# hyx1999/SAM-Decoding

Hardware: AMD Instinct MI355X
Metric: tokens/sec (+ mean accepted tokens), Vicuna-7B bs=1, samd_sam_only draft+verify (higher is better)
Workload: dtype f16

## Files before the change

sam-decoding_amd/csrc/gemm_kernels.hip:

```cpp
#include <hip/hip_runtime.h>
#include <cstdlib>
#include <type_traits>
#include "samd_common.h"

#define LAUNCHCHK() do { hipError_t e_ = hipGetLastError(); if (e_ != hipSuccess) { samd_set_error("kernel launch: %s", hipGetErrorString(e_)); return SAMD_E_HIP; } } while (0)

static int samd_cu_count() { return samd_device_cus(); }

typedef _Float16 half8 __attribute__((ext_vector_type(8)));
typedef __bf16 bf16x8 __attribute__((ext_vector_type(8)));
typedef float floatx4 __attribute__((ext_vector_type(4)));
typedef unsigned u32x4 __attribute__((ext_vector_type(4)));

struct GF16 { typedef _Float16 elem; typedef half8 vec8;
    static __device__ __forceinline__ floatx4 mfma(half8 a, half8 b, floatx4 c) { return __builtin_amdgcn_mfma_f32_16x16x32_f16(a, b, c, 0, 0, 0); } };
struct GBF16 { typedef __bf16 elem; typedef bf16x8 vec8;
    static __device__ __forceinline__ floatx4 mfma(bf16x8 a, bf16x8 b, floatx4 c) { return __builtin_amdgcn_mfma_f32_16x16x32_bf16(a, b, c, 0, 0, 0); } };

#define GEMM_KC 256
#define GEMM_WAVES 8
#define GEMM_COLS (16 * GEMM_WAVES)

typedef __attribute__((address_space(1))) const void *gptr_t;
typedef __attribute__((address_space(3))) void *lptr_t;

#ifdef SAMD_GEMM_ABLATE
__device__ int samd_abl_flag;
#endif

template <typename TT, int RT, int EPI, int DEPTH, bool GM = false>
__global__ __launch_bounds__(64 * GEMM_WAVES, RT >= 3 || DEPTH > 2 ? 2 : GEMM_WAVES / 2) void k_gemm_skinny(const typename TT::elem *__restrict__ A, const typename TT::elem *__restrict__ W,
                                                        float *__restrict__ partial, typename TT::elem *__restrict__ out,
                                                        int K, int N, int n_chunks, int n_splits) {
    typedef typename TT::elem E;
    typedef typename TT::vec8 V8;
    constexpr int R = 16 * RT;
    constexpr int NT = 64 * GEMM_WAVES;
    constexpr int XV = (R * 32) / NT;
    constexpr int NB = DEPTH + 1;
    extern __shared__ __attribute__((aligned(1024))) char gemm_lds[];
    E (*xs)[R][GEMM_KC] = reinterpret_cast<E (*)[R][GEMM_KC]>(gemm_lds);

    const int tid = threadIdx.x, w = tid >> 6, l = tid & 63, n = l & 15, g = l >> 4;
    const int n0 = blockIdx.x * GEMM_COLS + 16 * w;
    const int split = blockIdx.y;
    const int c0 = (int)((long long)split * n_chunks / n_splits), c1 = (int)((long long)(split + 1) * n_chunks / n_splits);
    constexpr size_t WCH = GM ? 8192 : 65536, WU = GM ? 1024 : 8192;
    const int ws = GM ? __builtin_amdgcn_readfirstlane(GEMM_WAVES * (int)blockIdx.x + w) : (int)blockIdx.x;
    const char *wtile = reinterpret_cast<const char *>(W) + (size_t)ws * n_chunks * WCH;
    const uint32_t wlane = (uint32_t)(GM ? l : tid) * 16;
    const uint32_t lds_base = (uint32_t)(uintptr_t)(lptr_t)&xs[0][0][0];

    floatx4 acc[RT];
#pragma unroll
    for (int mt = 0; mt < RT; mt++) acc[mt] = (floatx4){0.f, 0.f, 0.f, 0.f};

    u32x4 wr[DEPTH][4][2];
    auto load_wb = [&](u32x4 (&dst)[4][2], int c, int b) {
        const char *p = wtile + (size_t)c * WCH;
#pragma unroll
        for (int j = 0; j < 2; j++)
            asm volatile("global_load_dwordx4 %0, %1, %2 nt" : "=v"(dst[b][j]) : "v"(wlane), "s"(p + WU * (2 * b + j)) : "memory");
    };
    auto stage_xi = [&](int c, int buf, int i) {
        const int slot = tid + NT * i, row = slot >> 5, pos = slot & 31, unit = pos ^ (row & 15);
        const E *src = A + (size_t)row * K + (size_t)c * GEMM_KC + 8 * unit;
        E *dst = &xs[buf][0][0] + (size_t)(NT * i + 64 * w) * 8;
        __builtin_amdgcn_global_load_lds((gptr_t)src, (lptr_t)dst, 16, 0, 0);
        asm volatile("" ::: "memory");
    };
    auto load_w = [&](u32x4 (&dst)[4][2], int c) {
#pragma unroll
        for (int b = 0; b < 4; b++) load_wb(dst, c, b);
    };
    auto stage_x = [&](int c, int buf) {
#pragma unroll
        for (int i = 0; i < XV; i++) stage_xi(c, buf, i);
    };
    auto landed = [&](int younger_in_flight) {
        if (DEPTH > 2 && younger_in_flight >= 2) asm volatile("s_waitcnt vmcnt(%0)" : : "n"(2 * (8 + XV)) : "memory");
        else if (younger_in_flight >= 1) asm volatile("s_waitcnt vmcnt(%0)" : : "n"(8 + XV) : "memory");
        else asm volatile("s_waitcnt vmcnt(0)" : : : "memory");
        __builtin_amdgcn_s_barrier();
        asm volatile("" ::: "memory");
    };
    auto phase = [&](u32x4 (&cur)[4][2], int c, int buf) {
        landed(c1 - 1 - c);
        const uint32_t xbase = lds_base + (uint32_t)buf * (R * GEMM_KC * 2) + (uint32_t)n * (GEMM_KC * 2);
#pragma unroll
        for (int b = 0; b < 4; b++) {
            const uint32_t u0 = (uint32_t)((8 * b + 2 * g) ^ n) * 16, u1 = (uint32_t)((8 * b + 2 * g + 1) ^ n) * 16;
            const uint32_t a0 = xbase + u0, a1 = xbase + u1;
            u32x4 r[RT][2];
            if constexpr (RT == 1)
                asm volatile("ds_read_b128 %0, %2\n\tds_read_b128 %1, %3\n\ts_waitcnt lgkmcnt(0)" : "=&v"(r[0][0]), "=&v"(r[0][1]) : "v"(a0), "v"(a1));
            else if constexpr (RT == 2)
                asm volatile("ds_read_b128 %0, %4\n\tds_read_b128 %1, %5\n\tds_read_b128 %2, %4 offset:8192\n\tds_read_b128 %3, %5 offset:8192\n\t"
                             "s_waitcnt lgkmcnt(0)" : "=&v"(r[0][0]), "=&v"(r[0][1]), "=&v"(r[1][0]), "=&v"(r[1][1]) : "v"(a0), "v"(a1));
            else if constexpr (RT == 3)
                asm volatile("ds_read_b128 %0, %6\n\tds_read_b128 %1, %7\n\tds_read_b128 %2, %6 offset:8192\n\tds_read_b128 %3, %7 offset:8192\n\t"
                             "ds_read_b128 %4, %6 offset:16384\n\tds_read_b128 %5, %7 offset:16384\n\ts_waitcnt lgkmcnt(0)"
                             : "=&v"(r[0][0]), "=&v"(r[0][1]), "=&v"(r[1][0]), "=&v"(r[1][1]), "=&v"(r[2][0]), "=&v"(r[2][1]) : "v"(a0), "v"(a1));
            else
                asm volatile("ds_read_b128 %0, %8\n\tds_read_b128 %1, %9\n\tds_read_b128 %2, %8 offset:8192\n\tds_read_b128 %3, %9 offset:8192\n\t"
                             "ds_read_b128 %4, %8 offset:16384\n\tds_read_b128 %5, %9 offset:16384\n\tds_read_b128 %6, %8 offset:24576\n\t"
                             "ds_read_b128 %7, %9 offset:24576\n\ts_waitcnt lgkmcnt(0)"
                             : "=&v"(r[0][0]), "=&v"(r[0][1]), "=&v"(r[1][0]), "=&v"(r[1][1]), "=&v"(r[2][0]), "=&v"(r[2][1]), "=&v"(r[3][0]), "=&v"(r[3][1])
                             : "v"(a0), "v"(a1));
#pragma unroll
            for (int mt = 0; mt < RT; mt++) {
                acc[mt] = TT::mfma(__builtin_bit_cast(V8, r[mt][0]), __builtin_bit_cast(V8, cur[b][0]), acc[mt]);
                acc[mt] = TT::mfma(__builtin_bit_cast(V8, r[mt][1]), __builtin_bit_cast(V8, cur[b][1]), acc[mt]);
            }
            if (RT >= 3 && c + DEPTH < c1) {
                load_wb(cur, c + DEPTH, b);
                if (b < XV) stage_xi(c + DEPTH, buf == 0 ? NB - 1 : buf - 1, b);
            }
        }
        if (RT < 3 && c + DEPTH < c1) { load_w(cur, c + DEPTH); stage_x(c + DEPTH, buf == 0 ? NB - 1 : buf - 1); }
    };
    if (c0 < c1) {
#pragma unroll
        for (int d = 0; d < DEPTH; d++)
            if (c0 + d < c1) { load_w(wr[d], c0 + d); stage_x(c0 + d, d); }
        int buf = 0;
        for (int c = c0; c < c1; c += DEPTH) {
#pragma unroll
            for (int d = 0; d < DEPTH; d++)
                if (c + d < c1) { phase(wr[d], c + d, buf); buf = buf == NB - 1 ? 0 : buf + 1; }
        }
    }
    if constexpr (EPI == 1) {
        float *ex = reinterpret_cast<float *>(gemm_lds);
        __syncthreads();
        if (w >= 4) {
#pragma unroll
            for (int mt = 0; mt < RT; mt++)
#pragma unroll
                for (int r = 0; r < 4; r++) ex[(16 * mt + 4 * g + r) * 64 + 16 * (w - 4) + n] = acc[mt][r];
        }
        __syncthreads();
        if (w < 4) {
#pragma unroll
            for (int mt = 0; mt < RT; mt++)
#pragma unroll
                for (int r = 0; r < 4; r++) {
                    const int m = 16 * mt + 4 * g + r;
                    const float gf = (float)(E)acc[mt][r], uf = (float)(E)ex[m * 64 + 16 * w + n];
                    const E sv = (E)(gf / (1.f + __expf(-gf)));
                    out[(size_t)m * (N / 2) + blockIdx.x * 64 + 16 * w + n] = (E)((float)sv * uf);
                }
        }
        return;
    }
#pragma unroll
    for (int mt = 0; mt < RT; mt++) {
#pragma unroll
        for (int r = 0; r < 4; r++) {
            const int m = 16 * mt + 4 * g + r;
            if (out) out[(size_t)m * N + n0 + n] = (E)acc[mt][r];
            else __hip_atomic_store(&partial[((size_t)split * R + m) * N + n0 + n], acc[mt][r], __ATOMIC_RELAXED, __HIP_MEMORY_SCOPE_AGENT);
        }
    }
}

struct NormArgs { const float *ssq; const void *g; int tiles; float inv_hidden; float eps; };

#define NORM_NS 16
template <int NT>
__device__ __forceinline__ void norm_issue(const NormArgs &na, float (&sv)[NORM_NS]) {
    const int tid = threadIdx.x, row = tid & 15, p = tid >> 4;
#pragma unroll
    for (int k = 0; k < NORM_NS; k++) {
        sv[k] = 0.f;
        if ((NT / 16) * k >= na.tiles) continue;
        int t = p + (NT / 16) * k;
        t = t < na.tiles ? t : na.tiles - 1;
        const float *src = na.ssq + (size_t)t * 16 + row;
        asm volatile("global_load_dword %0, %1, off" : "=v"(sv[k]) : "v"(src) : "memory");
    }
}
template <int NT>
__device__ __forceinline__ void norm_finish(const NormArgs &na, float (&sv)[NORM_NS], float *part , float *rs ) {
    const int tid = threadIdx.x, row = tid & 15, p = tid >> 4;
    static_assert(NORM_NS == 16, "");
    asm volatile("" : "+v"(sv[0]), "+v"(sv[1]), "+v"(sv[2]), "+v"(sv[3]), "+v"(sv[4]), "+v"(sv[5]), "+v"(sv[6]), "+v"(sv[7]),
                      "+v"(sv[8]), "+v"(sv[9]), "+v"(sv[10]), "+v"(sv[11]), "+v"(sv[12]), "+v"(sv[13]), "+v"(sv[14]), "+v"(sv[15]) : : "memory");
    float s = 0.f;
#pragma unroll
    for (int k = 0; k < NORM_NS; k++) s += (p + (NT / 16) * k < na.tiles) ? sv[k] : 0.f;
    part[p * 16 + row] = s;
    asm volatile("s_waitcnt lgkmcnt(0)" ::: "memory");
    __builtin_amdgcn_s_barrier();
    asm volatile("" ::: "memory");
    if (tid < 16) {
        float tot = 0.f;
        for (int k = 0; k < NT / 16; k++) tot += part[k * 16 + tid];
        rs[tid] = rsqrtf(tot * na.inv_hidden + na.eps);
    }
    asm volatile("s_waitcnt lgkmcnt(0)" ::: "memory");
    __builtin_amdgcn_s_barrier();
    asm volatile("" ::: "memory");
}

template <typename E>
__device__ __forceinline__ u32x4 norm_scale8(u32x4 xraw, u32x4 graw, float rs) {
    const E *xe = reinterpret_cast<const E *>(&xraw);
    const E *ge = reinterpret_cast<const E *>(&graw);
    u32x4 out;
    E *oe = reinterpret_cast<E *>(&out);
#pragma unroll
    for (int j = 0; j < 8; j++) { const E h = (E)((float)xe[j] * rs); oe[j] = (E)((float)ge[j] * (float)h); }
    return out;
}


template <int DEPTH, int PC>
__device__ __forceinline__ void gemm_wait_younger(int younger) {
    if constexpr (PC == 0) asm volatile("s_waitcnt vmcnt(0)" : : : "memory");
    else {
        if (DEPTH > 3 && younger >= 3) asm volatile("s_waitcnt vmcnt(%0)" : : "n"(3 * PC) : "memory");
        else if (DEPTH > 2 && younger >= 2) asm volatile("s_waitcnt vmcnt(%0)" : : "n"(2 * PC) : "memory");
        else if (younger >= 1) asm volatile("s_waitcnt vmcnt(%0)" : : "n"(PC) : "memory");
        else asm volatile("s_waitcnt vmcnt(0)" : : : "memory");
    }
}

template <typename TT, int RT, int DEPTH, int CG, bool NORM, int AR = 16>
__global__ __launch_bounds__(64 * GEMM_WAVES, RT >= 3 || NORM ? 2 : GEMM_WAVES / 2) void k_gemm_qkv_rope(
        const typename TT::elem *__restrict__ A, const typename TT::elem *__restrict__ W, int K, int n_chunks,
        const float *__restrict__ cs, const int *__restrict__ d_L, const int *__restrict__ d_n,
        typename TT::elem *__restrict__ q_out, typename TT::elem *__restrict__ k_cache, typename TT::elem *__restrict__ v_cache,
        int H, int Hkv, long long max_len, NormArgs na, int v_t) {
    typedef typename TT::elem E;
    typedef typename TT::vec8 V8;
    constexpr int R = 16 * RT;
    constexpr int NT = 64 * GEMM_WAVES;
    constexpr int XV = (R * 32) / NT;
    constexpr int NB = DEPTH + 1;
    constexpr int WL = 4;
    constexpr int TW = 16 * CG, PP = 8 * CG;
    constexpr int CH = CG * 8192;
    extern __shared__ __attribute__((aligned(1024))) char gemm_lds[];
    E (*xs)[R][GEMM_KC] = reinterpret_cast<E (*)[R][GEMM_KC]>(gemm_lds);

    const int tid = threadIdx.x, w = tid >> 6, l = tid & 63, n = l & 15, g = l >> 4;
    const bool streams = CG == 4 || w < 2 * CG;
    static_assert(AR == 16 || (AR == 8 && NORM && RT == 1), "8 activation rows: the norm-fold kernels only");
    const bool stager = AR == 16 || w < GEMM_WAVES / 2;
    const int cg = CG == 4 ? (w & 3) : (streams ? w % CG : 0), kh = CG == 4 ? (w >> 2) : (streams ? w / CG : 0);
    const char *wtile = reinterpret_cast<const char *>(W) + (size_t)blockIdx.x * n_chunks * CH;
    const uint32_t wlane = (uint32_t)(64 * (CG * kh + cg) + l) * 16;
    const uint32_t lds_base = (uint32_t)(uintptr_t)(lptr_t)&xs[0][0][0];
    const int n_rows = d_n[0], L = d_L[0];

    floatx4 acc[RT];
#pragma unroll
    for (int mt = 0; mt < RT; mt++) acc[mt] = (floatx4){0.f, 0.f, 0.f, 0.f};

    u32x4 wr[DEPTH][2][2];
    auto load_wb = [&](u32x4 (&dst)[2][2], int c, int bl) {
        const char *p = wtile + (size_t)c * CH;
#pragma unroll
        for (int j = 0; j < 2; j++)
            asm volatile("global_load_dwordx4 %0, %1, %2 nt" : "=v"(dst[bl][j]) : "v"(wlane), "s"(p + (CH / 4) * (2 * bl + j)) : "memory");
    };
    static_assert(!NORM || RT == 1, "the norm-fold path is built for the 16-row tile");
    constexpr int XL = NORM ? 2 * XV : XV;
    u32x4 xr[NORM ? DEPTH : 1][NORM ? XV : 1], gr[NORM ? DEPTH : 1][NORM ? XV : 1];
    __shared__ float norm_part[NORM ? (NT / 16) * 16 : 1], norm_rs[NORM ? 16 : 1];
    auto stage_xi = [&](int c, int buf, int i, int d) {
        const int slot = tid + NT * i, row = slot >> 5, pos = slot & 31, unit = pos ^ (row & 15);
        const E *src = A + (size_t)row * K + (size_t)c * GEMM_KC + 8 * unit;
        if constexpr (NORM) {
            const E *gsrc = reinterpret_cast<const E *>(na.g) + (size_t)c * GEMM_KC + 8 * unit;
            asm volatile("global_load_dwordx4 %0, %1, off" : "=v"(xr[d][i]) : "v"(src) : "memory");
            asm volatile("global_load_dwordx4 %0, %1, off" : "=v"(gr[d][i]) : "v"(gsrc) : "memory");
        } else {
            E *dst = &xs[buf][0][0] + (size_t)(NT * i + 64 * w) * 8;
            __builtin_amdgcn_global_load_lds((gptr_t)src, (lptr_t)dst, 16, 0, 0);
            asm volatile("" ::: "memory");
        }
    };
    auto issue = [&](u32x4 (&dst)[2][2], int c, int buf, int d) {
        if (streams) { load_wb(dst, c, 0); load_wb(dst, c, 1); }
        if (stager) {
#pragma unroll
            for (int i = 0; i < XV; i++) stage_xi(c, buf, i, d);
        }
    };
    auto scale_to_lds = [&](int buf, int d) {
        if constexpr (NORM) {
            if (!stager) return;
#pragma unroll
            for (int i = 0; i < XV; i++) {
                const int slot = tid + NT * i, row = slot >> 5;
                asm volatile("" : "+v"(xr[d][i]), "+v"(gr[d][i]) : : "memory");
                const u32x4 v = norm_scale8<E>(xr[d][i], gr[d][i], norm_rs[row]);
                *reinterpret_cast<u32x4 *>(&xs[buf][0][0] + (size_t)slot * 8) = v;
            }
        }
    };
    auto landed = [&](int younger, int buf, int d) {
        if (streams) { if (stager) gemm_wait_younger<DEPTH, WL + XL>(younger); else gemm_wait_younger<DEPTH, WL>(younger); }
        else { if (stager) gemm_wait_younger<DEPTH, XL>(younger); else gemm_wait_younger<DEPTH, 0>(younger); }
        if constexpr (NORM) { scale_to_lds(buf, d); asm volatile("s_waitcnt lgkmcnt(0)" ::: "memory"); }
        __builtin_amdgcn_s_barrier();
        asm volatile("" ::: "memory");
    };
    auto phase = [&](u32x4 (&cur)[2][2], int c, int buf, int d) {
        landed(n_chunks - 1 - c, buf, d);
        const uint32_t xbase = lds_base + (uint32_t)buf * (R * GEMM_KC * 2) + (uint32_t)n * (GEMM_KC * 2);
#pragma unroll
        for (int bl = 0; bl < 2; bl++) {
            if (!streams) break;
            const int b = 2 * kh + bl;
            const uint32_t a0 = xbase + (uint32_t)((8 * b + 2 * g) ^ n) * 16, a1 = xbase + (uint32_t)((8 * b + 2 * g + 1) ^ n) * 16;
            u32x4 r[RT][2];
            if constexpr (RT == 1)
                asm volatile("ds_read_b128 %0, %2\n\tds_read_b128 %1, %3\n\ts_waitcnt lgkmcnt(0)" : "=&v"(r[0][0]), "=&v"(r[0][1]) : "v"(a0), "v"(a1));
            else if constexpr (RT == 2)
                asm volatile("ds_read_b128 %0, %4\n\tds_read_b128 %1, %5\n\tds_read_b128 %2, %4 offset:8192\n\tds_read_b128 %3, %5 offset:8192\n\t"
                             "s_waitcnt lgkmcnt(0)" : "=&v"(r[0][0]), "=&v"(r[0][1]), "=&v"(r[1][0]), "=&v"(r[1][1]) : "v"(a0), "v"(a1));
            else if constexpr (RT == 3)
                asm volatile("ds_read_b128 %0, %6\n\tds_read_b128 %1, %7\n\tds_read_b128 %2, %6 offset:8192\n\tds_read_b128 %3, %7 offset:8192\n\t"
                             "ds_read_b128 %4, %6 offset:16384\n\tds_read_b128 %5, %7 offset:16384\n\ts_waitcnt lgkmcnt(0)"
                             : "=&v"(r[0][0]), "=&v"(r[0][1]), "=&v"(r[1][0]), "=&v"(r[1][1]), "=&v"(r[2][0]), "=&v"(r[2][1]) : "v"(a0), "v"(a1));
            else
                asm volatile("ds_read_b128 %0, %8\n\tds_read_b128 %1, %9\n\tds_read_b128 %2, %8 offset:8192\n\tds_read_b128 %3, %9 offset:8192\n\t"
                             "ds_read_b128 %4, %8 offset:16384\n\tds_read_b128 %5, %9 offset:16384\n\tds_read_b128 %6, %8 offset:24576\n\t"
                             "ds_read_b128 %7, %9 offset:24576\n\ts_waitcnt lgkmcnt(0)"
                             : "=&v"(r[0][0]), "=&v"(r[0][1]), "=&v"(r[1][0]), "=&v"(r[1][1]), "=&v"(r[2][0]), "=&v"(r[2][1]), "=&v"(r[3][0]), "=&v"(r[3][1])
                             : "v"(a0), "v"(a1));
#pragma unroll
            for (int mt = 0; mt < RT; mt++) {
                acc[mt] = TT::mfma(__builtin_bit_cast(V8, r[mt][0]), __builtin_bit_cast(V8, cur[bl][0]), acc[mt]);
                acc[mt] = TT::mfma(__builtin_bit_cast(V8, r[mt][1]), __builtin_bit_cast(V8, cur[bl][1]), acc[mt]);
            }
        }
        if (c + DEPTH < n_chunks) issue(cur, c + DEPTH, buf == 0 ? NB - 1 : buf - 1, d);
    };
    float norm_sv[NORM ? NORM_NS : 1];
    if constexpr (NORM) norm_issue<NT>(na, norm_sv);
#pragma unroll
    for (int d = 0; d < DEPTH; d++)
        if (d < n_chunks) issue(wr[d], d, d, d);
    if constexpr (AR == 8) {
        if (!stager) {
#pragma unroll
            for (int bz = 0; bz < NB; bz++) *reinterpret_cast<u32x4 *>(&xs[bz][0][0] + (size_t)tid * 8) = (u32x4){0u, 0u, 0u, 0u};
        }
    }
    if constexpr (NORM) {
        if (n_chunks >= DEPTH) {
            if (streams) { if (stager) asm volatile("s_waitcnt vmcnt(%0)" : : "n"(DEPTH * (WL + XL)) : "memory"); else asm volatile("s_waitcnt vmcnt(%0)" : : "n"(DEPTH * WL) : "memory"); }
            else { if (stager) asm volatile("s_waitcnt vmcnt(%0)" : : "n"(DEPTH * XL) : "memory"); else asm volatile("s_waitcnt vmcnt(0)" : : : "memory"); }
        } else asm volatile("s_waitcnt vmcnt(0)" : : : "memory");
        norm_finish<NT>(na, norm_sv, norm_part, norm_rs);
    }
    {
        int buf = 0;
        for (int c = 0; c < n_chunks; c += DEPTH) {
#pragma unroll
            for (int d = 0; d < DEPTH; d++)
                if (c + d < n_chunks) { phase(wr[d], c + d, buf, d); buf = buf == NB - 1 ? 0 : buf + 1; }
        }
    }
    float *ex = reinterpret_cast<float *>(gemm_lds);
    __syncthreads();
    if (streams) {
#pragma unroll
        for (int mt = 0; mt < RT; mt++)
#pragma unroll
            for (int r = 0; r < 4; r++) ex[(kh * R + 16 * mt + 4 * g + r) * TW + 16 * cg + n] = acc[mt][r];
    }
    __syncthreads();
    const bool vt_tile = v_t && ((PP * (int)blockIdx.x) >> 6) >= H + Hkv;
    for (int i = tid; i < R * PP; i += NT) {
        const int row = vt_tile ? i % R : i / PP, p = vt_tile ? i / R : i % PP;
        if (row >= n_rows || L + row >= max_len) continue;
        const float x1 = (float)(E)(ex[row * TW + p] + ex[(R + row) * TW + p]);
        const float x2 = (float)(E)(ex[row * TW + PP + p] + ex[(R + row) * TW + PP + p]);
        const int pair = PP * (int)blockIdx.x + p, head = pair >> 6, j = pair & 63;
        if (head >= H + Hkv) {
            if (v_t) {
                E *dst = v_cache + (size_t)(head - H - Hkv) * max_len * 128 + L + row;
                dst[(size_t)j * max_len] = (E)x1; dst[(size_t)(j + 64) * max_len] = (E)x2;
                continue;
            }
            E *dst = v_cache + ((size_t)(head - H - Hkv) * max_len + L + row) * 128;
            dst[j] = (E)x1; dst[j + 64] = (E)x2;
            continue;
        }
        const float c = cs[(size_t)row * 128 + j], sn = cs[(size_t)row * 128 + 64 + j];
        const E o1 = (E)(x1 * c - x2 * sn), o2 = (E)(x2 * c + x1 * sn);
        E *dst = head < H ? q_out + ((size_t)row * H + head) * 128 : k_cache + ((size_t)(head - H) * max_len + L + row) * 128;
        dst[j] = o1; dst[j + 64] = o2;
    }
}

template <int CG>
__global__ __launch_bounds__(256) void k_gemm_pack_qkv(const uint4 *__restrict__ W, uint4 *__restrict__ out, int N, int K) {
    const long long u = (long long)blockIdx.x * 256 + threadIdx.x;
    const long long total = (long long)N * K / 8;
    if (u >= total) return;
    constexpr int PP = 8 * CG;
    const int n_chunks = K / GEMM_KC;
    const long long blk = u / (512 * CG);
    const int in = (int)(u % (512 * CG)), jj = in / (128 * CG), x = in % (128 * CG), w = x >> 6, g = (x >> 4) & 3, n = x & 15, cg = w % CG, kh = w / CG;
    const int t = (int)(blk / n_chunks), c = (int)(blk % n_chunks), bl = jj >> 1, j = jj & 1;
    const int q = 16 * cg + n, pair = PP * t + (q < PP ? q : q - PP);
    const long long row = 128LL * (pair >> 6) + (pair & 63) + (q < PP ? 0 : 64), col = 256LL * c + 64 * (2 * kh + bl) + 16 * g + 8 * j;
    out[u] = W[(row * K + col) / 8];
}

static int qkv_tile_groups(int n_heads_total) {
    static const int env = [] { const char *e = getenv("SAMD_QKV_TILE"); return e ? atoi(e) : 0; }();
    const int n_cu = samd_cu_count();
    const int N = n_heads_total * 128;
    if (N % 48 != 0 || env == 64) return 4;
    if (env == 48) return 3;
    const int t48 = N / 48, t64 = N / 64;
    return ((t48 + n_cu - 1) / n_cu) * 48 < ((t64 + n_cu - 1) / n_cu) * 64 ? 3 : 4;
}

template <typename TT, int RT, int DEPTH, bool NORM, int AR = 16>
__global__ __launch_bounds__(64 * GEMM_WAVES, RT >= 3 || DEPTH > 2 ? 2 : GEMM_WAVES / 2) void k_gemm_pairs_silu(const typename TT::elem *__restrict__ A, const typename TT::elem *__restrict__ W,
                                                                                                     typename TT::elem *__restrict__ out, int K, int inter, int n_chunks, int n_pairs, NormArgs na) {
    typedef typename TT::elem E;
    typedef typename TT::vec8 V8;
    constexpr int R = 16 * RT;
    constexpr int NT = 64 * GEMM_WAVES;
    constexpr int XV = (R * 32) / NT;
    constexpr int NB = DEPTH + 1;
    extern __shared__ __attribute__((aligned(1024))) char gemm_lds[];
    E (*xs)[R][GEMM_KC] = reinterpret_cast<E (*)[R][GEMM_KC]>(gemm_lds);

    const int tid = threadIdx.x, w = __builtin_amdgcn_readfirstlane(tid >> 6), l = tid & 63, n = l & 15, g = l >> 4;
#ifdef SAMD_GEMM_ABLATE
    const int abl = samd_abl_flag;
#else
    constexpr int abl = 0;
#endif
    const int p0 = (int)((long long)blockIdx.x * n_pairs / gridDim.x), p1 = (int)((long long)(blockIdx.x + 1) * n_pairs / gridDim.x);
    const bool active = w < 2 * (p1 - p0);
    static_assert(AR == 16 || (AR == 8 && NORM && RT == 1), "8 activation rows: the norm-fold kernels only");
    const bool stager = AR == 16 || w < GEMM_WAVES / 2;
    const int gi = 2 * p0 + w;
    const char *wgrp = reinterpret_cast<const char *>(W) + (size_t)(active ? gi : 0) * n_chunks * 8192;
    const uint32_t wlane = (uint32_t)l * 16;
    const uint32_t lds_base = (uint32_t)(uintptr_t)(lptr_t)&xs[0][0][0];

    floatx4 acc[RT];
#pragma unroll
    for (int mt = 0; mt < RT; mt++) acc[mt] = (floatx4){0.f, 0.f, 0.f, 0.f};
    u32x4 wr[DEPTH][4][2];
    auto load_w = [&](u32x4 (&dst)[4][2], int c) {
        const char *p = wgrp + (size_t)c * 8192;
#pragma unroll
        for (int b = 0; b < 4; b++)
#pragma unroll
            for (int j = 0; j < 2; j++)
                asm volatile("global_load_dwordx4 %0, %1, %2 nt" : "=v"(dst[b][j]) : "v"(wlane), "s"(p + 1024 * (2 * b + j)) : "memory");
    };
    static_assert(!NORM || RT == 1, "the norm-fold path is built for the 16-row tile");
    constexpr int XL = NORM ? 2 * XV : XV;
    u32x4 xr[NORM ? DEPTH : 1][NORM ? XV : 1], gr[NORM ? DEPTH : 1][NORM ? XV : 1];
    __shared__ float norm_part[NORM ? (NT / 16) * 16 : 1], norm_rs[NORM ? 16 : 1];
    auto stage_x = [&](int c, int buf, int d) {
        if (!stager || (abl & 4)) return;
#pragma unroll
        for (int i = 0; i < XV; i++) {
            const int slot = tid + NT * i, row = slot >> 5, pos = slot & 31, unit = pos ^ (row & 15);
            const E *src = A + (size_t)((abl & 8) ? (row & 15) : row) * K + (size_t)c * GEMM_KC + 8 * unit;
            if constexpr (NORM) {
                const E *gsrc = reinterpret_cast<const E *>(na.g) + (size_t)c * GEMM_KC + 8 * unit;
                asm volatile("global_load_dwordx4 %0, %1, off" : "=v"(xr[d][i]) : "v"(src) : "memory");
                asm volatile("global_load_dwordx4 %0, %1, off" : "=v"(gr[d][i]) : "v"(gsrc) : "memory");
            } else {
                E *dst = &xs[buf][0][0] + (size_t)(NT * i + 64 * w) * 8;
                __builtin_amdgcn_global_load_lds((gptr_t)src, (lptr_t)dst, 16, 0, 0);
                asm volatile("" ::: "memory");
            }
        }
    };
    auto landed = [&](int younger, int buf, int d) {
        const bool stg = stager && !(abl & 4);
        if (active) { if (stg) gemm_wait_younger<DEPTH, 8 + XL>(younger); else gemm_wait_younger<DEPTH, 8>(younger); }
        else { if (stg) gemm_wait_younger<DEPTH, XL>(younger); else gemm_wait_younger<DEPTH, 0>(younger); }
        if constexpr (NORM) {
            if (stager) {
#pragma unroll
                for (int i = 0; i < XV; i++) {
                    const int slot = tid + NT * i, row = slot >> 5;
                    asm volatile("" : "+v"(xr[d][i]), "+v"(gr[d][i]) : : "memory");
                    const u32x4 v = norm_scale8<E>(xr[d][i], gr[d][i], norm_rs[row]);
                    *reinterpret_cast<u32x4 *>(&xs[buf][0][0] + (size_t)slot * 8) = v;
                }
            }
            asm volatile("s_waitcnt lgkmcnt(0)" ::: "memory");
        }
        if (!(abl & 1)) __builtin_amdgcn_s_barrier();
        asm volatile("" ::: "memory");
    };
    auto phase = [&](u32x4 (&cur)[4][2], int c, int buf, int d) {
        landed(n_chunks - 1 - c, buf, d);
        if (active && !(abl & 2)) {
            const uint32_t xbase = lds_base + (uint32_t)buf * (R * GEMM_KC * 2) + (uint32_t)n * (GEMM_KC * 2);
#pragma unroll
            for (int b = 0; b < 4; b++) {
                const uint32_t a0 = xbase + (uint32_t)((8 * b + 2 * g) ^ n) * 16, a1 = xbase + (uint32_t)((8 * b + 2 * g + 1) ^ n) * 16;
                u32x4 r[RT][2];
                if constexpr (RT == 1)
                    asm volatile("ds_read_b128 %0, %2\n\tds_read_b128 %1, %3\n\ts_waitcnt lgkmcnt(0)" : "=&v"(r[0][0]), "=&v"(r[0][1]) : "v"(a0), "v"(a1));
                else if constexpr (RT == 2)
                    asm volatile("ds_read_b128 %0, %4\n\tds_read_b128 %1, %5\n\tds_read_b128 %2, %4 offset:8192\n\tds_read_b128 %3, %5 offset:8192\n\t"
                                 "s_waitcnt lgkmcnt(0)" : "=&v"(r[0][0]), "=&v"(r[0][1]), "=&v"(r[1][0]), "=&v"(r[1][1]) : "v"(a0), "v"(a1));
                else if constexpr (RT == 3)
                    asm volatile("ds_read_b128 %0, %6\n\tds_read_b128 %1, %7\n\tds_read_b128 %2, %6 offset:8192\n\tds_read_b128 %3, %7 offset:8192\n\t"
                                 "ds_read_b128 %4, %6 offset:16384\n\tds_read_b128 %5, %7 offset:16384\n\ts_waitcnt lgkmcnt(0)"
                                 : "=&v"(r[0][0]), "=&v"(r[0][1]), "=&v"(r[1][0]), "=&v"(r[1][1]), "=&v"(r[2][0]), "=&v"(r[2][1]) : "v"(a0), "v"(a1));
                else
                    asm volatile("ds_read_b128 %0, %8\n\tds_read_b128 %1, %9\n\tds_read_b128 %2, %8 offset:8192\n\tds_read_b128 %3, %9 offset:8192\n\t"
                                 "ds_read_b128 %4, %8 offset:16384\n\tds_read_b128 %5, %9 offset:16384\n\tds_read_b128 %6, %8 offset:24576\n\t"
                                 "ds_read_b128 %7, %9 offset:24576\n\ts_waitcnt lgkmcnt(0)"
                                 : "=&v"(r[0][0]), "=&v"(r[0][1]), "=&v"(r[1][0]), "=&v"(r[1][1]), "=&v"(r[2][0]), "=&v"(r[2][1]), "=&v"(r[3][0]), "=&v"(r[3][1])
                                 : "v"(a0), "v"(a1));
#pragma unroll
                for (int mt = 0; mt < RT; mt++) {
                    acc[mt] = TT::mfma(__builtin_bit_cast(V8, r[mt][0]), __builtin_bit_cast(V8, cur[b][0]), acc[mt]);
                    acc[mt] = TT::mfma(__builtin_bit_cast(V8, r[mt][1]), __builtin_bit_cast(V8, cur[b][1]), acc[mt]);
                }
            }
        }
        if (c + DEPTH < n_chunks) { if (active) load_w(cur, c + DEPTH); stage_x(c + DEPTH, buf == 0 ? NB - 1 : buf - 1, d); }
    };
    float norm_sv[NORM ? NORM_NS : 1];
    if constexpr (NORM) norm_issue<NT>(na, norm_sv);
#pragma unroll
    for (int d = 0; d < DEPTH; d++)
        if (d < n_chunks) { if (active) load_w(wr[d], d); stage_x(d, d, d); }
    if constexpr (AR == 8) {
        if (!stager) {
#pragma unroll
            for (int bz = 0; bz < NB; bz++) *reinterpret_cast<u32x4 *>(&xs[bz][0][0] + (size_t)tid * 8) = (u32x4){0u, 0u, 0u, 0u};
        }
    }
    if constexpr (NORM) {
        if (n_chunks >= DEPTH) {
            if (active) { if (stager) asm volatile("s_waitcnt vmcnt(%0)" : : "n"(DEPTH * (8 + XL)) : "memory"); else asm volatile("s_waitcnt vmcnt(%0)" : : "n"(DEPTH * 8) : "memory"); }
            else { if (stager) asm volatile("s_waitcnt vmcnt(%0)" : : "n"(DEPTH * XL) : "memory"); else asm volatile("s_waitcnt vmcnt(0)" : : : "memory"); }
        } else asm volatile("s_waitcnt vmcnt(0)" : : : "memory");
        norm_finish<NT>(na, norm_sv, norm_part, norm_rs);
    }
    {
        int buf = 0;
        for (int c = 0; c < n_chunks; c += DEPTH) {
#pragma unroll
            for (int d = 0; d < DEPTH; d++)
                if (c + d < n_chunks) { phase(wr[d], c + d, buf, d); buf = buf == NB - 1 ? 0 : buf + 1; }
        }
    }
    float *ex = reinterpret_cast<float *>(gemm_lds);
    __syncthreads();
    if (active && (w & 1)) {
#pragma unroll
        for (int mt = 0; mt < RT; mt++)
#pragma unroll
            for (int r = 0; r < 4; r++) ex[((w >> 1) * R + 16 * mt + 4 * g + r) * 16 + n] = acc[mt][r];
    }
    __syncthreads();
    if (active && !(w & 1)) {
        const int col = 16 * (p0 + (w >> 1)) + n;
#pragma unroll
        for (int mt = 0; mt < RT; mt++)
#pragma unroll
            for (int r = 0; r < 4; r++) {
                const int m = 16 * mt + 4 * g + r;
                const float gf = (float)(E)acc[mt][r], uf = (float)(E)ex[((w >> 1) * R + m) * 16 + n];
                const E sv = (E)(gf / (1.f + __expf(-gf)));
                out[(size_t)m * inter + col] = (E)((float)sv * uf);
            }
    }
}

template <typename TT, int ROWS, bool EARLY = false>
__global__ __launch_bounds__(64 * GEMM_WAVES, 2) void k_gemm_cs_residual(const typename TT::elem *__restrict__ A, const typename TT::elem *__restrict__ W,
                                                                           typename TT::elem *__restrict__ x, float *__restrict__ ssq, int K, int N, int n_chunks,
                                                                           const int *__restrict__ counter = nullptr, int *__restrict__ epoch = nullptr,
                                                                           int arrivals = 0) {
    typedef typename TT::elem E;
    typedef typename TT::vec8 V8;
    constexpr int CSD = 2;
    extern __shared__ __attribute__((aligned(1024))) char gemm_lds[];
    const int tid = threadIdx.x, w = __builtin_amdgcn_readfirstlane(tid >> 6), l = tid & 63, n = l & 15, g = l >> 4;
    E *xs = reinterpret_cast<E *>(gemm_lds) + (size_t)w * CSD * 16 * GEMM_KC;
    const uint32_t lds_base = (uint32_t)(uintptr_t)(lptr_t)xs;
    const char *wgrp = reinterpret_cast<const char *>(W) + (size_t)blockIdx.x * n_chunks * 8192;
    const uint32_t wlane = (uint32_t)l * 16;

    static_assert(ROWS == 8 || ROWS == 16, "");
    constexpr int AL = ROWS / 2;
    if constexpr (ROWS == 8) {
#pragma unroll
        for (int buf = 0; buf < CSD; buf++)
#pragma unroll
            for (int i = 4; i < 8; i++)
                *reinterpret_cast<u32x4 *>(xs + (size_t)buf * 16 * GEMM_KC + (size_t)(64 * i + l) * 8) = (u32x4){0u, 0u, 0u, 0u};
        asm volatile("s_waitcnt lgkmcnt(0)" ::: "memory");
    }
    floatx4 acc = (floatx4){0.f, 0.f, 0.f, 0.f};
    u32x4 wr[CSD][4][2];
    auto issue_w = [&](u32x4 (&dst)[4][2], int c) {
        const char *p = wgrp + (size_t)c * 8192;
#pragma unroll
        for (int b = 0; b < 4; b++)
#pragma unroll
            for (int j = 0; j < 2; j++)
                asm volatile("global_load_dwordx4 %0, %1, %2 nt" : "=v"(dst[b][j]) : "v"(wlane), "s"(p + 1024 * (2 * b + j)) : "memory");
    };
    auto issue_a = [&](int c, int buf) {
#pragma unroll
        for (int i = 0; i < AL; i++) {
            const int slot = l + 64 * i, row = slot >> 5, pos = slot & 31, unit = pos ^ (row & 15);
            const E *src = A + (size_t)row * K + (size_t)c * GEMM_KC + 8 * unit;
            E *dst_l = xs + (size_t)buf * 16 * GEMM_KC + (size_t)(64 * i) * 8;
            __builtin_amdgcn_global_load_lds((gptr_t)src, (lptr_t)dst_l, 16, 0, 0);
            asm volatile("" ::: "memory");
        }
    };
    auto issue = [&](u32x4 (&dst)[4][2], int c, int buf) { issue_w(dst, c); issue_a(c, buf); };
    auto phase = [&](u32x4 (&cur)[4][2], int c, int buf, bool more) {
        if (more) { if constexpr (EARLY) asm volatile("s_waitcnt vmcnt(%0)" : : "n"(AL) : "memory"); else asm volatile("s_waitcnt vmcnt(%0)" : : "n"(8 + AL) : "memory"); }
        else asm volatile("s_waitcnt vmcnt(0)" ::: "memory");
        const uint32_t xbase = lds_base + (uint32_t)buf * (16 * GEMM_KC * 2) + (uint32_t)n * (GEMM_KC * 2);
#pragma unroll
        for (int b = 0; b < 4; b++) {
            const uint32_t a0 = xbase + (uint32_t)((8 * b + 2 * g) ^ n) * 16, a1 = xbase + (uint32_t)((8 * b + 2 * g + 1) ^ n) * 16;
            u32x4 r0, r1;
            asm volatile("ds_read_b128 %0, %2\n\tds_read_b128 %1, %3\n\ts_waitcnt lgkmcnt(0)" : "=&v"(r0), "=&v"(r1) : "v"(a0), "v"(a1));
            acc = TT::mfma(__builtin_bit_cast(V8, r0), __builtin_bit_cast(V8, cur[b][0]), acc);
            acc = TT::mfma(__builtin_bit_cast(V8, r1), __builtin_bit_cast(V8, cur[b][1]), acc);
        }
    };
    const int mine = (n_chunks - w + GEMM_WAVES - 1) / GEMM_WAVES;
    if constexpr (EARLY) {
        if (mine > 0) issue_w(wr[0], w);
        if (mine > 1) issue_w(wr[1], w + GEMM_WAVES);
        __shared__ int my_epoch;
        if (tid == 0) {
            const int e = epoch[blockIdx.x];
            const int target = (e + 1) * arrivals;
            for (int spin = 0; spin < (1 << 22); spin++) {
                if (__hip_atomic_load(counter, __ATOMIC_RELAXED, __HIP_MEMORY_SCOPE_AGENT) >= target) break;
                __builtin_amdgcn_s_sleep(4);
            }
            my_epoch = e;
        }
        __syncthreads();
        __builtin_amdgcn_fence(__ATOMIC_ACQUIRE, "agent");
        if (mine > 0) issue_a(w, 0);
        if (mine > 1) issue_a(w + GEMM_WAVES, 1);
        if (mine > 0) phase(wr[0], w, 0, mine > 1);
        if (mine > 1) phase(wr[1], w + GEMM_WAVES, 1, false);
        if (tid == 0) epoch[blockIdx.x] = my_epoch + 1;
    } else {
        if (mine > 0) issue(wr[0], w, 0);
        if (mine > 1) issue(wr[1], w + GEMM_WAVES, 1);
        for (int i = 0; i < mine; i += 2) {
            phase(wr[0], w + GEMM_WAVES * i, 0, i + 1 < mine);
            if (i + 2 < mine) issue(wr[0], w + GEMM_WAVES * (i + 2), 0);
            if (i + 1 < mine) {
                phase(wr[1], w + GEMM_WAVES * (i + 1), 1, i + 2 < mine);
                if (i + 3 < mine) issue(wr[1], w + GEMM_WAVES * (i + 3), 1);
            }
        }
    }
    __syncthreads();
    float *ex = reinterpret_cast<float *>(gemm_lds);
#pragma unroll
    for (int r = 0; r < 4; r++) ex[(w * 16 + 4 * g + r) * 16 + n] = acc[r];
    __syncthreads();
    if (tid < 16 * ROWS) {
        const int row = tid >> 4, col = tid & 15;
        float sum = 0.f;
#pragma unroll
        for (int k = 0; k < GEMM_WAVES; k++) sum += ex[(k * 16 + row) * 16 + col];
        E *xp = x + (size_t)row * N + 16 * blockIdx.x + col;
        const E o = (E)sum;
        const E y = (E)((float)*xp + (float)o);
        *xp = y;
        float q = (float)y * (float)y;
        q += __shfl_xor(q, 1); q += __shfl_xor(q, 2); q += __shfl_xor(q, 4); q += __shfl_xor(q, 8);
        if (col == 0) ssq[(size_t)blockIdx.x * 16 + row] = q;
    }
}

__global__ __launch_bounds__(256) void k_gemm_pack_groups(const uint4 *__restrict__ W, uint4 *__restrict__ out, int N, int K) {
    const long long u = (long long)blockIdx.x * 256 + threadIdx.x;
    const long long total = (long long)N * K / 8;
    if (u >= total) return;
    const int n_chunks = K / GEMM_KC;
    const long long blk = u >> 9;
    const int in = (int)(u & 511), jj = in >> 6, lane = in & 63, g = lane >> 4, n = lane & 15, b = jj >> 1, j = jj & 1;
    const long long gi = blk / n_chunks; const int c = (int)(blk % n_chunks);
    const long long row = 16 * gi + n, col = 256LL * c + 64 * b + 16 * g + 8 * j;
    out[u] = W[(row * K + col) / 8];
}

__global__ __launch_bounds__(256) void k_gemm_pack(const uint4 *__restrict__ W, uint4 *__restrict__ out, int N, int K) {
    const long long u = (long long)blockIdx.x * 256 + threadIdx.x;
    const long long total = (long long)N * K / 8;
    if (u >= total) return;
    const int n_chunks = K / GEMM_KC;
    const long long blk = u >> 12;
    const int in = (int)(u & 4095), jj = in >> 9, tid = in & 511, w = tid >> 6, g = (tid >> 4) & 3, n = tid & 15;
    const int t = (int)(blk / n_chunks), c = (int)(blk % n_chunks), b = jj >> 1, j = jj & 1;
    const long long row = 128LL * t + 16 * w + n, col = 256LL * c + 64 * b + 16 * g + 8 * j;
    out[u] = W[(row * K + col) / 8];
}

template <typename TT, int RT, int EPI, int DEPTH, bool GM = false>
static hipError_t gemm_launch(dim3 grid, hipStream_t st, const void *A, const void *W, float *partial, void *out, int K, int N, int chunks, int splits) {
    constexpr int lds = (DEPTH + 1) * 16 * RT * GEMM_KC * 2;
    if constexpr (lds > 65536) {
        static unsigned long long done = 0ull;
        const hipError_t attr = samd_reserve_lds((const void *)k_gemm_skinny<TT, RT, EPI, DEPTH, GM>, lds, &done);
        if (attr != hipSuccess) return attr;
    }
    hipLaunchKernelGGL((k_gemm_skinny<TT, RT, EPI, DEPTH, GM>), grid, dim3(64 * GEMM_WAVES), lds, st, (const typename TT::elem *)A, (const typename TT::elem *)W, partial,
                       (typename TT::elem *)out, K, N, chunks, splits);
    return hipSuccess;
}

template <int EPI, bool GM = false>
static hipError_t gemm_dispatch(int dtype, int rows_pad, dim3 grid, hipStream_t st, const void *A, const void *W, float *partial, void *out, int K, int N, int chunks,
                                int splits) {
#define GO(TT, RT, D) return gemm_launch<TT, RT, EPI, D, GM>(grid, st, A, W, partial, out, K, N, chunks, splits)
#define ROWS(TT) do { if (rows_pad == 16) GO(TT, 1, 2); else if (rows_pad == 32) GO(TT, 2, 2); else if (rows_pad == 48) GO(TT, 3, 2); else GO(TT, 4, 2); } while (0)
    if (dtype == SAMD_F16) ROWS(GF16); else ROWS(GBF16);
#undef ROWS
#undef GO
}

template <typename TT, int RT, int DEPTH, int CG, bool NORM = false, int AR = 16>
static hipError_t qkv_rope_launch(hipStream_t st, const void *A, const void *W, int K, int tiles, const float *cs, const int *d_L, const int *d_n, void *q, void *k, void *v,
                                  int H, int Hkv, long long max_len, int v_t, NormArgs na = NormArgs{nullptr, nullptr, 0, 0.f, 0.f}) {
    constexpr int lds_a = (DEPTH + 1) * 16 * RT * GEMM_KC * 2, lds_e = 2 * 16 * RT * 16 * CG * 4, lds = lds_a > lds_e ? lds_a : lds_e;
    if constexpr (lds > 60000) {
        static unsigned long long done = 0ull;
        const hipError_t attr = samd_reserve_lds((const void *)k_gemm_qkv_rope<TT, RT, DEPTH, CG, NORM, AR>, lds + 4096, &done);
        if (attr != hipSuccess) return attr;
    }
    hipLaunchKernelGGL((k_gemm_qkv_rope<TT, RT, DEPTH, CG, NORM, AR>), dim3(tiles), dim3(64 * GEMM_WAVES), lds, st, (const typename TT::elem *)A, (const typename TT::elem *)W, K, K / GEMM_KC,
                       cs, d_L, d_n, (typename TT::elem *)q, (typename TT::elem *)k, (typename TT::elem *)v, H, Hkv, max_len, na, v_t);
    return hipSuccess;
}

template <typename TT, int RT, int DEPTH, bool NORM = false, int AR = 16>
static hipError_t pairs_silu_launch(hipStream_t st, int grid, const void *A, const void *W, void *out, int K, int inter, int n_pairs,
                                    NormArgs na = NormArgs{nullptr, nullptr, 0, 0.f, 0.f}) {
    constexpr int lds_a = (DEPTH + 1) * 16 * RT * GEMM_KC * 2, lds_e = 4 * 16 * RT * 16 * 4, lds = lds_a > lds_e ? lds_a : lds_e;
    if constexpr (lds > 60000) {
        static unsigned long long done = 0ull;
        const hipError_t attr = samd_reserve_lds((const void *)k_gemm_pairs_silu<TT, RT, DEPTH, NORM, AR>, lds + 4096, &done);
        if (attr != hipSuccess) return attr;
    }
    hipLaunchKernelGGL((k_gemm_pairs_silu<TT, RT, DEPTH, NORM, AR>), dim3(grid), dim3(64 * GEMM_WAVES), lds, st, (const typename TT::elem *)A, (const typename TT::elem *)W,
                       (typename TT::elem *)out, K, inter, K / GEMM_KC, n_pairs, na);
    return hipSuccess;
}

extern "C" {

int samd_gemm_splits(int32_t N, int32_t K, int32_t rows_pad) {
    static const int env_cap = [] { const char *e = getenv("SAMD_GEMM_SPLIT_CAP"); const int v = e ? atoi(e) : 8; return v < 1 ? 1 : (v > 8 ? 8 : v); }();
    static const int env_fixed = [] { const char *e = getenv("SAMD_GEMM_SPLITS"); const int v = e ? atoi(e) : 0; return v < 0 ? 0 : (v > 8 ? 8 : v); }();
    const int cols = N / GEMM_COLS, chunks = K / GEMM_KC;
    (void)rows_pad;
    if (env_fixed) return env_fixed > chunks ? (chunks < 1 ? 1 : chunks) : env_fixed;
    int s = 256 / (cols > 0 ? cols : 1);
    if (s > env_cap) s = env_cap;
    if (s > chunks) s = chunks;
    return s < 1 ? 1 : s;
}

int64_t samd_gemm_workspace(int32_t rows_pad, int32_t N, int32_t splits) { return (int64_t)splits * rows_pad * N * 4; }

int samd_gemm_skinny_silu(const void *d_A, const void *d_W, int32_t rows_pad, int32_t N, int32_t K, void *d_out, int32_t dtype, void *stream) {
    if (!d_A || !d_W || !d_out || (rows_pad != 16 && rows_pad != 32 && rows_pad != 48 && rows_pad != 64) || N < GEMM_COLS || N % GEMM_COLS != 0 || K < GEMM_KC ||
        K % GEMM_KC != 0 || (dtype != SAMD_F16 && dtype != SAMD_BF16)) {
        samd_set_error("samd_gemm_skinny_silu: unsupported shape (rows 16/32/48/64, N %% 128 == 0, K %% 256 == 0) or null pointer"); return SAMD_E_INVALID;
    }
    const hipError_t e = gemm_dispatch<1>(dtype, rows_pad, dim3(N / GEMM_COLS, 1), (hipStream_t)stream, d_A, d_W, nullptr, d_out, K, N, K / GEMM_KC, 1);
    if (e != hipSuccess) { samd_set_error("samd_gemm_skinny_silu: %s", hipGetErrorString(e)); return SAMD_E_HIP; }
    LAUNCHCHK();
    return SAMD_OK;
}

int samd_gemm_pack_weights(const void *d_W, void *d_packed, int32_t N, int32_t K, void *stream) {
    if (!d_W || !d_packed || d_W == d_packed || N < GEMM_COLS || N % GEMM_COLS != 0 || K < GEMM_KC || K % GEMM_KC != 0) {
        samd_set_error("samd_gemm_pack_weights: needs N %% 128 == 0, K %% 256 == 0 and distinct buffers"); return SAMD_E_INVALID;
    }
    const long long units = (long long)N * K / 8;
    hipLaunchKernelGGL(k_gemm_pack, dim3((unsigned)((units + 255) / 256)), dim3(256), 0, (hipStream_t)stream, (const uint4 *)d_W, (uint4 *)d_packed, N, K);
    LAUNCHCHK();
    return SAMD_OK;
}

int samd_gemm_pack_groups(const void *d_W, void *d_packed, int32_t N, int32_t K, void *stream) {
    if (!d_W || !d_packed || d_W == d_packed || N < 16 || N % 16 != 0 || K < GEMM_KC || K % GEMM_KC != 0) {
        samd_set_error("samd_gemm_pack_groups: needs N %% 16 == 0, K %% 256 == 0 and distinct buffers"); return SAMD_E_INVALID;
    }
    const long long units = (long long)N * K / 8;
    hipLaunchKernelGGL(k_gemm_pack_groups, dim3((unsigned)((units + 255) / 256)), dim3(256), 0, (hipStream_t)stream, (const uint4 *)d_W, (uint4 *)d_packed, N, K);
    LAUNCHCHK();
    return SAMD_OK;
}

int samd_gemm_pairs_silu_norm(const void *d_x, const float *d_ssq, const void *d_norm_weight, float eps, const void *d_Wg, int32_t rows_pad, int32_t inter, int32_t K,
                              void *d_out, int32_t dtype, void *stream) {
    if (!d_x || !d_ssq || !d_norm_weight || !d_Wg || !d_out || (rows_pad != 16 && rows_pad != 8) || inter < 16 || inter % 16 != 0 || K < GEMM_KC || K % GEMM_KC != 0 ||
        K / 16 > 32 * NORM_NS || (dtype != SAMD_F16 && dtype != SAMD_BF16)) {
        samd_set_error("samd_gemm_pairs_silu_norm: unsupported shape (8 or 16 rows, inter %% 16 == 0, K %% 256 == 0, K <= 8192, f16/bf16) or null pointer"); return SAMD_E_INVALID;
    }
    const int n_cu = samd_cu_count();
    const int n_pairs = inter / 16;
    int grid = n_pairs < n_cu ? n_pairs : n_cu;
    while ((n_pairs + grid - 1) / grid > 4) grid += n_cu;
    const NormArgs na{d_ssq, d_norm_weight, K / 16, 1.f / (float)K, eps};
    hipStream_t st = (hipStream_t)stream;
    const hipError_t e = rows_pad == 8
        ? (dtype == SAMD_F16 ? pairs_silu_launch<GF16, 1, 3, true, 8>(st, grid, d_x, d_Wg, d_out, K, inter, n_pairs, na)
                             : pairs_silu_launch<GBF16, 1, 3, true, 8>(st, grid, d_x, d_Wg, d_out, K, inter, n_pairs, na))
        : (dtype == SAMD_F16 ? pairs_silu_launch<GF16, 1, 3, true>(st, grid, d_x, d_Wg, d_out, K, inter, n_pairs, na)
                             : pairs_silu_launch<GBF16, 1, 3, true>(st, grid, d_x, d_Wg, d_out, K, inter, n_pairs, na));
    if (e != hipSuccess) { samd_set_error("samd_gemm_pairs_silu_norm: %s", hipGetErrorString(e)); return SAMD_E_HIP; }
    LAUNCHCHK();
    return SAMD_OK;
}

int samd_gemm_cs_residual(const void *d_A, const void *d_Wg, int32_t rows_pad, int32_t N, int32_t K, void *d_x, float *d_ssq, int32_t dtype, void *stream) {
    if (!d_A || !d_Wg || !d_x || !d_ssq || (rows_pad != 16 && rows_pad != 8) || N < 16 || N % 16 != 0 || K < GEMM_KC || K % GEMM_KC != 0 || (dtype != SAMD_F16 && dtype != SAMD_BF16)) {
        samd_set_error("samd_gemm_cs_residual: unsupported shape (8 or 16 rows, N %% 16 == 0, K %% 256 == 0, f16/bf16) or null pointer"); return SAMD_E_INVALID;
    }
    constexpr int lds = GEMM_WAVES * 2 * 16 * GEMM_KC * 2;
    hipStream_t st = (hipStream_t)stream;
    hipError_t e = hipSuccess;
#define GO(TT, ROWS, ET) do { static unsigned long long done = 0ull; \
        e = samd_reserve_lds((const void *)k_gemm_cs_residual<TT, ROWS>, lds, &done); \
        if (e == hipSuccess) hipLaunchKernelGGL((k_gemm_cs_residual<TT, ROWS>), dim3(N / 16), dim3(64 * GEMM_WAVES), lds, st, (const ET *)d_A, (const ET *)d_Wg, (ET *)d_x, d_ssq, K, N, K / GEMM_KC, (const int *)nullptr, (int *)nullptr, 0); } while (0)
    if (dtype == SAMD_F16) { if (rows_pad == 8) GO(GF16, 8, _Float16); else GO(GF16, 16, _Float16); }
    else { if (rows_pad == 8) GO(GBF16, 8, __bf16); else GO(GBF16, 16, __bf16); }
#undef GO
    if (e != hipSuccess) { samd_set_error("samd_gemm_cs_residual: %s", hipGetErrorString(e)); return SAMD_E_HIP; }
    LAUNCHCHK();
    return SAMD_OK;
}

int samd_gemm_cs_residual_early(const void *d_A, const void *d_Wg, int32_t N, int32_t K, void *d_x, float *d_ssq, int32_t dtype, const int32_t *d_counter,
                                int32_t *d_epoch, int32_t arrivals, void *stream) {
    if (!d_A || !d_Wg || !d_x || !d_ssq || !d_counter || !d_epoch || arrivals < 1 || N < 16 || N % 16 != 0 || K != 2 * GEMM_WAVES * GEMM_KC ||
        (dtype != SAMD_F16 && dtype != SAMD_BF16)) {
        samd_set_error("samd_gemm_cs_residual_early: unsupported shape (K must be 4096, N %% 16 == 0, f16/bf16) or null pointer"); return SAMD_E_INVALID;
    }
    constexpr int lds = GEMM_WAVES * 2 * 16 * GEMM_KC * 2;
    hipStream_t st = (hipStream_t)stream;
    hipError_t e = hipSuccess;
    if (dtype == SAMD_F16) {
        static unsigned long long done = 0ull;
        e = samd_reserve_lds((const void *)k_gemm_cs_residual<GF16, 8, true>, lds, &done);
        if (e == hipSuccess) hipLaunchKernelGGL((k_gemm_cs_residual<GF16, 8, true>), dim3(N / 16), dim3(64 * GEMM_WAVES), lds, st, (const _Float16 *)d_A, (const _Float16 *)d_Wg,
                                                (_Float16 *)d_x, d_ssq, K, N, K / GEMM_KC, d_counter, d_epoch, arrivals);
    } else {
        static unsigned long long done = 0ull;
        e = samd_reserve_lds((const void *)k_gemm_cs_residual<GBF16, 8, true>, lds, &done);
        if (e == hipSuccess) hipLaunchKernelGGL((k_gemm_cs_residual<GBF16, 8, true>), dim3(N / 16), dim3(64 * GEMM_WAVES), lds, st, (const __bf16 *)d_A, (const __bf16 *)d_Wg,
                                                (__bf16 *)d_x, d_ssq, K, N, K / GEMM_KC, d_counter, d_epoch, arrivals);
    }
    if (e != hipSuccess) { samd_set_error("samd_gemm_cs_residual_early: %s", hipGetErrorString(e)); return SAMD_E_HIP; }
    LAUNCHCHK();
    return SAMD_OK;
}

int samd_gemm_pairs_silu(const void *d_A, const void *d_Wg, int32_t rows_pad, int32_t inter, int32_t K, void *d_out, int32_t dtype, void *stream) {
    if (!d_A || !d_Wg || !d_out || (rows_pad != 16 && rows_pad != 32 && rows_pad != 48 && rows_pad != 64) || inter < 16 || inter % 16 != 0 || K < GEMM_KC ||
        K % GEMM_KC != 0 || (dtype != SAMD_F16 && dtype != SAMD_BF16)) {
        samd_set_error("samd_gemm_pairs_silu: unsupported shape (rows 16/32/48/64, inter %% 16 == 0, K %% 256 == 0, f16/bf16) or null pointer"); return SAMD_E_INVALID;
    }
    const int n_cu = samd_cu_count();
    const int n_pairs = inter / 16;
    int grid = n_pairs < n_cu ? n_pairs : n_cu;
    while ((n_pairs + grid - 1) / grid > 4) grid += n_cu;
    hipStream_t st = (hipStream_t)stream;
    hipError_t e;
    static const int depth_env = [] { const char *e = getenv("SAMD_PAIRS_DEPTH"); return e ? atoi(e) : 0; }();
#ifdef SAMD_GEMM_ABLATE
    static const int abl_set = [] { const char *e = getenv("SAMD_GEMM_ABL"); const int v = e ? atoi(e) : 0; return hipMemcpyToSymbol(HIP_SYMBOL(samd_abl_flag), &v, 4) == hipSuccess ? 1 : -1; }();
    (void)abl_set;
#endif
#define ARGS st, grid, d_A, d_Wg, d_out, K, inter, n_pairs
#define GO(TT) (rows_pad == 16 ? (depth_env == 2 ? pairs_silu_launch<TT, 1, 2>(ARGS) : depth_env == 4 ? pairs_silu_launch<TT, 1, 4>(ARGS) : pairs_silu_launch<TT, 1, 3>(ARGS)) \
                : rows_pad == 32 ? (depth_env == 2 ? pairs_silu_launch<TT, 2, 2>(ARGS) : pairs_silu_launch<TT, 2, 3>(ARGS)) \
                : rows_pad == 48 ? pairs_silu_launch<TT, 3, 2>(ARGS) : pairs_silu_launch<TT, 4, 2>(ARGS))
    e = dtype == SAMD_F16 ? GO(GF16) : GO(GBF16);
#undef GO
#undef ARGS
    if (e != hipSuccess) { samd_set_error("samd_gemm_pairs_silu: %s", hipGetErrorString(e)); return SAMD_E_HIP; }
    LAUNCHCHK();
    return SAMD_OK;
}

int samd_gemm_pack_qkv64(const void *d_W, void *d_packed, int32_t n_heads_total, int32_t K, void *stream) {
    if (!d_W || !d_packed || d_W == d_packed || n_heads_total < 1 || K < GEMM_KC || K % GEMM_KC != 0) {
        samd_set_error("samd_gemm_pack_qkv64: needs K %% 256 == 0, whole 128-column heads and distinct buffers"); return SAMD_E_INVALID;
    }
    const long long units = (long long)n_heads_total * 128 * K / 8;
    if (qkv_tile_groups(n_heads_total) == 3)
        hipLaunchKernelGGL(k_gemm_pack_qkv<3>, dim3((unsigned)((units + 255) / 256)), dim3(256), 0, (hipStream_t)stream, (const uint4 *)d_W, (uint4 *)d_packed, n_heads_total * 128, K);
    else
        hipLaunchKernelGGL(k_gemm_pack_qkv<4>, dim3((unsigned)((units + 255) / 256)), dim3(256), 0, (hipStream_t)stream, (const uint4 *)d_W, (uint4 *)d_packed, n_heads_total * 128, K);
    LAUNCHCHK();
    return SAMD_OK;
}

static int gemm_qkv_rope_impl(const void *d_A, const void *d_W64, int32_t rows_pad, int32_t K, const float *d_cs, const int32_t *d_cache_length, const int32_t *d_n,
                              void *d_q_out, void *d_k_cache, void *d_v_cache, int32_t n_heads, int32_t n_kv_heads, int32_t head_dim, int64_t max_len,
                              int32_t dtype, void *stream, int v_t) {
    if (!d_A || !d_W64 || !d_cs || !d_cache_length || !d_n || !d_q_out || !d_k_cache || !d_v_cache || head_dim != 128 || n_heads < 1 || n_kv_heads < 1 ||
        (rows_pad != 16 && rows_pad != 32 && rows_pad != 48 && rows_pad != 64) || K < GEMM_KC || K % GEMM_KC != 0 || (dtype != SAMD_F16 && dtype != SAMD_BF16)) {
        samd_set_error("samd_gemm_qkv_rope: unsupported shape (rows 16/32/48/64, head_dim 128, K %% 256 == 0, f16/bf16) or null pointer"); return SAMD_E_INVALID;
    }
    static const int depth_env = [] { const char *e = getenv("SAMD_QKV_DEPTH"); return e ? atoi(e) : 0; }();
    const int groups = qkv_tile_groups(n_heads + 2 * n_kv_heads);
    const int tiles = (n_heads + 2 * n_kv_heads) * 128 / (16 * groups);
    hipStream_t st = (hipStream_t)stream;
    hipError_t e = hipSuccess;
#define GO(TT, RT, D, CG) e = qkv_rope_launch<TT, RT, D, CG>(st, d_A, d_W64, K, tiles, d_cs, d_cache_length, d_n, d_q_out, d_k_cache, d_v_cache, n_heads, n_kv_heads, (long long)max_len, v_t)
#define ROWS(TT, CG) do { if (rows_pad == 16) { if (depth_env == 2) GO(TT, 1, 2, CG); else if (depth_env == 3) GO(TT, 1, 3, CG); else GO(TT, 1, 4, CG); } \
                          else if (rows_pad == 32) { if (depth_env == 2) GO(TT, 2, 2, CG); else GO(TT, 2, 4, CG); } \
                          else if (rows_pad == 48) GO(TT, 3, 3, CG); else GO(TT, 4, 3, CG); } while (0)
    if (groups == 3) { if (dtype == SAMD_F16) ROWS(GF16, 3); else ROWS(GBF16, 3); }
    else { if (dtype == SAMD_F16) ROWS(GF16, 4); else ROWS(GBF16, 4); }
#undef ROWS
#undef GO
    if (e != hipSuccess) { samd_set_error("samd_gemm_qkv_rope: %s", hipGetErrorString(e)); return SAMD_E_HIP; }
    LAUNCHCHK();
    return SAMD_OK;
}

int samd_gemm_qkv_rope(const void *d_A, const void *d_W64, int32_t rows_pad, int32_t K, const float *d_cs, const int32_t *d_cache_length, const int32_t *d_n,
                       void *d_q_out, void *d_k_cache, void *d_v_cache, int32_t n_heads, int32_t n_kv_heads, int32_t head_dim, int64_t max_len,
                       int32_t dtype, void *stream) {
    return gemm_qkv_rope_impl(d_A, d_W64, rows_pad, K, d_cs, d_cache_length, d_n, d_q_out, d_k_cache, d_v_cache, n_heads, n_kv_heads, head_dim, max_len, dtype, stream, 0);
}

int samd_gemm_qkv_rope_vt(const void *d_A, const void *d_W64, int32_t rows_pad, int32_t K, const float *d_cs, const int32_t *d_cache_length, const int32_t *d_n,
                          void *d_q_out, void *d_k_cache, void *d_vt_cache, int32_t n_heads, int32_t n_kv_heads, int32_t head_dim, int64_t max_len,
                          int32_t dtype, void *stream) {
    return gemm_qkv_rope_impl(d_A, d_W64, rows_pad, K, d_cs, d_cache_length, d_n, d_q_out, d_k_cache, d_vt_cache, n_heads, n_kv_heads, head_dim, max_len, dtype, stream, 1);
}

static int gemm_qkv_rope_norm_impl(const void *d_x, const float *d_ssq, const void *d_norm_weight, float eps, const void *d_W64, int32_t rows_pad, int32_t K,
                                   const float *d_cs, const int32_t *d_cache_length, const int32_t *d_n, void *d_q_out, void *d_k_cache, void *d_v_cache,
                                   int32_t n_heads, int32_t n_kv_heads, int32_t head_dim, int64_t max_len, int32_t dtype, void *stream, int v_t) {
    if (!d_x || !d_ssq || !d_norm_weight || !d_W64 || !d_cs || !d_cache_length || !d_n || !d_q_out || !d_k_cache || !d_v_cache || head_dim != 128 || n_heads < 1 ||
        n_kv_heads < 1 || (rows_pad != 16 && rows_pad != 8) || K < GEMM_KC || K % GEMM_KC != 0 || K / 16 > 32 * NORM_NS || (dtype != SAMD_F16 && dtype != SAMD_BF16)) {
        samd_set_error("samd_gemm_qkv_rope_norm: unsupported shape (8 or 16 rows, head_dim 128, K %% 256 == 0, K <= 8192, f16/bf16) or null pointer"); return SAMD_E_INVALID;
    }
    const int groups = qkv_tile_groups(n_heads + 2 * n_kv_heads);
    const int tiles = (n_heads + 2 * n_kv_heads) * 128 / (16 * groups);
    const NormArgs na{d_ssq, d_norm_weight, K / 16, 1.f / (float)K, eps};
    hipStream_t st = (hipStream_t)stream;
    hipError_t e = hipSuccess;
#define GO(TT, CG, AR) e = qkv_rope_launch<TT, 1, 4, CG, true, AR>(st, d_x, d_W64, K, tiles, d_cs, d_cache_length, d_n, d_q_out, d_k_cache, d_v_cache, n_heads, n_kv_heads, (long long)max_len, v_t, na)
    if (rows_pad == 8) {
        if (groups == 3) { if (dtype == SAMD_F16) GO(GF16, 3, 8); else GO(GBF16, 3, 8); }
        else { if (dtype == SAMD_F16) GO(GF16, 4, 8); else GO(GBF16, 4, 8); }
    } else {
        if (groups == 3) { if (dtype == SAMD_F16) GO(GF16, 3, 16); else GO(GBF16, 3, 16); }
        else { if (dtype == SAMD_F16) GO(GF16, 4, 16); else GO(GBF16, 4, 16); }
    }
#undef GO
    if (e != hipSuccess) { samd_set_error("samd_gemm_qkv_rope_norm: %s", hipGetErrorString(e)); return SAMD_E_HIP; }
    LAUNCHCHK();
    return SAMD_OK;
}

int samd_gemm_qkv_rope_norm(const void *d_x, const float *d_ssq, const void *d_norm_weight, float eps, const void *d_W64, int32_t rows_pad, int32_t K,
                            const float *d_cs, const int32_t *d_cache_length, const int32_t *d_n, void *d_q_out, void *d_k_cache, void *d_v_cache,
                            int32_t n_heads, int32_t n_kv_heads, int32_t head_dim, int64_t max_len, int32_t dtype, void *stream) {
    return gemm_qkv_rope_norm_impl(d_x, d_ssq, d_norm_weight, eps, d_W64, rows_pad, K, d_cs, d_cache_length, d_n, d_q_out, d_k_cache, d_v_cache, n_heads, n_kv_heads, head_dim,
                                   max_len, dtype, stream, 0);
}

int samd_gemm_qkv_rope_norm_vt(const void *d_x, const float *d_ssq, const void *d_norm_weight, float eps, const void *d_W64, int32_t rows_pad, int32_t K,
                               const float *d_cs, const int32_t *d_cache_length, const int32_t *d_n, void *d_q_out, void *d_k_cache, void *d_vt_cache,
                               int32_t n_heads, int32_t n_kv_heads, int32_t head_dim, int64_t max_len, int32_t dtype, void *stream) {
    return gemm_qkv_rope_norm_impl(d_x, d_ssq, d_norm_weight, eps, d_W64, rows_pad, K, d_cs, d_cache_length, d_n, d_q_out, d_k_cache, d_vt_cache, n_heads, n_kv_heads, head_dim,
                                   max_len, dtype, stream, 1);
}

int samd_gemm_skinny(const void *d_A, const void *d_W, int32_t rows_pad, int32_t N, int32_t K, int32_t splits, float *d_partial,
                     void *d_out, int32_t dtype, void *stream) {
    if (!d_A || !d_W || (rows_pad != 16 && rows_pad != 32 && rows_pad != 48 && rows_pad != 64) || N < GEMM_COLS || N % GEMM_COLS != 0 || K < GEMM_KC ||
        K % GEMM_KC != 0 || splits < 1 || splits > K / GEMM_KC || (splits == 1 ? !d_out : !d_partial) || (dtype != SAMD_F16 && dtype != SAMD_BF16)) {
        samd_set_error("samd_gemm_skinny: unsupported shape (rows 16/32/48/64, N %% 128 == 0, K %% 256 == 0) or null pointer"); return SAMD_E_INVALID;
    }
    const hipError_t e = gemm_dispatch<0>(dtype, rows_pad, dim3(N / GEMM_COLS, splits), (hipStream_t)stream, d_A, d_W, d_partial, splits == 1 ? d_out : nullptr, K, N,
                                          K / GEMM_KC, splits);
    if (e != hipSuccess) { samd_set_error("samd_gemm_skinny: %s", hipGetErrorString(e)); return SAMD_E_HIP; }
    LAUNCHCHK();
    return SAMD_OK;
}

int samd_gemm_skinny_groups(const void *d_A, const void *d_Wg, int32_t rows_pad, int32_t N, int32_t K, int32_t splits, float *d_partial,
                            void *d_out, int32_t dtype, void *stream) {
    if (!d_A || !d_Wg || (rows_pad != 16 && rows_pad != 32 && rows_pad != 48 && rows_pad != 64) || N < GEMM_COLS || N % GEMM_COLS != 0 || K < GEMM_KC ||
        K % GEMM_KC != 0 || splits < 1 || splits > K / GEMM_KC || (splits == 1 ? !d_out : !d_partial) || (dtype != SAMD_F16 && dtype != SAMD_BF16)) {
        samd_set_error("samd_gemm_skinny_groups: unsupported shape (rows 16/32/48/64, N %% 128 == 0, K %% 256 == 0) or null pointer"); return SAMD_E_INVALID;
    }
    const hipError_t e = gemm_dispatch<0, true>(dtype, rows_pad, dim3(N / GEMM_COLS, splits), (hipStream_t)stream, d_A, d_Wg, d_partial, splits == 1 ? d_out : nullptr, K, N,
                                                K / GEMM_KC, splits);
    if (e != hipSuccess) { samd_set_error("samd_gemm_skinny_groups: %s", hipGetErrorString(e)); return SAMD_E_HIP; }
    LAUNCHCHK();
    return SAMD_OK;
}

}

template <typename TT> struct F8Widen;
template <> struct F8Widen<GF16> {
    static __device__ __forceinline__ half8 cvt(unsigned w0, unsigned w1) {
        const auto a = __builtin_amdgcn_cvt_scalef32_pk_f16_fp8(w0, 1.0f, false), b = __builtin_amdgcn_cvt_scalef32_pk_f16_fp8(w0, 1.0f, true);
        const auto c = __builtin_amdgcn_cvt_scalef32_pk_f16_fp8(w1, 1.0f, false), d = __builtin_amdgcn_cvt_scalef32_pk_f16_fp8(w1, 1.0f, true);
        return __builtin_bit_cast(half8, (u32x4){__builtin_bit_cast(unsigned, a), __builtin_bit_cast(unsigned, b), __builtin_bit_cast(unsigned, c), __builtin_bit_cast(unsigned, d)});
    }
};
template <> struct F8Widen<GBF16> {
    static __device__ __forceinline__ bf16x8 cvt(unsigned w0, unsigned w1) {
        const auto a = __builtin_amdgcn_cvt_scalef32_pk_bf16_fp8(w0, 1.0f, false), b = __builtin_amdgcn_cvt_scalef32_pk_bf16_fp8(w0, 1.0f, true);
        const auto c = __builtin_amdgcn_cvt_scalef32_pk_bf16_fp8(w1, 1.0f, false), d = __builtin_amdgcn_cvt_scalef32_pk_bf16_fp8(w1, 1.0f, true);
        return __builtin_bit_cast(bf16x8, (u32x4){__builtin_bit_cast(unsigned, a), __builtin_bit_cast(unsigned, b), __builtin_bit_cast(unsigned, c), __builtin_bit_cast(unsigned, d)});
    }
};

template <int RT>
__device__ __forceinline__ void gemm_read_a2(u32x4 (&r)[RT][2], uint32_t a0, uint32_t a1) {
    if constexpr (RT == 1)
        asm volatile("ds_read_b128 %0, %2\n\tds_read_b128 %1, %3\n\ts_waitcnt lgkmcnt(0)" : "=&v"(r[0][0]), "=&v"(r[0][1]) : "v"(a0), "v"(a1));
    else if constexpr (RT == 2)
        asm volatile("ds_read_b128 %0, %4\n\tds_read_b128 %1, %5\n\tds_read_b128 %2, %4 offset:8192\n\tds_read_b128 %3, %5 offset:8192\n\t"
                     "s_waitcnt lgkmcnt(0)" : "=&v"(r[0][0]), "=&v"(r[0][1]), "=&v"(r[1][0]), "=&v"(r[1][1]) : "v"(a0), "v"(a1));
    else if constexpr (RT == 3)
        asm volatile("ds_read_b128 %0, %6\n\tds_read_b128 %1, %7\n\tds_read_b128 %2, %6 offset:8192\n\tds_read_b128 %3, %7 offset:8192\n\t"
                     "ds_read_b128 %4, %6 offset:16384\n\tds_read_b128 %5, %7 offset:16384\n\ts_waitcnt lgkmcnt(0)"
                     : "=&v"(r[0][0]), "=&v"(r[0][1]), "=&v"(r[1][0]), "=&v"(r[1][1]), "=&v"(r[2][0]), "=&v"(r[2][1]) : "v"(a0), "v"(a1));
    else
        asm volatile("ds_read_b128 %0, %8\n\tds_read_b128 %1, %9\n\tds_read_b128 %2, %8 offset:8192\n\tds_read_b128 %3, %9 offset:8192\n\t"
                     "ds_read_b128 %4, %8 offset:16384\n\tds_read_b128 %5, %9 offset:16384\n\tds_read_b128 %6, %8 offset:24576\n\t"
                     "ds_read_b128 %7, %9 offset:24576\n\ts_waitcnt lgkmcnt(0)"
                     : "=&v"(r[0][0]), "=&v"(r[0][1]), "=&v"(r[1][0]), "=&v"(r[1][1]), "=&v"(r[2][0]), "=&v"(r[2][1]), "=&v"(r[3][0]), "=&v"(r[3][1])
                     : "v"(a0), "v"(a1));
}

template <typename TT, int RT, int DEPTH>
__global__ __launch_bounds__(64 * GEMM_WAVES, 2) void k_gemm_skinny_f8(const typename TT::elem *__restrict__ A, const unsigned char *__restrict__ W8,
                                                                     const float *__restrict__ scale, float *__restrict__ partial,
                                                                     typename TT::elem *__restrict__ out, int K, int N, int n_chunks, int n_splits) {
    typedef typename TT::elem E;
    constexpr int R = 16 * RT;
    constexpr int NT = 64 * GEMM_WAVES;
    constexpr int XV = (R * 32) / NT;
    constexpr int NB = DEPTH + 1;
    constexpr int PC = 4 + XV;
    constexpr size_t WCH = 32768, WU = 8192;
    extern __shared__ __attribute__((aligned(1024))) char gemm_lds[];
    E (*xs)[R][GEMM_KC] = reinterpret_cast<E (*)[R][GEMM_KC]>(gemm_lds);

    const int tid = threadIdx.x, w = tid >> 6, l = tid & 63, n = l & 15, g = l >> 4;
    const int n0 = blockIdx.x * GEMM_COLS + 16 * w;
    const int split = blockIdx.y;
    const int c0 = (int)((long long)split * n_chunks / n_splits), c1 = (int)((long long)(split + 1) * n_chunks / n_splits);
    const char *wtile = reinterpret_cast<const char *>(W8) + (size_t)blockIdx.x * n_chunks * WCH;
    const uint32_t wlane = (uint32_t)tid * 16;
    const uint32_t lds_base = (uint32_t)(uintptr_t)(lptr_t)&xs[0][0][0];
    const float sc = scale[n0 + n];

    floatx4 acc[RT];
#pragma unroll
    for (int mt = 0; mt < RT; mt++) acc[mt] = (floatx4){0.f, 0.f, 0.f, 0.f};

    u32x4 wr[DEPTH][4];
    auto load_wb = [&](u32x4 (&dst)[4], int c, int b) {
        const char *p = wtile + (size_t)c * WCH;
        asm volatile("global_load_dwordx4 %0, %1, %2 nt" : "=v"(dst[b]) : "v"(wlane), "s"(p + WU * b) : "memory");
    };
    auto stage_xi = [&](int c, int buf, int i) {
        const int slot = tid + NT * i, row = slot >> 5, pos = slot & 31, unit = pos ^ (row & 15);
        const E *src = A + (size_t)row * K + (size_t)c * GEMM_KC + 8 * unit;
        E *dst = &xs[buf][0][0] + (size_t)(NT * i + 64 * w) * 8;
        __builtin_amdgcn_global_load_lds((gptr_t)src, (lptr_t)dst, 16, 0, 0);
        asm volatile("" ::: "memory");
    };
    auto load_w = [&](u32x4 (&dst)[4], int c) {
#pragma unroll
        for (int b = 0; b < 4; b++) load_wb(dst, c, b);
    };
    auto stage_x = [&](int c, int buf) {
#pragma unroll
        for (int i = 0; i < XV; i++) stage_xi(c, buf, i);
    };
    auto phase = [&](u32x4 (&cur)[4], int c, int buf) {
        gemm_wait_younger<DEPTH, PC>(c1 - 1 - c);
        __builtin_amdgcn_s_barrier();
        asm volatile("" ::: "memory");
        const uint32_t xbase = lds_base + (uint32_t)buf * (R * GEMM_KC * 2) + (uint32_t)n * (GEMM_KC * 2);
#pragma unroll
        for (int b = 0; b < 4; b++) {
            const uint32_t a0 = xbase + (uint32_t)((8 * b + 2 * g) ^ n) * 16, a1 = xbase + (uint32_t)((8 * b + 2 * g + 1) ^ n) * 16;
            u32x4 r[RT][2];
            gemm_read_a2<RT>(r, a0, a1);
            asm volatile("" : "+v"(cur[b]) : : "memory");
            const auto lo = F8Widen<TT>::cvt(cur[b][0], cur[b][1]), hi = F8Widen<TT>::cvt(cur[b][2], cur[b][3]);
#pragma unroll
            for (int mt = 0; mt < RT; mt++) {
                acc[mt] = TT::mfma(__builtin_bit_cast(typename TT::vec8, r[mt][0]), lo, acc[mt]);
                acc[mt] = TT::mfma(__builtin_bit_cast(typename TT::vec8, r[mt][1]), hi, acc[mt]);
            }
            if (RT >= 3 && c + DEPTH < c1) {
                load_wb(cur, c + DEPTH, b);
                if (b < XV) stage_xi(c + DEPTH, buf == 0 ? NB - 1 : buf - 1, b);
            }
        }
        if (RT < 3 && c + DEPTH < c1) { load_w(cur, c + DEPTH); stage_x(c + DEPTH, buf == 0 ? NB - 1 : buf - 1); }
    };
    if (c0 < c1) {
#pragma unroll
        for (int d = 0; d < DEPTH; d++)
            if (c0 + d < c1) { load_w(wr[d], c0 + d); stage_x(c0 + d, d); }
        int buf = 0;
        for (int c = c0; c < c1; c += DEPTH) {
#pragma unroll
            for (int d = 0; d < DEPTH; d++)
                if (c + d < c1) { phase(wr[d], c + d, buf); buf = buf == NB - 1 ? 0 : buf + 1; }
        }
    }
#pragma unroll
    for (int mt = 0; mt < RT; mt++) {
#pragma unroll
        for (int r = 0; r < 4; r++) {
            const int m = 16 * mt + 4 * g + r;
            const float v = acc[mt][r] * sc;
            if (out) out[(size_t)m * N + n0 + n] = (E)v;
            else __hip_atomic_store(&partial[((size_t)split * R + m) * N + n0 + n], v, __ATOMIC_RELAXED, __HIP_MEMORY_SCOPE_AGENT);
        }
    }
}

__global__ __launch_bounds__(256) void k_gemm_pack_f8(const uint4 *__restrict__ W8, uint4 *__restrict__ out, int N, int K) {
    const long long u = (long long)blockIdx.x * 256 + threadIdx.x;
    const long long total = (long long)N * K / 16;
    if (u >= total) return;
    const int n_chunks = K / GEMM_KC;
    const long long blk = u >> 11;
    const int in = (int)(u & 2047), b = in >> 9, tid = in & 511, w = tid >> 6, g = (tid >> 4) & 3, n = tid & 15;
    const int t = (int)(blk / n_chunks), c = (int)(blk % n_chunks);
    const long long row = 128LL * t + 16 * w + n, col = 256LL * c + 64 * b + 16 * g;
    out[u] = W8[(row * K + col) / 16];
}

static constexpr int stream_lds(int depth, int rt) { return (depth + 1) * 16 * rt * GEMM_KC * 2; }

template <auto KERN, int LDS, typename... A>
static hipError_t stream_launch(dim3 grid, hipStream_t st, A... args) {
    if constexpr (LDS > 65536) {
        static unsigned long long done = 0ull;
        const hipError_t attr = samd_reserve_lds((const void *)KERN, LDS, &done);
        if (attr != hipSuccess) return attr;
    }
    hipLaunchKernelGGL(KERN, grid, dim3(64 * GEMM_WAVES), LDS, st, args...);
    return hipSuccess;
}

extern "C" {

int samd_gemm_pack_f8(const void *d_W8, void *d_out, int32_t N, int32_t K, void *stream) {
    if (!d_W8 || !d_out || d_W8 == d_out || N < GEMM_COLS || N % GEMM_COLS != 0 || K < GEMM_KC || K % GEMM_KC != 0) {
        samd_set_error("samd_gemm_pack_f8: needs N %% 128 == 0, K %% 256 == 0 and distinct buffers"); return SAMD_E_INVALID;
    }
    const long long units = (long long)N * K / 16;
    hipLaunchKernelGGL(k_gemm_pack_f8, dim3((unsigned)((units + 255) / 256)), dim3(256), 0, (hipStream_t)stream, (const uint4 *)d_W8, (uint4 *)d_out, N, K);
    LAUNCHCHK();
    return SAMD_OK;
}

int samd_gemm_skinny_f8(const void *d_A, const void *d_W8p, const float *d_scale, int32_t rows_pad, int32_t N, int32_t K, int32_t splits, float *d_partial,
                        void *d_out, int32_t dtype, void *stream) {
    if (!d_A || !d_W8p || !d_scale || (rows_pad != 16 && rows_pad != 32 && rows_pad != 48 && rows_pad != 64) || N < GEMM_COLS || N % GEMM_COLS != 0 ||
        K < GEMM_KC || K % GEMM_KC != 0 || splits < 1 || splits > K / GEMM_KC || (splits == 1 ? !d_out : !d_partial) || (dtype != SAMD_F16 && dtype != SAMD_BF16)) {
        samd_set_error("samd_gemm_skinny_f8: unsupported shape (rows 16/32/48/64, N %% 128 == 0, K %% 256 == 0) or null pointer"); return SAMD_E_INVALID;
    }
    const dim3 grid(N / GEMM_COLS, splits);
    const hipStream_t st = (hipStream_t)stream;
    float *part = splits == 1 ? nullptr : d_partial;
    void *out = splits == 1 ? d_out : nullptr;
#define GO(TT, RT, D) e = stream_launch<k_gemm_skinny_f8<TT, RT, D>, stream_lds(D, RT)>(grid, st, (const typename TT::elem *)d_A, (const unsigned char *)d_W8p, \
        d_scale, part, (typename TT::elem *)out, K, N, K / GEMM_KC, splits)
#define ROWS(TT) do { if (rows_pad == 16) GO(TT, 1, 4); else if (rows_pad == 32) GO(TT, 2, 4); else if (rows_pad == 48) GO(TT, 3, 4); else GO(TT, 4, 3); } while (0)
    hipError_t e;
    if (dtype == SAMD_F16) ROWS(GF16); else ROWS(GBF16);
#undef ROWS
#undef GO
    if (e != hipSuccess) { samd_set_error("samd_gemm_skinny_f8: %s", hipGetErrorString(e)); return SAMD_E_HIP; }
    LAUNCHCHK();
    return SAMD_OK;
}

}

template <typename TT> struct F4Widen;
template <> struct F4Widen<GF16> {
    static __device__ __forceinline__ half8 cvt(unsigned w, float s) {
        const auto a = __builtin_amdgcn_cvt_scalef32_pk_f16_fp4(w, s, 0), b = __builtin_amdgcn_cvt_scalef32_pk_f16_fp4(w, s, 1);
        const auto c = __builtin_amdgcn_cvt_scalef32_pk_f16_fp4(w, s, 2), d = __builtin_amdgcn_cvt_scalef32_pk_f16_fp4(w, s, 3);
        return __builtin_bit_cast(half8, (u32x4){__builtin_bit_cast(unsigned, a), __builtin_bit_cast(unsigned, b), __builtin_bit_cast(unsigned, c), __builtin_bit_cast(unsigned, d)});
    }
};
template <> struct F4Widen<GBF16> {
    static __device__ __forceinline__ bf16x8 cvt(unsigned w, float s) {
        const auto a = __builtin_amdgcn_cvt_scalef32_pk_bf16_fp4(w, s, 0), b = __builtin_amdgcn_cvt_scalef32_pk_bf16_fp4(w, s, 1);
        const auto c = __builtin_amdgcn_cvt_scalef32_pk_bf16_fp4(w, s, 2), d = __builtin_amdgcn_cvt_scalef32_pk_bf16_fp4(w, s, 3);
        return __builtin_bit_cast(bf16x8, (u32x4){__builtin_bit_cast(unsigned, a), __builtin_bit_cast(unsigned, b), __builtin_bit_cast(unsigned, c), __builtin_bit_cast(unsigned, d)});
    }
};

typedef unsigned u32x2 __attribute__((ext_vector_type(2)));
typedef _Float16 half2v __attribute__((ext_vector_type(2)));

template <typename TT> struct I4Widen;
template <> struct I4Widen<GF16> {
    struct G { half2v s, zb; };
    static __device__ __forceinline__ G group(u32x2 gd, int j) {
        const unsigned s = (gd[0] >> (16 * j)) & 0xffffu, z = (gd[1] >> (16 * j)) & 0xffffu;
        return {__builtin_bit_cast(half2v, s | (s << 16)), __builtin_bit_cast(half2v, z | (z << 16))};
    }
    static __device__ __forceinline__ half8 cvt(unsigned x, G g) {
        u32x4 r;
#pragma unroll
        for (int i = 0; i < 4; i++) {
            const half2v q = __builtin_bit_cast(half2v, ((x >> (4 * i)) & 0x000f000fu) | 0x64006400u);
            r[i] = __builtin_bit_cast(unsigned, (q - g.zb) * g.s);
        }
        return __builtin_bit_cast(half8, r);
    }
};
template <> struct I4Widen<GBF16> {
    struct G { float s, zb; };
    static __device__ __forceinline__ G group(u32x2 gd, int j) {
        return {__builtin_bit_cast(float, (gd[0] >> (16 * j)) << 16), __builtin_bit_cast(float, (gd[1] >> (16 * j)) << 16)};
    }
    static __device__ __forceinline__ bf16x8 cvt(unsigned x, G g) {
        u32x4 r;
#pragma unroll
        for (int i = 0; i < 4; i++) {
            const unsigned t = x >> (4 * i);
            const float lo = __builtin_bit_cast(float, ((t << 16) & 0x000f0000u) | 0x43000000u);
            const float hi = __builtin_bit_cast(float, (t & 0x000f0000u) | 0x43000000u);
            const float a = (lo - g.zb) * g.s, b = (hi - g.zb) * g.s;
            unsigned p;
            asm("v_cvt_pk_bf16_f32 %0, %1, %2" : "=v"(p) : "v"(a), "v"(b));
            r[i] = p;
        }
        return __builtin_bit_cast(bf16x8, r);
    }
};

enum { SIDE_DENSE, SIDE_EXPERT, SIDE_WIDE };

#define MOE_MAX_E 256
#define MOE_MAX_K 8
#define MOE_MAX_ROWS 64
#define MOE_WS_ACTIVE 16
#define MOE_WS_COUNT (MOE_WS_ACTIVE + MOE_MAX_E)
#define MOE_WS_LIST (MOE_WS_COUNT + MOE_MAX_E)
// ... 1733 lines not shown
```

sam-decoding_amd/samd_hip/engine.py:

```python
import ctypes as C
import os

import numpy as np
import torch

from . import (F32, MAX_DRAFT, REP_COUNTERS, REP_DMETA, REP_KVINDEX, REP_META, REP_TOKENS, REP_VERDICT, REPORT_INTS,
               Params, SamdError, Session, StaticAutomaton, TokenRecycleTable, require_gpu, torch_dtype_code)


class StepReport:
    __slots__ = ("type", "n", "n_leaves", "max_depth", "match_dyn", "match_static", "best", "accept", "next_token", "is_tree",
                 "tokens", "kv_index", "steps", "error")

    def __init__(self, r):
        d, v = r[REP_DMETA:REP_DMETA + 16], r[REP_VERDICT:REP_VERDICT + 8]
        self.type, self.n, self.n_leaves, self.max_depth = int(d[0]), int(d[1]), int(d[2]), int(d[3])
        self.match_dyn, self.match_static = int(d[5]), int(d[7])
        self.best, self.accept, self.next_token, self.is_tree = int(v[0]), int(v[1]), int(v[3]), int(v[5])
        self.tokens = r[REP_TOKENS:REP_TOKENS + self.accept].tolist()
        self.kv_index = r[REP_KVINDEX:REP_KVINDEX + self.accept].tolist()
        self.steps = int(r[REP_COUNTERS])
        self.error = int(r[REP_META + 9])


class ScriptedVerifier:

    def __init__(self, target, vocab, device="cuda", with_logits=False):
        require_gpu()
        self.vocab, self.device = int(vocab), torch.device(device)
        self.host_target = [int(t) for t in target]
        self.target = torch.tensor(self.host_target, dtype=torch.int32, device=self.device)
        self.argmax = torch.zeros(MAX_DRAFT, dtype=torch.int32, device=self.device)
        self.with_logits = with_logits
        self.logits = torch.zeros((MAX_DRAFT, self.vocab), dtype=torch.float32, device=self.device) if with_logits else None
        self._base = ((torch.arange(self.vocab, device=self.device, dtype=torch.int64) * 37)) if with_logits else None
        self.dtype = torch.float32

    def next_token(self, ctx):
        k = len(ctx)
        if k < len(self.host_target) and list(ctx) == self.host_target[:k]:
            return self.host_target[k]
        h = 1469598103
        for t in ctx[-3:]:
            h = (h * 1000003 + t + 7) % 2147483647
        return 3 + h % (self.vocab - 3)

    def _rows(self, n_rows):
        nt = self.argmax[:n_rows].to(torch.int64)
        v = self.vocab
        r = ((self._base[None, :] + 11 * nt[:, None]) % v).to(torch.float32) / float(v)
        idx = torch.arange(n_rows, device=self.device)
        r[idx, nt] += 8.0
        r[idx, (nt * 7 + 1) % v] += 3.0
        self.logits[:n_rows] = r

    def prefill(self, session, input_ids, on_chunk=None):
        ids = [int(t) for t in input_ids.reshape(-1).tolist()]
        n = len(ids)
        session.set_cache_length(n)
        if on_chunk is not None:
            if not self.with_logits:
                raise SamdError("ScriptedVerifier(with_logits=True) is required for Token Recycle")
            for c0 in range(0, n, MAX_DRAFT):
                m = min(MAX_DRAFT, n - c0)
                am = [self.next_token(ids[:c0 + i + 1]) for i in range(m)]
                self.argmax[:m] = torch.tensor(am, dtype=torch.int32, device=self.device)
                self._rows(m)
                on_chunk(torch.tensor(ids[c0:c0 + m] + [0] * (MAX_DRAFT - m), dtype=torch.int32, device=self.device), self.logits, m, None)
        first = torch.tensor([self.next_token(ids)], dtype=torch.int32, device=self.device)
        session.set_start_token(first)
        self._keep = first
        if not self.with_logits:
            return None
        self.argmax[:1] = first
        self._rows(1)
        return self.logits[0].clone()

    def forward_tokens(self, session, tokens, relpos, mask_rows, n, L):
        if not self.with_logits:
            raise SamdError("ScriptedVerifier(with_logits=True) is required for the granular decode()")
        session.set_cache_length(L)
        self.verify(session, MAX_DRAFT)
        return self.logits[:n].clone()

    def verify(self, session, R):
        session.scripted_argmax(self.target, len(self.host_target), self.vocab, self.argmax)
        if self.with_logits:
            self._rows(MAX_DRAFT)
        return dict(argmax=self.argmax, logits=self.logits)

    def compact(self, session):
        pass

    def bucket(self, n):
        return MAX_DRAFT


class ScriptedAcceptance:

    def __init__(self, runner, vocab, target_len, ranked_logits=False, order1_hot_vocab=0):
        self.runner, self.vocab, self.target_len = runner, int(vocab), int(target_len)
        self.ranked_logits = bool(ranked_logits)
        self.order1_hot_vocab = int(order1_hot_vocab)
        self.target = torch.zeros(self.target_len, dtype=torch.int32, device=runner.device)
        self.pf_mask = runner.pf_mask
        self._prompt_len = 0

    def set_target(self, target):
        t = torch.as_tensor(np.asarray(target, dtype=np.int32))[:self.target_len]
        self.target.zero_()
        self.target[:t.numel()] = t.to(self.target.device)

    def prefill(self, session, input_ids, on_chunk=None):
        last = self.runner.prefill(session, input_ids, on_chunk)
        n = input_ids.numel()
        session.set_start_token(self.target[n:n + 1])
        return last

    def verify(self, session, R):
        b = self.runner.verify(session, R)
        session.scripted_argmax(self.target, self.target_len, self.vocab, b["argmax"])
        if self.ranked_logits:
            if self.order1_hot_vocab > 0:
                session.scripted_logits(b["argmax"], b["logits"], self.order1_hot_vocab, order=1)
            else:
                session.scripted_logits(b["argmax"], b["logits"], self.vocab)
        return b

    def compact(self, session):
        self.runner.compact(session)

    def bucket(self, n):
        return self.runner.bucket(n)

    def warm(self, R):
        self.runner.warm(R)

    def hidden_rows(self, R):
        return self.runner.hidden_rows(R)


class _StopForward(Exception):
    """raised by the engine's layer hook to end a forward after its first launches (the eager head of a step)"""


class _GraphChain:

    def __init__(self, n, head=None):
        self.parts = [torch.cuda.CUDAGraph() for _ in range(n)]
        self.head = head

    def replay(self):
        if self.head is not None:
            self.head()
        for g in self.parts:
            g.replay()


class DecodeEngine:
    def __init__(self, verifier, session: Session, static: StaticAutomaton, params: Params, recycle: TokenRecycleTable = None,
                 recycle_parent=None, use_graphs=True):
        require_gpu()
        self.verifier, self.session, self.static, self.params = verifier, session, static, params
        self.recycle = recycle
        self.device = torch.device("cuda")
        if recycle is not None:
            self.tr_parent = torch.tensor(recycle_parent, dtype=torch.int32, device=self.device)
            self.tr_tokens = torch.zeros(MAX_DRAFT, dtype=torch.int32, device=self.device)
        self.report_buf = torch.zeros(REPORT_INTS, dtype=torch.int32).pin_memory()
        self._report_np = self.report_buf.numpy()
        self.use_graphs = use_graphs
        self._graphs = {}
        self.bucket_steps = {}
        self._views = session.device_views()
        self._n_ptr = self._views["dmeta"] + 4
        self._push = None
        if recycle is None and type(self) is DecodeEngine and os.environ.get("SAMD_REPORT_PUSH", "1") != "0":
            self._push = session.report_target()

    def _recycle_update(self, d_tokens, logits, n_rows, d_n):
        dt = F32 if logits.dtype == torch.float32 else torch_dtype_code(logits.dtype)
        self.recycle.update(d_tokens, logits, dt, n_rows, logits.shape[1], logits.stride(0), d_n)

    def _install_tree(self):
        self.recycle.draft(self._views["start_token"], self.tr_tokens)
        self.session.set_draft_if_deferred(self.tr_tokens, self.tr_parent, self.recycle.n_nodes, reverse=True)

    def _enqueue_step(self, R):
        b = self.verifier.verify(self.session, R)
        if self.recycle is not None:
            self._recycle_update(self._views["tokens"], b["logits"], min(R, MAX_DRAFT), C.c_void_p(self._n_ptr))
        self.session.step(self.static, self.params, b["argmax"])
        if self.recycle is not None:
            self._install_tree()
        self.verifier.compact(self.session)
        if self._push is None:
            self.session.report_async(self.report_buf)

    def _ingest_beside(self, ids, prefill):
        s = self.session
        cur = torch.cuda.current_stream()
        if os.environ.get("SAMD_INGEST_STREAM", "1") == "0":
            prefill()
            s.add_tokens(ids)
            s.static_walk(self.static, ids, ids.numel(), commit=True)
            return
        if getattr(self, "_side", None) is None:
            self._side = torch.cuda.Stream(device=self.device)
        self._side.wait_stream(cur)
        with torch.cuda.stream(self._side):
            s.add_tokens(ids)
            s.static_walk(self.static, ids, ids.numel(), commit=True)
        ids.record_stream(self._side)
        prefill()
        cur.wait_stream(self._side)

    def start(self, input_ids):
        s = self.session
        s.reset()
        on_chunk = None
        if self.recycle is not None:
            on_chunk = lambda toks, logits, n, hidden: self._recycle_update(toks, logits, n, None)
        ids = input_ids.reshape(-1).to(device=self.device, dtype=torch.int32)
        self._ingest_beside(ids, lambda: self.verifier.prefill(s, ids, on_chunk))
        s.draft(self.static, self.params, self._views["start_token"])
        if self.recycle is not None:
            self._install_tree()
        s.report_async(self.report_buf)
        torch.cuda.current_stream().synchronize()
        return StepReport(self._report_np)

    def step(self, n_next):
        R = self.verifier.bucket(n_next)
        self.bucket_steps[R] = self.bucket_steps.get(R, 0) + 1
        push = self._push
        g = None
        if self.use_graphs:
            g = self._graphs.get(R)
            if g is None:
                g = self._capture(R)
        if push is not None:
            last = int(push[0][REPORT_INTS])
        if g is None:
            self._enqueue_step(R)
        else:
            g.replay()
        if push is not None:
            from . import lib
            self._steps_since_query = getattr(self, "_steps_since_query", 0) + 1
            if self._steps_since_query >= 64:
                self._steps_since_query = 0
                torch.cuda.current_stream().query()
            if lib().samd_report_wait(push[1], last, 5_000_000) != 0:
                torch.cuda.current_stream().synchronize()
                if int(push[0][REPORT_INTS]) == last:
                    raise SamdError("the step kernel did not push its report")
            self._report_np[:] = push[0][:REPORT_INTS]
            return StepReport(self._report_np)
        torch.cuda.current_stream().synchronize()
        return StepReport(self._report_np)

    def supports_fused_sampling(self):
        return self.recycle is None and type(self) is DecodeEngine

    def start_sampled(self, input_ids):
        s = self.session
        s.reset()
        ids = input_ids.reshape(-1).to(device=self.device, dtype=torch.int32)
        last = []
        self._ingest_beside(ids, lambda: last.append(self.verifier.prefill(s, ids, None)))
        if last[0] is None:
            raise SamdError("this verifier does not expose logits; sampling needs them")
        sample_p = torch.softmax(last[0].reshape(1, -1).float(), dim=-1)
        self._start = self._draw(sample_p)
        s.set_start_token(self._start)
        s.draft(self.static, self.params, self._views["start_token"])
        s.report_async(self.report_buf)
        torch.cuda.current_stream().synchronize()
        return StepReport(self._report_np)

    def _draw(self, sample_p):
        self._rng_before_draw = torch.cuda.get_rng_state(self.device)
        return torch.multinomial(sample_p, 1).reshape(-1).to(torch.int32)

    def undo_pending_draw(self):
        state = getattr(self, "_rng_before_draw", None)
        if state is not None:
            torch.cuda.set_rng_state(state, self.device)
            self._rng_before_draw = None

    def step_sampled(self, rep, gen_config):
        import random
        s = self.session
        n, C_, D = rep.n, max(rep.n_leaves, 1), max(rep.max_depth, 1)
        R = self.verifier.bucket(n)
        self.bucket_steps[R] = self.bucket_steps.get(R, 0) + 1
        b = self.verifier.verify(s, R)
        node_logits = b["logits"][:n]
        V = node_logits.shape[-1]
        if getattr(self, "_samp", None) is None or self._samp["work"].dtype != node_logits.dtype or self._samp["work"].numel() != V:
            self._samp = dict(cand=torch.zeros(MAX_DRAFT * MAX_DRAFT, dtype=torch.int64, device=self.device),
                              rowmap=torch.zeros(MAX_DRAFT * MAX_DRAFT, dtype=torch.int32, device=self.device),
                              work=torch.empty(V, dtype=node_logits.dtype, device=self.device),
                              out=torch.zeros(5, dtype=torch.int32, device=self.device),
                              out_host=torch.zeros(5, dtype=torch.int32).pin_memory())
        t = self._samp
        s.candidates(t["cand"], t["rowmap"])
        probs = torch.softmax(gen_config.logits_processor(None, node_logits), dim=-1).contiguous()
        n_u = C_ * D + 8
        state = random.getstate()
        u = torch.from_numpy(np.asarray([random.random() for _ in range(n_u)], dtype=np.float64)).to(self.device)
        from . import _ptr, check, current_stream, lib
        check(lib().samd_posterior_sampled_nodes(_ptr(probs), torch_dtype_code(probs.dtype), _ptr(t["rowmap"]), n, _ptr(t["cand"]), C_, D, V,
                                                 _ptr(u), n_u, _ptr(t["work"]), _ptr(t["out"]), current_stream()))
        out = t["out"]
        cell = out[0].long() * D + out[1].long() - 1
        node = t["rowmap"][cell].long()
        node = torch.where((node < 0) | (node >= n), torch.full_like(node, n - 1), node)
        p_raw = torch.softmax(node_logits[node], dim=0)
        sample_p = torch.where(out[3] != 0, t["work"], p_raw)
        self._start = self._draw(sample_p.view(1, -1))
        s.step_given(self.static, self.params, out, self._start)
        self.verifier.compact(s)
        s.report_async(self.report_buf)
        t["out_host"].copy_(out, non_blocking=True)
        torch.cuda.current_stream().synchronize()
        used, status = int(t["out_host"][2]), int(t["out_host"][4])
        random.setstate(state)
        for _ in range(used):
            random.random()
        if status:
            raise SamdError("samd_posterior_sampled ran out of uniforms")
        return StepReport(self._report_np)

    def _capture(self, R):
        self._warm(R)
        torch.cuda.current_stream().synchronize()
        runner = getattr(self.verifier, "runner", self.verifier)
        cuts = [int(x) for x in os.environ.get("SAMD_GRAPH_SPLIT_LAYER", "2").split(",") if x.strip()]
        n_layers = len(getattr(runner, "w", {}).get("layers", ())) if hasattr(runner, "layer_hook") else 0
        eager = int(os.environ.get("SAMD_EAGER_HEAD_LAYERS", "0"))
        eager = eager if 0 < eager < n_layers else 0
        cuts = sorted({c for c in cuts if eager < c < n_layers})
        if not cuts and not eager:
            g = torch.cuda.CUDAGraph()
            with torch.cuda.graph(g):
                self._enqueue_step(R)
        else:
            def head():
                def stop(li):
                    if li >= eager:
                        raise _StopForward()
                runner.layer_hook = stop
                try:
                    self.verifier.verify(self.session, R)
                except _StopForward:
                    pass
                finally:
                    runner.layer_hook = None
            g = _GraphChain(len(cuts) + 1, head if eager else None)
            cur = torch.cuda.current_stream(self.device)
            side = torch.cuda.Stream(device=self.device)
            side.wait_stream(cur)
            with torch.cuda.stream(side):
                part = [0]
                started = [not eager]
                if not eager:
                    g.parts[0].capture_begin()

                def hook(li):
                    if not started[0]:
                        if li == eager:
                            g.parts[0].capture_begin()
                            started[0] = True
                        return
                    if li in cuts and part[0] < len(g.parts) - 1:
                        g.parts[part[0]].capture_end()
                        part[0] += 1
                        g.parts[part[0]].capture_begin()
                runner.layer_hook = hook
                try:
                    self._enqueue_step(R)
                except BaseException:
                    runner.layer_hook = None
                    try:
                        if started[0]:
                            g.parts[part[0]].capture_end()
                    except Exception:
                        pass
                    cur.wait_stream(side)
                    raise
                finally:
                    runner.layer_hook = None
                g.parts[part[0]].capture_end()
            cur.wait_stream(side)
        self._graphs[R] = g
        return g

    def _warm(self, R):
        v = self.verifier
        if hasattr(v, "warm"):
            v.warm(R)


class TreeModelEngine(DecodeEngine):

    def __init__(self, verifier, session, static, params, tree_model, use_graphs=True):
        super().__init__(verifier, session, static, params, use_graphs=use_graphs)
        self.tm = tree_model

    def _report(self):
        self.session.report_async(self.report_buf)
        torch.cuda.current_stream().synchronize()
        return StepReport(self._report_np)

    def _maybe_tree(self, rep, start_token=None):
        if rep.type != 2:
            return rep
        if start_token is None:
            start_token = self.session.read_draft().tokens[0]
        start = torch.tensor([start_token], dtype=torch.long, device=self.device)
        tokens, parents = self.tm.gen_draft_device(start)
        return self._install(rep, tokens, parents)

    def _install(self, rep, tokens, parents):
        self._keep = (tokens.to(torch.int32).contiguous(), parents.to(torch.int32).contiguous())
        self.session.set_draft(self._keep[0], self._keep[1], int(tokens.numel()), type_=1)
        if os.environ.get("SAMD_TREE_REPORT_SYNC", "0") == "1":
            return self._report()
        rep.type, rep.n, rep.n_leaves, rep.max_depth = 1, int(tokens.numel()), -1, -1
        return rep

    def start(self, input_ids):
        s = self.session
        s.reset()
        self.tm.reset()
        ids = input_ids.reshape(-1).to(device=self.device, dtype=torch.int32)
        hidden = []
        self._ingest_beside(ids, lambda: self.verifier.prefill(s, ids, lambda toks, logits, n, h: hidden.append(h[:n].clone())))
        self.tm.update(tokens=ids.to(torch.long), last_hidden_states=torch.cat(hidden, dim=0))
        s.draft(self.static, self.params, self._views["start_token"])
        return self._maybe_tree(self._report())

    def step(self, n_next):
        R = self.verifier.bucket(n_next)
        self.bucket_steps[R] = self.bucket_steps.get(R, 0) + 1
        if not self.use_graphs:
            self._enqueue_step(R)
        else:
            g = self._graphs.get(R) or self._capture(R)
            g.replay()
        torch.cuda.current_stream().synchronize()
        rep = StepReport(self._report_np)
        fast = getattr(self.tm, "gen_draft_from_step", None)
        if rep.type == 2 and fast is not None:
            out = fast(self.verifier.hidden_rows(R), self._views, rep.accept, n_next)
            if out is not None:
                return self._install(rep, *out)
        rows = [k if k >= 0 else n_next - 1 for k in rep.kv_index]
        hs = self.verifier.hidden_rows(R)[torch.tensor(rows, dtype=torch.long, device=self.device)]
        self.tm.update(tokens=torch.tensor(rep.tokens, dtype=torch.long, device=self.device), last_hidden_states=hs)
        return self._maybe_tree(rep, rep.next_token)
```

sam-decoding_amd/samd_hip/llama.py:

```python
import ctypes as C
import math
import os

import torch

from . import (F16, BF16, MAX_DRAFT, TILE_ROWS, QkvEpilogue, SamdError, Session, Warm, _ptr, check, current_stream, lib, require_gpu,
               torch_dtype_code)
from . import fp8 as F8
from . import mxfp4 as MX
from . import int4 as I4
from . import int8 as I8
from . import moe as MOE


def _env_weight_format(weight_format):
    return weight_format if weight_format is not None else (os.environ.get("SAMD_WEIGHT_FORMAT") or None)


def _weight_format(weight_format, weights, dtype):
    has_i8 = any(k + "_z8" in l for l in weights["layers"] for k in I8.PROJECTIONS)
    has_f8b = any(k + "_sinv" in l for l in weights["layers"] for k in F8.PROJECTIONS)
    has_f8 = any(l[k].dtype == torch.float8_e4m3fn and k + "_sinv" not in l for l in weights["layers"] for k in F8.PROJECTIONS if k in l)
    has_i4 = any(k + "_z" in l for l in weights["layers"] for k in I4.PROJECTIONS)
    has_f4 = any(_is_f4_tensor(l[k]) and k + "_z" not in l and k + "_z8" not in l for l in weights["layers"] for k in MX.PROJECTIONS if k in l)
    names = {torch.float16: ("fp16", "float16", "half"), torch.bfloat16: ("bf16", "bfloat16")}.get(dtype, ())
    if weight_format is None:
        fmt = "fp8" if has_f8 else ("fp8b128" if has_f8b else ("mxfp4" if has_f4 else ("int4g128" if has_i4 else ("int8g128" if has_i8 else None))))
    elif weight_format in ("fp8", "fp8b128", "mxfp4", "int4g128", "int8g128"):
        fmt = weight_format
    elif weight_format == dtype or (isinstance(weight_format, str) and weight_format.lower() in names):
        fmt = None
    else:
        hint = " (the AWQ / GPTQ format is spelled 'int4g128': 4-bit codes in groups of 128, the only group size the kernel has)" \
            if weight_format == "int4" else ""
        raise SamdError(f"weight_format {weight_format!r}: expected None, 'fp8', 'mxfp4', 'int4g128', 'fp8b128' or the model dtype ({dtype}), or 'int8g128'{hint}")
    if has_f8 and fmt != "fp8":
        raise SamdError(f"the weights carry float8_e4m3fn projections; weight_format {weight_format!r} would need them dequantised (pass None or 'fp8')")
    if has_f8b and fmt != "fp8b128":
        raise SamdError(f"the weights carry block-scaled FP8 projections; weight_format {weight_format!r} would need them dequantised (pass None or 'fp8b128')")
    if has_f4 and fmt != "mxfp4":
        raise SamdError(f"the weights carry MXFP4 projections; weight_format {weight_format!r} would need them dequantised (pass None or 'mxfp4')")
    if has_i4 and fmt != "int4g128":
        raise SamdError(f"the weights carry INT4 (AWQ / GPTQ) projections; weight_format {weight_format!r} would need them dequantised (pass None or 'int4g128')")
    if has_i8 and fmt != "int8g128":
        raise SamdError(f"the weights carry INT8 (GPTQ) projections; weight_format {weight_format!r} would need them dequantised (pass None or 'int8g128')")
    return fmt


QUANT_FORMATS = ("fp8", "fp8b128", "mxfp4", "int4g128", "int8g128")


def quant_prefill_min_rows(default):
    raw = os.environ.get("SAMD_QUANT_PREFILL_MIN_ROWS")
    if raw is None or raw.strip() == "":
        return int(default)
    try:
        rows = int(raw.strip())
    except ValueError:
        raise SamdError(f"SAMD_QUANT_PREFILL_MIN_ROWS={raw!r}: expected an integer number of prompt rows (a multiple of 64, >= 128)") from None
    if rows < 2 * TILE_ROWS or rows % TILE_ROWS != 0:
        raise SamdError(f"SAMD_QUANT_PREFILL_MIN_ROWS={rows}: must be a multiple of 64 and >= 128")
    return rows


def _is_f4_tensor(t):
    return t.dtype == torch.uint8 or MX.is_fp4_dtype(t.dtype)


def _cfg_get(cfg, name, default=None):
    if isinstance(cfg, dict):
        return cfg.get(name, default)
    return getattr(cfg, name, default)


class LlamaShape:

    def __init__(self, cfg, qkv_bias=None, qk_norm=None):
        self.hidden = int(_cfg_get(cfg, "hidden_size"))
        self.inter = int(_cfg_get(cfg, "intermediate_size"))
        self.layers = int(_cfg_get(cfg, "num_hidden_layers"))
        self.heads = int(_cfg_get(cfg, "num_attention_heads"))
        kv = _cfg_get(cfg, "num_key_value_heads")
        self.kv_heads = int(kv) if kv is not None else self.heads
        hd = _cfg_get(cfg, "head_dim")
        self.head_dim = int(hd) if hd else self.hidden // self.heads
        self.vocab = int(_cfg_get(cfg, "vocab_size"))
        self.eps = float(_cfg_get(cfg, "rms_norm_eps", 1e-6))
        self.max_pos = int(_cfg_get(cfg, "max_position_embeddings", 2048))
        rp = _cfg_get(cfg, "rope_parameters") or _cfg_get(cfg, "rope_scaling") or {}
        theta = _cfg_get(cfg, "rope_theta")
        if theta is None and isinstance(rp, dict):
            theta = rp.get("rope_theta")
        self.rope_theta = float(theta if theta is not None else 10000.0)
        self.rope_scaling = dict(rp) if isinstance(rp, dict) else {}
        if self.head_dim != 128:
            raise SamdError("the gfx950 tree-attention kernel is specialised for head_dim 128 (Vicuna-7B / Llama-3-8B)")
        self.model_type = str(_cfg_get(cfg, "model_type", None) or "llama")
        layer_types = _cfg_get(cfg, "layer_types", None) or ()
        if _cfg_get(cfg, "use_sliding_window", False) or any(t != "full_attention" for t in layer_types):
            raise SamdError("sliding-window attention layers are not supported (use_sliding_window / layer_types)")
        if _cfg_get(cfg, "attention_bias", False):
            raise SamdError("attention_bias=True puts a bias on o_proj, which the runner does not support (q|k|v biases alone are)")
        if _cfg_get(cfg, "mlp_bias", False):
            raise SamdError("MLP projection biases (mlp_bias=True) are not supported")
        self.qkv_bias = (self.model_type == "qwen2") if qkv_bias is None else bool(qkv_bias)
        self.qk_norm = (self.model_type in ("qwen3", "qwen3_moe")) if qk_norm is None else bool(qk_norm)
        self.n_experts = self.top_k = self.moe_inter = 0
        self.norm_topk = False
        self.sparse = [False] * self.layers
        if self.model_type == "qwen3_moe":
            self.n_experts = int(_cfg_get(cfg, "num_experts", 0) or 0)
            self.top_k = int(_cfg_get(cfg, "num_experts_per_tok", 0) or 0)
            self.moe_inter = int(_cfg_get(cfg, "moe_intermediate_size", 0) or 0)
            self.norm_topk = bool(_cfg_get(cfg, "norm_topk_prob", False))
            self.sparse = MOE.sparse_layer_map(self.layers, self.n_experts, _cfg_get(cfg, "mlp_only_layers"), _cfg_get(cfg, "decoder_sparse_step", 1))
        self.moe = any(self.sparse)
        if self.moe:
            MOE.check_shape(self.hidden, self.moe_inter, self.n_experts, self.top_k)

    def inv_freq(self):
        d = self.head_dim
        inv = 1.0 / (self.rope_theta ** (torch.arange(0, d, 2, dtype=torch.float64) / d))
        rs = self.rope_scaling
        kind = rs.get("rope_type", rs.get("type", "default")) if rs else "default"
        if kind == "llama3":
            factor, lo, hi = rs["factor"], rs["low_freq_factor"], rs["high_freq_factor"]
            old = rs["original_max_position_embeddings"]
            wavelen = 2 * math.pi / inv
            scaled = torch.where(wavelen > old / lo, inv / factor, inv)
            smooth = (old / wavelen - lo) / (hi - lo)
            mid = (1 - smooth) * inv / factor + smooth * inv
            is_mid = (wavelen <= old / lo) & (wavelen >= old / hi)
            inv = torch.where(is_mid, mid, scaled)
        elif kind == "linear":
            inv = inv / rs["factor"]
        elif kind not in ("default", None):
            raise SamdError(f"unsupported rope scaling '{kind}'")
        return inv


class LlamaRunner:

    BUCKETS = (1, 8, 16, 32, 48, 64, 128)

    def __init__(self, shape, weights, max_cache_len, dtype=torch.float16, device="cuda", kv=None, native_gemm=True, packed_lm_head=None,
                 attention=None, weight_format=None, draft_head=False, expert_format=MOE.AUTO):
        sparse_l = [l for l in weights["layers"] if "experts_gu" in l]
        experts_i8 = [any(k in l for k in ("experts_gu_z8", "experts_gu_s8", "experts_down_z8", "experts_down_s8")) for l in sparse_l]
        experts_i4 = [any(k in l for k in ("experts_gu_z", "experts_gu_s", "experts_down_z", "experts_down_s")) for l in sparse_l]
        experts_f8 = [any(k in l for k in ("experts_gu_sinv", "experts_down_sinv")) or F8.is_fp8_dtype(l["experts_gu"].dtype)
                      or F8.is_fp8_dtype(l["experts_down"].dtype) for l in sparse_l]
        experts4 = [not i4e and not f8e and not i8e and (MOE.is_4bit(l["experts_gu"]) or MOE.is_4bit(l["experts_down"]))
                    for l, i4e, f8e, i8e in zip(sparse_l, experts_i4, experts_f8, experts_i8)]
        self.expert_format = MOE.resolve_expert_format(expert_format, any(experts4), shape.moe, carries_int4=any(experts_i4),
                                                       carries_fp8=any(experts_f8), carries_int8=any(experts_i8))
        if shape.moe:
            MOE.reject_unsupported(_weight_format(weight_format, weights, dtype), native_gemm, draft_head)
        if any(experts4):
            if not all(experts4):
                raise SamdError(f"a mix of 4-bit and model-dtype sparse layers ({sum(experts4)} of {len(experts4)} carry MXFP4 experts): "
                                "the runner takes the experts of all sparse layers in one format")
            for i, l in enumerate(weights["layers"]):
                if "experts_gu" in l:
                    MOE.check_quantised_experts(l["experts_gu"], l.get("experts_gu_scale"), l["experts_down"], l.get("experts_down_scale"), dtype,
                                                f"layer {i} experts")
        if any(experts_i4):
            if not all(experts_i4):
                raise SamdError(f"a mix of INT4 and other sparse layers ({sum(experts_i4)} of {len(experts_i4)} carry INT4 experts): "
                                "the runner takes the experts of all sparse layers in one format")
            for i, l in enumerate(weights["layers"]):
                if "experts_gu" in l:
                    MOE.check_int4_experts((l["experts_gu"], l.get("experts_gu_z"), l.get("experts_gu_s")),
                                           (l["experts_down"], l.get("experts_down_z"), l.get("experts_down_s")), dtype, f"layer {i} experts")
        if any(experts_i8):
            if not all(experts_i8):
                raise SamdError(f"a mix of INT8 and other sparse layers ({sum(experts_i8)} of {len(experts_i8)} carry INT8 experts): "
                                "the runner takes the experts of all sparse layers in one format")
            for i, l in enumerate(weights["layers"]):
                if "experts_gu" in l:
                    MOE.check_int8_experts((l["experts_gu"], l.get("experts_gu_z8"), l.get("experts_gu_s8")),
                                           (l["experts_down"], l.get("experts_down_z8"), l.get("experts_down_s8")), dtype, f"layer {i} experts")
        if any(experts_f8):
            if not all(experts_f8):
                raise SamdError(f"a mix of block-scaled FP8 and other sparse layers ({sum(experts_f8)} of {len(experts_f8)} carry FP8 experts): "
                                "the runner takes the experts of all sparse layers in one format")
            for i, l in enumerate(weights["layers"]):
                if "experts_gu" in l:
                    MOE.check_fp8_experts((l["experts_gu"], l.get("experts_gu_sinv")), (l["experts_down"], l.get("experts_down_sinv")),
                                          f"layer {i} experts")
        self.draft_head = bool(draft_head)
        require_gpu()
        self.shape, self.dtype, self.device = shape, dtype, torch.device(device)
        self.dt = torch_dtype_code(dtype)
        if self.dt not in (F16, BF16):
            raise SamdError("LlamaRunner computes in fp16 or bf16")
        self.weight_format = _weight_format(weight_format, weights, dtype)
        f8, f4, i4 = self.weight_format == "fp8", self.weight_format == "mxfp4", self.weight_format == "int4g128"
        f8b = self.weight_format == "fp8b128"
        i8 = self.weight_format == "int8g128"
        quant = f8 or f4 or i4 or f8b or i8
        if i8 and not native_gemm:
            raise SamdError("INT8 projections exist only in the streaming kernel's packed form: native_gemm=False is not available with weight_format 'int8g128'")
        if f8b and not native_gemm:
            raise SamdError("FP8 projections exist only in the streaming kernel's packed form: native_gemm=False is not available with weight_format 'fp8b128'")
        if f8b:
            if shape.inter % 128 != 0:
                raise SamdError(f"block-scaled FP8 projection wgu: intermediate_size {shape.inter} is not a multiple of 128, so a 128 x 128 block "
                                "would straddle gate and up")
            for li, l in enumerate(weights["layers"]):
                for k in F8.PROJECTIONS:
                    N, K = l[k].shape
                    if N % 128 != 0 or K % 256 != 0:
                        raise SamdError(f"block-scaled FP8 projection {k} of layer {li}, shape ({N}, {K}): the kernel needs N % 128 == 0 and K % 256 == 0")
        if f8 and not native_gemm:
            raise SamdError("FP8 projections exist only in the streaming kernel's packed form: native_gemm=False is not available with weight_format 'fp8'")
        if f4 and not native_gemm:
            raise SamdError("MXFP4 projections exist only in the streaming kernel's packed form: native_gemm=False is not available with weight_format 'mxfp4'")
        if i4 and not native_gemm:
            raise SamdError("INT4 projections exist only in the streaming kernel's packed form: native_gemm=False is not available with weight_format 'int4g128'")
        s = shape
        self.w = weights
        streams = lambda t: bool(native_gemm) and t.shape[0] % 128 == 0 and t.shape[1] % 256 == 0
        self.native_gemm_max_rows = int(os.environ.get("SAMD_NATIVE_GEMM_MAX_ROWS", 64))
        moe = shape.moe
        self.route_log = None
        if quant or moe:
            self.native_gemm_max_rows = TILE_ROWS
        self.layer_hook = None
        self.warm_kb = int(os.environ.get("SAMD_L2_WARM_KB", 0))
        self.warm_delay = int(os.environ.get("SAMD_L2_WARM_DELAY", 0))
        self.warm_where = int(os.environ.get("SAMD_L2_WARM_WHERE", 0))
        self.attention = attention or os.environ.get("SAMD_ATTENTION", "split")
        if self.attention not in ("split", "split2", "split3", "block"):
            raise SamdError(f"unknown attention mode '{self.attention}'")
        self.qkv_epilogue = bool(s.qkv_bias or s.qk_norm)
        if self.qkv_epilogue and self.attention not in ("split", "split3"):
            raise SamdError(f"attention mode '{self.attention}' rotates q / k inside its own kernel, which has no q|k|v bias or q / k norm: "
                            f"use 'split' or 'split3' for this model")
        self.v_layout_t = self.attention == "block" or (self.attention in ("split", "split3") and s.head_dim == 128
                                                        and os.environ.get("SAMD_V_LAYOUT", "t") != "rows")
        self.v_transposed = self.v_layout_t
        def pack(t):
            if not streams(t):
                return None
            out = torch.empty_like(t)
            check(lib().samd_gemm_pack_weights(_ptr(t), _ptr(out), t.shape[0], t.shape[1], current_stream()))
            return out
        def pack_gate_up(t):
            if s.inter % 16 != 0 or not streams(t):
                return None
            gate, up = t[:s.inter].view(s.inter // 16, 16, -1), t[s.inter:].view(s.inter // 16, 16, -1)
            w = torch.stack([gate, up], dim=1).reshape(2 * s.inter, -1).contiguous()
            out = torch.empty_like(w)
            check(lib().samd_gemm_pack_groups(_ptr(w), _ptr(out), 2 * s.inter, w.shape[1], current_stream()))
            return out
        def pack_qkv64(t):
            heads_total = s.heads + 2 * s.kv_heads
            mode = os.environ.get("SAMD_QKV_FUSED", "1")
            n_cols = heads_total * 128
            enough = n_cols // 64 >= 128 or (n_cols % 48 == 0 and n_cols // 48 >= 128)
            if (not streams(t) or self.attention != "split" or (not enough and mode != "force") or s.head_dim != 128 or mode == "0"
                    or self.qkv_epilogue):
                return None
            out = torch.empty_like(t)
            check(lib().samd_gemm_pack_qkv64(_ptr(t), _ptr(out), heads_total, t.shape[1], current_stream()))
            return out
        def pack_groups(t, fold):
            if not fold or t.shape[0] % 16 != 0 or t.shape[1] % 256 != 0:
                return None
            out = torch.empty_like(t)
            check(lib().samd_gemm_pack_groups(_ptr(t), _ptr(out), t.shape[0], t.shape[1], current_stream()))
            return out
        def pack_f8(l, k):
            t = l[k]
            N, K = t.shape
            if N % 128 != 0 or K % 256 != 0:
                raise SamdError(f"FP8 projection {k} of shape {tuple(t.shape)}: the FP8 kernel needs N % 128 == 0 and K % 256 == 0")
            if t.dtype == torch.float8_e4m3fn:
                q, scale = t.to(self.device).contiguous(), l.pop(k + "_scale").to(device=self.device, dtype=torch.float32).contiguous()
            else:
                q, scale = F8.quantize_rows(t)
            l[k] = torch.empty(t.shape, dtype=torch.float8_e4m3fn, device="meta")
            del t
            out = torch.empty_like(q)
            check(lib().samd_gemm_pack_f8(_ptr(q), _ptr(out), N, K, current_stream()))
            return out, scale
        def pack_f8b(l, k):
            t = l[k]
            N, K = t.shape
            if t.dtype == torch.float8_e4m3fn:
                q, sinv = t.to(self.device).contiguous(), l.pop(k + "_sinv").to(device=self.device).contiguous()
                F8.check_block_scales(q, sinv, f"block-scaled FP8 projection {k}")
            else:
                q, sinv = F8.quantize_blocks(t)
            l[k] = torch.empty(t.shape, dtype=torch.float8_e4m3fn, device="meta")
            del t
            out = torch.empty_like(q)
            check(lib().samd_gemm_pack_f8(_ptr(q), _ptr(out), N, K, current_stream()))
            return out, sinv
        def pack_f4(l, k):
            t = l[k]
            N, K = (t.shape[0], 2 * t.shape[1]) if _is_f4_tensor(t) else t.shape
            if N % 128 != 0 or K % 256 != 0:
                raise SamdError(f"MXFP4 projection {k} of shape ({N}, {K}): the MXFP4 kernel needs N % 128 == 0 and K % 256 == 0")
            if _is_f4_tensor(t):
                q, e8 = MX.fuse_mxfp4([(t, l.pop(k + "_e8"))], self.device)
                if tuple(e8.shape) != (N, K // 32):
                    raise SamdError(f"MXFP4 projection {k}: block scales of shape {tuple(e8.shape)} for a ({N}, {K}) matrix")
                MX.check_exponents(e8, dtype, f"MXFP4 projection {k}")
            else:
                q, e8 = MX.quantize_blocks(t, dtype)
            l[k] = torch.empty((N, K), dtype=torch.uint8, device="meta")
            del t
            out = torch.empty(MX.packed_bytes(N, K), dtype=torch.uint8, device=self.device)
            check(lib().samd_gemm_pack_f4(_ptr(q), _ptr(e8), _ptr(out), N, K, current_stream()))
            return out
        def pack_i4(l, k):
            t = l[k]
            if k + "_z" in l:
                q, z, sc = I4.fuse_int4([(t, l.pop(k + "_z"), l.pop(k + "_s"))], self.device, dtype)
            else:
                if t.shape[0] % 128 != 0 or t.shape[1] % 256 != 0:
                    raise SamdError(f"INT4 projection {k} of shape {tuple(t.shape)}: the INT4 kernel needs N % 128 == 0 and K % 256 == 0")
                q, z, sc = I4.quantize_groups(t, dtype)
            I4.check_groups(q, z, sc, dtype, k)
            N, K = q.shape[0], 2 * q.shape[1]
            l[k] = torch.empty((N, K), dtype=torch.uint8, device="meta")
            del t
            out = torch.empty(I4.packed_bytes(N, K), dtype=torch.uint8, device=self.device)
            check(lib().samd_gemm_pack_i4(_ptr(q), _ptr(z), _ptr(sc), _ptr(out), N, K, self.dt, current_stream()))
            return out
        def pack_i8(l, k):
            t = l[k]
            if k + "_z8" in l:
                q, z, sc = I8.fuse_int8([(t, l.pop(k + "_z8"), l.pop(k + "_s8"))], self.device, dtype)
            else:
                if t.shape[0] % 128 != 0 or t.shape[1] % 256 != 0:
                    raise SamdError(f"INT8 projection {k} of shape {tuple(t.shape)}: the INT8 kernel needs N % 128 == 0 and K % 256 == 0")
                q, z, sc = I8.quantize_groups(t, dtype)
            I8.check_groups(q, z, sc, dtype, k)
            N, K = q.shape
            l[k] = torch.empty((N, K), dtype=torch.uint8, device="meta")
            del t
            out = torch.empty(I8.packed_bytes(N, K), dtype=torch.uint8, device=self.device)
            check(lib().samd_gemm_pack_i8(_ptr(q), _ptr(z), _ptr(sc), _ptr(out), N, K, self.dt, current_stream()))
            return out
        layers = []
        for l in weights["layers"]:
            if i8:
                lp = dict(wqkv=None, wqkv64=None, wo=None, wo_g=None, wgu=None, wdown=None, wdown_g=None)
                for k in I8.PROJECTIONS:
                    lp[k + "_i8"] = pack_i8(l, k)
                layers.append(lp)
                continue
            if i4:
                lp = dict(wqkv=None, wqkv64=None, wo=None, wo_g=None, wgu=None, wdown=None, wdown_g=None)
                for k in I4.PROJECTIONS:
                    lp[k + "_i4"] = pack_i4(l, k)
                layers.append(lp)
                continue
            if f4:
                lp = dict(wqkv=None, wqkv64=None, wo=None, wo_g=None, wgu=None, wdown=None, wdown_g=None)
                for k in MX.PROJECTIONS:
                    lp[k + "_f4"] = pack_f4(l, k)
                layers.append(lp)
                continue
            if f8:
                lp = dict(wqkv=None, wqkv64=None, wo=None, wo_g=None, wgu=None, wdown=None, wdown_g=None)
                for k in F8.PROJECTIONS:
                    lp[k + "_f8"] = pack_f8(l, k)
                layers.append(lp)
                continue
            if f8b:
                lp = dict(wqkv=None, wqkv64=None, wo=None, wo_g=None, wgu=None, wdown=None, wdown_g=None)
                for k in F8.PROJECTIONS:
                    lp[k + "_f8b"] = pack_f8b(l, k)
                layers.append(lp)
                continue
            sparse = "experts_gu" in l
            lp = dict(wgu=None if sparse else pack_gate_up(l["wgu"]), wqkv64=pack_qkv64(l["wqkv"]))
            lp["wqkv"] = pack(l["wqkv"]) if lp["wqkv64"] is None else None
            fold = (lp["wqkv64"] is not None and lp["wgu"] is not None and s.hidden <= 8192 and os.environ.get("SAMD_NORM_FOLD", "1") != "0"
                    and not moe)
            if sparse:
                gu_cols = s.hidden // 2 if MOE.is_4bit(l["experts_gu"]) and "experts_gu_sinv" not in l and "experts_gu_z8" not in l else s.hidden
                if tuple(l["router"].shape) != (s.n_experts, s.hidden) or tuple(l["experts_gu"].shape) != (s.n_experts, 2 * s.moe_inter, gu_cols):
                    raise SamdError(f"sparse layer weights of shapes {tuple(l['router'].shape)}, {tuple(l['experts_gu'].shape)} do not match the shape")
                if self.expert_format == "mxfp4":
                    ekeys = ("experts_gu", "experts_gu_scale", "experts_down", "experts_down_scale")
                    if MOE.is_4bit(l["experts_gu"]):
                        quad = tuple(MX._bytes(l[k]).to(self.device).contiguous() for k in ekeys)
                    else:
                        quad = MOE.quantize_experts(l["experts_gu"], l["experts_down"], dtype, f"layer {len(layers)} experts")
                    lp["moe_gu"], lp["moe_down"] = MOE.pack_experts_mxfp4(*quad)
                    for k, t in zip(ekeys, quad):
                        l[k] = torch.empty(t.shape, dtype=torch.uint8, device="meta")
                    del quad
                elif self.expert_format == "int4g128":
                    gkeys, dkeys = ("experts_gu", "experts_gu_z", "experts_gu_s"), ("experts_down", "experts_down_z", "experts_down_s")
                    if "experts_gu_z" in l:
                        gu3, dn3 = (tuple(l[k].to(self.device).contiguous() for k in ks) for ks in (gkeys, dkeys))
                    else:
                        gu3, dn3 = MOE.quantize_experts_int4(l["experts_gu"], l["experts_down"], dtype, f"layer {len(layers)} experts")
                    lp["moe_gu"], lp["moe_down"] = MOE.pack_experts_int4(gu3, dn3, dtype)
                    for k, t in zip(gkeys + dkeys, gu3 + dn3):
                        l[k] = torch.empty(t.shape, dtype=t.dtype, device="meta")
                    del gu3, dn3
                elif self.expert_format == "int8g128":
                    gkeys, dkeys = ("experts_gu", "experts_gu_z8", "experts_gu_s8"), ("experts_down", "experts_down_z8", "experts_down_s8")
                    if "experts_gu_z8" in l:
                        gu3, dn3 = (tuple(l[k].to(self.device).contiguous() for k in ks) for ks in (gkeys, dkeys))
                    else:
                        gu3, dn3 = MOE.quantize_experts_int8(l["experts_gu"], l["experts_down"], dtype, f"layer {len(layers)} experts")
                    lp["moe_gu"], lp["moe_down"] = MOE.pack_experts_int8(gu3, dn3, dtype)
                    for k, t in zip(gkeys + dkeys, gu3 + dn3):
                        l[k] = torch.empty(t.shape, dtype=t.dtype, device="meta")
                    del gu3, dn3
                elif self.expert_format == "fp8b128":
                    gkeys, dkeys = ("experts_gu", "experts_gu_sinv"), ("experts_down", "experts_down_sinv")
                    if "experts_gu_sinv" in l:
                        gu2, dn2 = (tuple(l[k].to(self.device).contiguous() for k in ks) for ks in (gkeys, dkeys))
                    else:
                        gu2, dn2 = MOE.quantize_experts_fp8(l["experts_gu"], l["experts_down"], f"layer {len(layers)} experts")
                    lp["moe_gu"], lp["moe_down"] = MOE.pack_experts_fp8(gu2, dn2)
                    for k, t in zip(gkeys + dkeys, gu2 + dn2):
                        l[k] = torch.empty(t.shape, dtype=torch.float8_e4m3fn if t.dtype == torch.uint8 else t.dtype, device="meta")
                    del gu2, dn2
                else:
                    lp["moe_gu"], lp["moe_down"] = MOE.pack_experts(l["experts_gu"], l["experts_down"])
                    for k in ("experts_gu", "experts_down"):
                        l[k] = torch.empty(l[k].shape, dtype=l[k].dtype, device="meta")
                lp["wo_g"], lp["wdown_g"], lp["wdown"] = pack_groups(l["wo"], fold), None, None
                lp["wo"] = pack(l["wo"])
                layers.append(lp)
                continue
            lp["wo_g"], lp["wdown_g"] = pack_groups(l["wo"], fold), pack_groups(l["wdown"], fold)
            both = os.environ.get("SAMD_GEMM_ONE_COPY", "0") != "1"
            for k in ("wo", "wdown"):
                gm_ok = lp[k + "_g"] is not None and l[k].shape[0] % 128 == 0
                lp[k] = pack(l[k]) if (both or not gm_ok) else None
            layers.append(lp)
        self.wp = dict(lm_head=packed_lm_head if packed_lm_head is not None else pack(weights["lm_head"]), layers=layers)
        self.native_gemm = self.wp["lm_head"] is not None or any(v is not None for l in self.wp["layers"] for v in l.values())
        if not self.native_gemm:
            self.wp = None
        self.fused_mlp = self.wp is not None and all(l["wgu"] is not None for l in self.wp["layers"] if "moe_gu" not in l)
# ... 274 lines not shown
                    l.weight.data = cat[r:r + n]
                    r += n
                shared[0] += 1
            return cat
        for lyr in m.layers:
            a, f = lyr.self_attn, lyr.mlp
            extra = {}
            if qkv_bias:
                extra["bqkv"] = get(torch.cat([a.q_proj.bias, a.k_proj.bias, a.v_proj.bias]))
            if qk_norm:
                extra["q_norm"], extra["k_norm"] = get(a.q_norm.weight), get(a.k_norm.weight)
            if ckpt_i4:
                lw = {}
                for k, names in (("wqkv", ("q_proj", "k_proj", "v_proj")), ("wo", ("o_proj",)), ("wgu", ("gate_proj", "up_proj")), ("wdown", ("down_proj",))):
                    own = a if k in ("wqkv", "wo") else f
                    lw[k], lw[k + "_z"], lw[k + "_s"] = I4.fuse_int4(
                        [I4.linear_int4(getattr(own, x), f"layers.{len(layers)}.{x}", config=qcfg) for x in names], dev, dtype)
                layers.append(dict(lw, ln1=get(lyr.input_layernorm.weight), ln2=get(lyr.post_attention_layernorm.weight), **extra))
                continue
            if ckpt_i8:
                lw = {}
                for k, names in (("wqkv", ("q_proj", "k_proj", "v_proj")), ("wo", ("o_proj",)), ("wgu", ("gate_proj", "up_proj")), ("wdown", ("down_proj",))):
                    own = a if k in ("wqkv", "wo") else f
                    lw[k], lw[k + "_z8"], lw[k + "_s8"] = I8.fuse_int8(
                        [I8.linear_int8(getattr(own, x), f"layers.{len(layers)}.{x}", config=qcfg) for x in names], dev, dtype)
                layers.append(dict(lw, ln1=get(lyr.input_layernorm.weight), ln2=get(lyr.post_attention_layernorm.weight), **extra))
                continue
            if ckpt_f4:
                lw = {}
                for k, lins in (("wqkv", (a.q_proj, a.k_proj, a.v_proj)), ("wo", (a.o_proj,)), ("wgu", (f.gate_proj, f.up_proj)), ("wdown", (f.down_proj,))):
                    lw[k], lw[k + "_e8"] = MX.fuse_mxfp4([MX.linear_mxfp4(x) for x in lins], dev)
                layers.append(dict(lw, ln1=get(lyr.input_layernorm.weight), ln2=get(lyr.post_attention_layernorm.weight), **extra))
                continue
            if ckpt_f8b:
                lw, li = {}, len(layers)
                for k, own, names in (("wqkv", a, ("q_proj", "k_proj", "v_proj")), ("wo", a, ("o_proj",)), ("wgu", f, ("gate_proj", "up_proj")),
                                      ("wdown", f, ("down_proj",))):
                    full = [f"layers.{li}.{'self_attn' if own is a else 'mlp'}.{x}" for x in names]
                    lw[k], lw[k + "_sinv"] = F8.fuse_fp8_blocks([F8.linear_fp8_block(getattr(own, x), n, qcfg8) for x, n in zip(names, full)], dev, full)
                layers.append(dict(lw, ln1=get(lyr.input_layernorm.weight), ln2=get(lyr.post_attention_layernorm.weight), **extra))
                continue
            if ckpt_f8:
                lw = {}
                for k, lins in (("wqkv", (a.q_proj, a.k_proj, a.v_proj)), ("wo", (a.o_proj,)), ("wgu", (f.gate_proj, f.up_proj)), ("wdown", (f.down_proj,))):
                    lw[k], lw[k + "_scale"] = F8.fuse_fp8([F8.linear_fp8(x) for x in lins], dev)
                layers.append(dict(lw, ln1=get(lyr.input_layernorm.weight), ln2=get(lyr.post_attention_layernorm.weight), **extra))
                continue
            li = len(layers)
            qkv_names, o_name = [f"layers.{li}.self_attn.{x}" for x in ("q_proj", "k_proj", "v_proj")], f"layers.{li}.self_attn.o_proj"
            if sparse[li] and any(experts_f8):
                layers.append(dict(
                    wqkv=fuse((a.q_proj, a.k_proj, a.v_proj), qkv_names), wo=get(lin_w(a.o_proj, o_name)), router=get(f.gate.weight),
                    **MOE.import_experts_fp8(f.experts, f"layers.{li}.mlp.experts", dev, qcfg8),
                    ln1=get(lyr.input_layernorm.weight), ln2=get(lyr.post_attention_layernorm.weight), **extra))
                continue
            if sparse[li] and any(experts_i4):
                layers.append(dict(
                    wqkv=fuse((a.q_proj, a.k_proj, a.v_proj), qkv_names), wo=get(lin_w(a.o_proj, o_name)), router=get(f.gate.weight),
                    **MOE.import_experts_int4(f.experts, f"layers.{li}.mlp.experts", dtype, dev, qcfg),
                    ln1=get(lyr.input_layernorm.weight), ln2=get(lyr.post_attention_layernorm.weight), **extra))
                continue
            if sparse[li] and moe_i8:
                layers.append(dict(
                    wqkv=fuse((a.q_proj, a.k_proj, a.v_proj), qkv_names), wo=get(lin_w(a.o_proj, o_name)), router=get(f.gate.weight),
                    **MOE.import_experts_int8(f.experts, f"layers.{li}.mlp.experts", dtype, dev, qcfg),
                    ln1=get(lyr.input_layernorm.weight), ln2=get(lyr.post_attention_layernorm.weight), **extra))
                continue
            if sparse[len(layers)] and any(experts4):
                ex, raw = f.experts, lambda t: MX._bytes(t.detach()).to(dev).contiguous()
                layers.append(dict(
                    wqkv=fuse((a.q_proj, a.k_proj, a.v_proj), qkv_names), wo=get(lin_w(a.o_proj, o_name)), router=get(f.gate.weight),
                    experts_gu=raw(ex.gate_up_proj), experts_gu_scale=raw(ex.gate_up_proj_scale),
                    experts_down=raw(ex.down_proj), experts_down_scale=raw(ex.down_proj_scale),
                    ln1=get(lyr.input_layernorm.weight), ln2=get(lyr.post_attention_layernorm.weight), **extra))
                continue
            if sparse[len(layers)]:
                layers.append(dict(
                    wqkv=fuse((a.q_proj, a.k_proj, a.v_proj), qkv_names), wo=get(lin_w(a.o_proj, o_name)), router=get(f.gate.weight),
                    experts_gu=get(f.experts.gate_up_proj), experts_down=get(f.experts.down_proj),
                    ln1=get(lyr.input_layernorm.weight), ln2=get(lyr.post_attention_layernorm.weight), **extra))
                continue
            layers.append(dict(
                wqkv=fuse((a.q_proj, a.k_proj, a.v_proj), qkv_names),
                wo=get(lin_w(a.o_proj, o_name)),
                wgu=fuse((f.gate_proj, f.up_proj), [f"layers.{li}.mlp.gate_proj", f"layers.{li}.mlp.up_proj"]),
                wdown=get(lin_w(f.down_proj, f"layers.{li}.mlp.down_proj")),
                ln1=get(lyr.input_layernorm.weight), ln2=get(lyr.post_attention_layernorm.weight), **extra))
        weights = dict(embed=get(m.embed_tokens.weight), layers=layers, norm=get(m.norm.weight), lm_head=get(lm.lm_head.weight))
        if shared[0]:
            import logging
            logging.getLogger("samd_hip").info("LlamaRunner.from_hf: %d fused projection groups now back the HF module's q/k/v and gate/up "
                                               "weights (share_weights); its parameters are views of the runner's matrices", shared[0])
        return cls(shape, weights, max_cache_len, dtype, device, weight_format=weight_format, expert_format=expert_format, **kw)

    @classmethod
    def _hf_experts_are_4bit(cls, lyr, i):
        ex = lyr.mlp.experts
        gu, dn = MOE.is_4bit(ex.gate_up_proj), MOE.is_4bit(ex.down_proj)
        if gu != dn:
            raise SamdError(f"layers.{i}.mlp.experts: gate_up_proj is {ex.gate_up_proj.dtype} and down_proj {ex.down_proj.dtype}; "
                            "4-bit experts need both tensors 4-bit")
        return gu

    @classmethod
    def _hf_experts_are_fp8(cls, lyr, i):
        ex = getattr(getattr(lyr, "mlp", None), "experts", None)
        if ex is None:
            return False
        if hasattr(ex, "gate_up_proj"):
            kinds = [(f"layers.{i}.mlp.experts.{p}", F8.is_fp8_dtype(getattr(ex, p).dtype)) for p in ("gate_up_proj", "down_proj")
                     if getattr(ex, p, None) is not None]
        elif hasattr(ex, "__len__") and hasattr(ex, "__getitem__"):
            kinds = [(f"layers.{i}.mlp.experts.{e}.{p}", F8.is_fp8_dtype(getattr(ex[e], p).weight.dtype))
                     for e in range(len(ex)) for p in MOE.INT4_EXPERT_PROJECTIONS if getattr(getattr(ex[e], p, None), "weight", None) is not None]
        else:
            return False
        n8 = sum(k for _, k in kinds)
        if 0 < n8 < len(kinds):
            plain = [n for n, k in kinds if not k][:3]
            raise SamdError(f"layers.{i}.mlp.experts: a mix of FP8 and other expert tensors ({n8} of {len(kinds)} are FP8; e.g. "
                            f"{', '.join(plain)} are not): FP8 experts need every expert tensor float8_e4m3fn")
        return n8 > 0

    @classmethod
    def _hf_experts_are_int8(cls, lyr, config=None):
        ex = getattr(getattr(lyr, "mlp", None), "experts", None)
        if ex is None or hasattr(ex, "gate_up_proj") or not hasattr(ex, "__len__") or not hasattr(ex, "__getitem__") or len(ex) == 0:
            return False
        return all(I8.is_int8_module(getattr(ex[e], p, None), config) for e in range(len(ex)) for p in MOE.INT4_EXPERT_PROJECTIONS)

    @classmethod
    def _hf_experts_are_int4(cls, lyr, i):
        ex = getattr(getattr(lyr, "mlp", None), "experts", None)
        if ex is None or hasattr(ex, "gate_up_proj") or not hasattr(ex, "__len__") or not hasattr(ex, "__getitem__"):
            return False
        kinds = [(f"layers.{i}.mlp.experts.{e}.{p}", I4.is_int4_module(getattr(ex[e], p, None)))
                 for e in range(len(ex)) for p in MOE.INT4_EXPERT_PROJECTIONS]
        n4 = sum(k for _, k in kinds)
        if 0 < n4 < len(kinds):
            plain = [n for n, k in kinds if not k][:3]
            raise SamdError(f"layers.{i}.mlp.experts: a mix of INT4 and other expert projections ({n4} of {len(kinds)} are INT4; e.g. "
                            f"{', '.join(plain)} are not): INT4 experts need gate_proj, up_proj and down_proj of every expert INT4")
        return n4 > 0

    _LAYER_PARAMS = ("self_attn.q_proj.weight", "self_attn.k_proj.weight", "self_attn.v_proj.weight", "self_attn.o_proj.weight",
                     "mlp.gate_proj.weight", "mlp.up_proj.weight", "mlp.down_proj.weight", "input_layernorm.weight", "post_attention_layernorm.weight")
    _QKV_BIAS = ("self_attn.q_proj.bias", "self_attn.k_proj.bias", "self_attn.v_proj.bias")
    _QK_NORM = ("self_attn.q_norm.weight", "self_attn.k_norm.weight")

    @classmethod
    def _hf_layer_extras(cls, layers):
        if len(layers) == 0:
            raise SamdError("the model has no decoder layers")
        def names_of(lyr, i):
            skip = {f"{n[:-len('.weight')]}.{sc}" for n, p in lyr.named_parameters()
                    if n.endswith(".weight") and (F8.is_fp8_dtype(p.dtype) or _is_f4_tensor(p))
                    for sc in ("weight_scale", "input_scale", "weight_scale_inv")}
            params = dict(lyr.named_parameters())
            for n, mod in lyr.named_modules():
                if n and I4.is_int4_module(mod):
                    for own in list(params):
                        if own.startswith(n + "."):
                            del params[own]
                    params[n + ".weight"] = None
                    if getattr(mod, "bias", None) is not None:
                        params[n + ".bias"] = None
            if any(MOE.is_4bit(params.get(n)) for n in MOE.SPARSE_MLP_PARAMS[1:]):
                skip |= set(MOE.EXPERT_SCALE_PARAMS)
            if cls._hf_experts_are_fp8(lyr, i):
                skip |= set(MOE.FP8_EXPERT_SCALE_PARAMS)
                if not hasattr(lyr.mlp.experts, "gate_up_proj"):
                    for e in range(len(lyr.mlp.experts)):
                        for pn in MOE.INT4_EXPERT_PROJECTIONS:
                            params.pop(f"mlp.experts.{e}.{pn}.weight", None)
                    params.update({n: None for n in MOE.SPARSE_MLP_PARAMS[1:]})
            if cls._hf_experts_are_int4(lyr, i):
                for e in range(len(lyr.mlp.experts)):
                    for pn in MOE.INT4_EXPERT_PROJECTIONS:
                        params.pop(f"mlp.experts.{e}.{pn}.weight", None)
                params.update({n: None for n in MOE.SPARSE_MLP_PARAMS[1:]})
            return set(params) - skip
        names0 = names_of(layers[0], 0)
        qkv_bias = any(n in names0 for n in cls._QKV_BIAS)
        qk_norm = any(n in names0 for n in cls._QK_NORM)
        want = set(cls._LAYER_PARAMS) | (set(cls._QKV_BIAS) if qkv_bias else set()) | (set(cls._QK_NORM) if qk_norm else set())
        want_sparse = (want - set(MOE.DENSE_MLP_PARAMS)) | set(MOE.SPARSE_MLP_PARAMS)
        for i, lyr in enumerate(layers):
            names = names_of(lyr, i)
            if names == want:
                continue
            if any(n.startswith("mlp.experts.") or n == "mlp.gate.weight" for n in names):
                if names == want_sparse:
                    continue
                if any("shared_expert" in n for n in names):
                    raise SamdError(f"layer {i}: a shared expert is not supported (parameters {sorted(n for n in names if 'shared_expert' in n)})")
                raise SamdError(f"layer {i}: sparse MLP parameters the runner does not consume {sorted(names - want_sparse)}, or lacks "
                                f"{sorted(want_sparse - names)} (it reads mlp.gate.weight and the fused mlp.experts.gate_up_proj / down_proj)")
            extra, missing = sorted(names - want), sorted(want - names)
            if "self_attn.o_proj.bias" in extra:
                raise SamdError(f"layer {i}: o_proj bias is not supported (q|k|v biases are)")
            if any(n.startswith("mlp.") and n.endswith(".bias") for n in extra):
                raise SamdError(f"layer {i}: MLP projection biases are not supported")
            raise SamdError(f"layer {i}: parameters the runner does not consume {extra}, or lacks {missing} "
                            f"(it reads the Llama layer, q|k|v biases (Qwen2) and q / k norm weights (Qwen3))")
        return qkv_bias, qk_norm

    @classmethod
    def _hf_sparse_layers(cls, layers):
        return [any(n.startswith("mlp.experts.") for n, _ in lyr.named_parameters()) or cls._hf_experts_are_int4(lyr, i)
                for i, lyr in enumerate(layers)]

    @classmethod
    def random_init(cls, cfg, max_cache_len, dtype=torch.float16, device="cuda", seed=0, std=0.02, weight_format=None, expert_format=MOE.AUTO, **kw):
        require_gpu()
        shape = LlamaShape(cfg)
        MOE.resolve_expert_format(expert_format, False, shape.moe)
        g = torch.Generator(device=device).manual_seed(seed)

        def rnd(*size):
            return (torch.randn(size, generator=g, device=device, dtype=torch.float32) * std).to(dtype)
        s = shape
        qkv_out = (s.heads + 2 * s.kv_heads) * s.head_dim
        if s.moe:
            MOE.reject_unsupported(_env_weight_format(weight_format), kw.get("native_gemm", True), kw.get("draft_head", False))

        def mlp(i):
            if s.sparse[i]:
                return dict(router=rnd(s.n_experts, s.hidden), experts_gu=rnd(s.n_experts, 2 * s.moe_inter, s.hidden),
                            experts_down=rnd(s.n_experts, s.hidden, s.moe_inter))
            return dict(wgu=rnd(2 * s.inter, s.hidden), wdown=rnd(s.hidden, s.inter))
        layers = [dict(wqkv=rnd(qkv_out, s.hidden), wo=rnd(s.hidden, s.heads * s.head_dim), **mlp(i),
                       ln1=torch.ones(s.hidden, dtype=dtype, device=device),
                       ln2=torch.ones(s.hidden, dtype=dtype, device=device)) for i in range(s.layers)]

        def norm_w():
            mag = 0.5 + 1.5 * torch.rand(s.head_dim, generator=g, device=device)
            sign = torch.where(torch.rand(s.head_dim, generator=g, device=device) < 0.5, -1.0, 1.0)
            return (mag * sign).to(dtype)
        for l in layers:
            if s.qkv_bias:
                l["bqkv"] = (torch.randn(qkv_out, generator=g, device=device, dtype=torch.float32) * 0.5).to(dtype)
            if s.qk_norm:
                l["q_norm"], l["k_norm"] = norm_w(), norm_w()
        weights = dict(embed=rnd(s.vocab, s.hidden), layers=layers, norm=torch.ones(s.hidden, dtype=dtype, device=device),
                       lm_head=rnd(s.vocab, s.hidden))
        return cls(shape, weights, max_cache_len, dtype, device, weight_format=_env_weight_format(weight_format), expert_format=expert_format, **kw)

    def weight_bytes(self, experts=None):
        n_act = self.shape.top_k if experts is None else int(experts)
        nb = lambda t: t.numel() * t.element_size() if t.dim() != 3 else t[0].numel() * t.element_size() * min(n_act, t.shape[0])
        n = nb(self.w["lm_head"]) + nb(self.w["norm"])
        if self.weight_format in ("mxfp4", "int4g128", "int8g128"):
            sfx = {"mxfp4": "_f4", "int4g128": "_i4", "int8g128": "_i8"}[self.weight_format]
            for l, lp in zip(self.w["layers"], self.wp["layers"]):
                n += sum(nb(t) for k, t in l.items() if k not in MX.PROJECTIONS) + sum(nb(lp[k + sfx]) for k in MX.PROJECTIONS)
            return n
        for l in self.w["layers"]:
            n += sum(nb(t) for t in l.values())
        if self.expert_format == "int8g128":
            n += sum(nb(l[k]) for l in self.w["layers"] for k in ("experts_gu_z8", "experts_down_z8") if k in l)
        if self.weight_format == "fp8":
            n += sum(nb(l[k + "_f8"][1]) for l in self.wp["layers"] for k in F8.PROJECTIONS)
        if self.weight_format == "fp8b128":
            n += sum(nb(l[k + "_f8b"][1]) for l in self.wp["layers"] for k in F8.PROJECTIONS)
        return n

    def _rows_pad(self, R):
        return max(R, 16) if self.native_gemm else R

    def _buffers(self, R):
        if R not in self._buf:
            s, dt, dev = self.shape, self.dtype, self.device
            RP = self._rows_pad(R)
            z = lambda r, *sz: torch.zeros((max(r, RP),) + sz, dtype=dt, device=dev)
            ws_bytes = max(lib().samd_tree_attention_workspace(R, s.heads, s.head_dim), lib().samd_tree_attention_rope_workspace(R, s.heads, s.head_dim))
            part_elems = 0
            if self.native_gemm:
                qkv_out = (s.heads + 2 * s.kv_heads) * s.head_dim
                for n, k in ((qkv_out, s.hidden), (s.hidden, s.heads * s.head_dim), (2 * s.inter, s.hidden), (s.hidden, s.inter)):
                    if RP <= self.native_gemm_max_rows:
                        part_elems = max(part_elems, lib().samd_gemm_splits(n, k, RP) * RP * n)
            self._buf[R] = dict(x=z(R, s.hidden), h=z(R, s.hidden), qkv=z(R, (s.heads + 2 * s.kv_heads) * s.head_dim),
                                q=z(R, s.heads, s.head_dim), attn=z(R, s.heads, s.head_dim), o=z(R, s.hidden),
                                gu=z(R, 2 * s.inter), act=z(R, s.inter), d=z(R, s.hidden), logits=z(R, s.vocab),
                                argmax=torch.zeros(MAX_DRAFT, dtype=torch.int32, device=dev), rows_pad=RP,
                                part=torch.zeros(max(part_elems, 1), dtype=torch.float32, device=dev),
                                ws=torch.zeros(ws_bytes, dtype=torch.uint8, device=dev), ws_bytes=ws_bytes,
                                cs=torch.zeros((MAX_DRAFT, s.head_dim), dtype=torch.float32, device=dev),
                                ssq=torch.zeros((max(s.hidden // 16, 1), 16), dtype=torch.float32, device=dev))
            if s.moe:
                self._buf[R]["moe"] = MOE.MoeBuffers(RP, s.hidden, s.moe_inter, s.n_experts, s.top_k, dt, self.dt, dev)
        return self._buf[R]

    def max_draft_rows(self):
        wide_ok = (not self.row_major_released) and self.attention in ("split", "split3") and not getattr(self, "draft_head", False)
        return MAX_DRAFT if wide_ok else min(MAX_DRAFT, 64)

    def bucket(self, n):
        for b in self.BUCKETS:
            if n <= b:
                return b
        raise SamdError(f"draft of {n} nodes exceeds {MAX_DRAFT}")

    def forward_rows(self, R, d_tokens, d_relpos, d_mask, d_L, d_n, x_in=None, d_vis=None, _span=None):
        if self.shape.moe:
            MOE.reject_unsupported(draft_head=getattr(self, "draft_head", False))
        if self._rows_pad(R) > self.native_gemm_max_rows and self.row_major_released:
            raise SamdError(f"a {R}-row forward needs the row-major projection matrices (released: SAMD_RELEASE_ROW_MAJOR / release_row_major()); "
                            f"drafts above {self.native_gemm_max_rows} nodes and the library-GEMM path are unavailable on this runner")
        L, s, b, dt, st = lib(), self.shape, (self._buffers(R) if _span is None else _span.b), self.dt, current_stream()
        RP, part = b["rows_pad"], b["part"]
        resumed = _span is not None and _span.first > 0
        if (_span is None and self.norm_fold and RP == 16 and x_in is None and d_vis is None and not getattr(self, "draft_head", False)
                and RP <= self.native_gemm_max_rows):
            return self._forward_rows_fold(R, b, d_tokens, d_relpos, d_mask, d_L, d_n)

        def hint(w, wp, fused=False, is_head=False):
            if wp is None or RP > self.native_gemm_max_rows or self.warm_kb <= 0:
                return None
            n, k = w.shape
            sp = 1 if (fused or is_head) else L.samd_gemm_splits(n, k, RP)
            return C.byref(Warm(wp.data_ptr(), n, k, sp, self.warm_kb, self.warm_delay, self.warm_where))

        def gemm(a, w, wp, out, wg=None, f8=None, f4=None, i4=None, f8b=None, i8=None):
            n, k = w.shape
            if i8 is not None:
                sp = L.samd_gemm_splits(n, k, RP)
                check(L.samd_gemm_skinny_i8(_ptr(a), _ptr(i8), RP, n, k, sp, _ptr(part), _ptr(out), dt, st))
                return (out, 0, 0) if sp == 1 else (part, sp, RP * n)
            if i4 is not None:
                sp = L.samd_gemm_splits(n, k, RP)
                check(L.samd_gemm_skinny_i4(_ptr(a), _ptr(i4), RP, n, k, sp, _ptr(part), _ptr(out), dt, st))
                return (out, 0, 0) if sp == 1 else (part, sp, RP * n)
            if f4 is not None:
                sp = L.samd_gemm_splits(n, k, RP)
                check(L.samd_gemm_skinny_f4(_ptr(a), _ptr(f4), RP, n, k, sp, _ptr(part), _ptr(out), dt, st))
                return (out, 0, 0) if sp == 1 else (part, sp, RP * n)
            if f8b is not None:
                sp = L.samd_gemm_splits(n, k, RP)
                check(L.samd_gemm_skinny_f8b(_ptr(a), _ptr(f8b[0]), _ptr(f8b[1]), RP, n, k, sp, _ptr(part), _ptr(out), dt, st))
                return (out, 0, 0) if sp == 1 else (part, sp, RP * n)
            if f8 is not None:
                sp = L.samd_gemm_splits(n, k, RP)
                check(L.samd_gemm_skinny_f8(_ptr(a), _ptr(f8[0]), _ptr(f8[1]), RP, n, k, sp, _ptr(part), _ptr(out), dt, st))
                return (out, 0, 0) if sp == 1 else (part, sp, RP * n)
            if (wp is None and wg is None) or RP > self.native_gemm_max_rows:
                torch.mm(a[:R], w.t(), out=out[:R])
                return out, 0, 0
            sp = L.samd_gemm_splits(n, k, RP) if out is not b["logits"] else 1
            if wp is not None and os.environ.get("SAMD_GEMM_PREFER_GROUPS", "0") != "1":
                check(L.samd_gemm_skinny(_ptr(a), _ptr(wp), RP, n, k, sp, _ptr(part), _ptr(out), dt, st))
            else:
                check(L.samd_gemm_skinny_groups(_ptr(a), _ptr(wg if wg is not None else wp), RP, n, k, sp, _ptr(part), _ptr(out), dt, st))
            return (out, 0, 0) if sp == 1 else (part, sp, RP * n)

        if resumed:
            pass
        elif x_in is None:
            check(L.samd_embed_rows(_ptr(d_tokens), _ptr(self.w["embed"]), _ptr(b["x"]), R, s.hidden, s.vocab, dt, st))
        else:
            rows_in = min(R, x_in.shape[0])
            if x_in.data_ptr() != b["x"].data_ptr():
                b["x"][:rows_in].copy_(x_in[:rows_in])
        head = getattr(self, "draft_head", False)
        log_routes = s.moe and self.route_log is not None and not torch.cuda.is_current_stream_capturing()
        block = self.attention == "block"
        vt = self.v_transposed and not block
        if self.attention != "split3" and not resumed:
            check(L.samd_rope_rows(_ptr(d_relpos), _ptr(d_vis if d_vis is not None else d_L), _ptr(self.cos), _ptr(self.sin), _ptr(b["cs"]), R,
                                   s.head_dim, self.rope_rows, st))
        if d_vis is not None and not block:
            raise SamdError("a visible length different from the write position needs attention mode 'block'")
        delta, dn, dstride = (None if _span is None else _span.delta), 0, 0
        packed = self.wp["layers"] if self.wp else [{}] * len(self.w["layers"])
        for li, w in enumerate(self.w["layers"]):
            if _span is not None and li < _span.first:
                continue
            if self.layer_hook is not None:
                self.layer_hook(li)
            wp = packed[li]
            raw_in = head and li == 0
            if not raw_in:
                check(L.samd_rmsnorm_warm(_ptr(b["x"]), _ptr(delta), _ptr(w["ln1"]), _ptr(b["h"]), R, s.hidden, s.eps, dt, dn, dstride,
                                          hint(w["wqkv"], wp.get("wqkv")), st))
            fused_qkv = wp.get("wqkv64") is not None and self.attention == "split" and RP <= self.native_gemm_max_rows and d_vis is None
            if fused_qkv:
                check((L.samd_gemm_qkv_rope_vt if vt else L.samd_gemm_qkv_rope)(
                    _ptr(b["x"] if raw_in else b["h"]), _ptr(wp["wqkv64"]), RP, s.hidden, _ptr(b["cs"]), _ptr(d_L), _ptr(d_n),
                    _ptr(b["q"]), _ptr(self.kv[li, 0]), _ptr(self.kv[li, 1]), s.heads, s.kv_heads, s.head_dim, self.max_len, dt, st))
            else:
                src, n_p, stride = gemm(b["x"] if raw_in else b["h"], w["wqkv"], wp.get("wqkv"), b["qkv"], f8=wp.get("wqkv_f8"), f8b=wp.get("wqkv_f8b"), f4=wp.get("wqkv_f4"), i4=wp.get("wqkv_i4"), i8=wp.get("wqkv_i8"))
            if block:
                check(L.samd_attention_block(_ptr(src), n_p, stride, _ptr(b["cs"]), _ptr(self.kv[li, 0]), _ptr(self.kv[li, 1]), _ptr(b["attn"]), dt, R,
                                             s.heads, s.kv_heads, s.head_dim, self.max_len, _ptr(d_mask), _ptr(d_L), _ptr(d_vis), _ptr(d_n), self.scale, st))
            elif self.attention == "split2":
                check(L.samd_tree_attention_rope(_ptr(src), n_p, stride, _ptr(b["cs"]), _ptr(self.kv[li, 0]), _ptr(self.kv[li, 1]), _ptr(b["attn"]), dt, R,
                                                 s.heads, s.kv_heads, s.head_dim, self.max_len, _ptr(d_mask), _ptr(d_L), _ptr(d_n), self.scale,
                                                 _ptr(b["ws"]), b["ws_bytes"], st))
            else:
                if fused_qkv:
                    pass
                elif self.epi is not None:
                    cs_form = self.attention == "split"
                    check(L.samd_rope_kv_write_epi(
                        _ptr(src), _ptr(d_relpos), _ptr(d_L), _ptr(d_n), None if cs_form else _ptr(self.cos), None if cs_form else _ptr(self.sin),
                        _ptr(b["cs"]) if cs_form else None, _ptr(b["q"]), _ptr(self.kv[li, 0]), _ptr(self.kv[li, 1]), int(vt), R, s.heads,
                        s.kv_heads, s.head_dim, self.max_len, self.rope_rows, dt, n_p, stride, C.byref(self.epi[li]), st))
                elif self.attention == "split":
                    check((L.samd_rope_kv_write_cs_vt if vt else L.samd_rope_kv_write_cs)(
                        _ptr(src), _ptr(d_relpos), _ptr(d_L), _ptr(d_n), _ptr(b["cs"]), _ptr(b["q"]), _ptr(self.kv[li, 0]),
                        _ptr(self.kv[li, 1]), R, s.heads, s.kv_heads, s.head_dim, self.max_len, dt, n_p, stride, st))
                else:
                    check((L.samd_rope_kv_write_vt if vt else L.samd_rope_kv_write)(
                        _ptr(src), _ptr(d_relpos), _ptr(d_L), _ptr(d_n), _ptr(self.cos), _ptr(self.sin),
                        _ptr(b["q"]), _ptr(self.kv[li, 0]), _ptr(self.kv[li, 1]), R, s.heads, s.kv_heads,
                        s.head_dim, self.max_len, self.rope_rows, dt, n_p, stride, st))
                check((L.samd_tree_attention_vt if vt else L.samd_tree_attention_warm)(
                    _ptr(b["q"]), _ptr(self.kv[li, 0]), _ptr(self.kv[li, 1]), _ptr(b["attn"]), dt, R, s.heads,
                    s.kv_heads, s.head_dim, self.max_len, _ptr(d_mask), _ptr(d_L), _ptr(d_n), self.scale,
                    _ptr(b["ws"]), b["ws_bytes"], hint(w["wo"], wp.get("wo")), st))
            src, n_p, stride = gemm(b["attn"].view(b["attn"].shape[0], -1), w["wo"], wp.get("wo"), b["o"], wg=wp.get("wo_g"), f8=wp.get("wo_f8"), f8b=wp.get("wo_f8b"), f4=wp.get("wo_f4"), i4=wp.get("wo_i4"), i8=wp.get("wo_i8"))
            check(L.samd_rmsnorm_warm(_ptr(b["x"]), _ptr(src), _ptr(w["ln2"]), _ptr(b["h"]), R, s.hidden, s.eps, dt, n_p, stride,
                                      None, st))
            if "moe_gu" in wp:
                if _span is not None:
                    return b, li
                mb = b["moe"]
                mb.route(b["h"], w["router"], d_n, s.norm_topk)
                if log_routes:
                    idx = mb.topk_idx.clone()
                    self.route_log.append((li, int((idx[:, 0] >= 0).sum()), idx, mb.topk_w.clone()))
                delta, dn, dstride = mb.experts(b["h"], wp["moe_gu"], wp["moe_down"], d_n, self.expert_format), 0, 0
                continue
            if wp.get("wgu") is not None and RP <= self.native_gemm_max_rows:
                check(L.samd_gemm_pairs_silu(_ptr(b["h"]), _ptr(wp["wgu"]), RP, s.inter, s.hidden, _ptr(b["act"]), dt, st))
            else:
                src, n_p, stride = gemm(b["h"], w["wgu"], None, b["gu"], f8=wp.get("wgu_f8"), f8b=wp.get("wgu_f8b"), f4=wp.get("wgu_f4"), i4=wp.get("wgu_i4"), i8=wp.get("wgu_i8"))
                check(L.samd_silu_mul(_ptr(src), _ptr(b["act"]), R, s.inter, dt, n_p, stride, st))
            delta, dn, dstride = gemm(b["act"], w["wdown"], wp.get("wdown"), b["d"], wg=wp.get("wdown_g"), f8=wp.get("wdown_f8"), f8b=wp.get("wdown_f8b"), f4=wp.get("wdown_f4"), i4=wp.get("wdown_i4"), i8=wp.get("wdown_i8"))
        if _span is not None and not _span.head:
            return b, len(self.w["layers"])
        check(L.samd_rmsnorm_warm(_ptr(b["x"]), _ptr(delta), _ptr(self.w["norm"]), _ptr(b["h"]), R, s.hidden, s.eps, dt, dn, dstride,
                                  hint(self.w["lm_head"], self.wp["lm_head"] if self.wp else None, is_head=True), st))
        gemm(b["x"] if head else b["h"], self.w["lm_head"], self.wp["lm_head"] if self.wp else None, b["logits"])
        if not head:
            check(L.samd_argmax_rows(_ptr(b["logits"]), dt, R, s.vocab, s.vocab, None, _ptr(b["argmax"]), st))
        return b if _span is None else (b, len(self.w["layers"]))

    def _forward_rows_fold(self, R, b, d_tokens, d_relpos, d_mask, d_L, d_n):
        L, s, dt, st = lib(), self.shape, self.dt, current_stream()
        x, ssq = b["x"], b["ssq"]
        rows_cs = 8 if R <= 8 else 16
        rows_a = rows_cs if os.environ.get("SAMD_NORM_ROWS8", "1") != "0" else 16
        if s.head_dim == 128 and os.environ.get("SAMD_FUSE_EMBED_ROPE", "1") != "0":
            check(L.samd_embed_rows_ssq_rope(_ptr(d_tokens), _ptr(self.w["embed"]), _ptr(x), _ptr(ssq), 16, s.hidden, s.vocab, dt, _ptr(d_relpos), _ptr(d_L),
                                             _ptr(self.cos), _ptr(self.sin), _ptr(b["cs"]), R, s.head_dim, self.rope_rows, st))
        else:
            check(L.samd_embed_rows_ssq(_ptr(d_tokens), _ptr(self.w["embed"]), _ptr(x), _ptr(ssq), 16, s.hidden, s.vocab, dt, st))
            check(L.samd_rope_rows(_ptr(d_relpos), _ptr(d_L), _ptr(self.cos), _ptr(self.sin), _ptr(b["cs"]), R, s.head_dim, self.rope_rows, st))
        attn2d = b["attn"].view(b["attn"].shape[0], -1)
        qkv_launch = L.samd_gemm_qkv_rope_norm_vt if self.v_transposed else L.samd_gemm_qkv_rope_norm
        attn_launch = L.samd_tree_attention_vt if self.v_transposed else L.samd_tree_attention_warm
        for li, (w, wp) in enumerate(zip(self.w["layers"], self.wp["layers"])):
            if self.layer_hook is not None:
                self.layer_hook(li)
            check(qkv_launch(_ptr(x), _ptr(ssq), _ptr(w["ln1"]), s.eps, _ptr(wp["wqkv64"]), rows_a, s.hidden, _ptr(b["cs"]), _ptr(d_L), _ptr(d_n),
                             _ptr(b["q"]), _ptr(self.kv[li, 0]), _ptr(self.kv[li, 1]), s.heads, s.kv_heads, s.head_dim, self.max_len, dt, st))
            check(attn_launch(_ptr(b["q"]), _ptr(self.kv[li, 0]), _ptr(self.kv[li, 1]), _ptr(b["attn"]), dt, R, s.heads,
                              s.kv_heads, s.head_dim, self.max_len, _ptr(d_mask), _ptr(d_L), _ptr(d_n), self.scale,
                              _ptr(b["ws"]), b["ws_bytes"], None, st))
            check(L.samd_gemm_cs_residual(_ptr(attn2d), _ptr(wp["wo_g"]), rows_cs, s.hidden, attn2d.shape[1], _ptr(x), _ptr(ssq), dt, st))
            check(L.samd_gemm_pairs_silu_norm(_ptr(x), _ptr(ssq), _ptr(w["ln2"]), s.eps, _ptr(wp["wgu"]), rows_a, s.inter, s.hidden, _ptr(b["act"]), dt, st))
            check(L.samd_gemm_cs_residual(_ptr(b["act"]), _ptr(wp["wdown_g"]), rows_cs, s.hidden, s.inter, _ptr(x), _ptr(ssq), dt, st))
        check(L.samd_rmsnorm(_ptr(x), None, _ptr(self.w["norm"]), _ptr(b["h"]), R, s.hidden, s.eps, dt, 0, 0, st))
        wl = self.wp["lm_head"]
        if wl is not None:
            check(L.samd_gemm_skinny(_ptr(b["h"]), _ptr(wl), 16, s.vocab, s.hidden, 1, _ptr(b["part"]), _ptr(b["logits"]), dt, st))
        else:
            torch.mm(b["h"][:R], self.w["lm_head"].t(), out=b["logits"][:R])
        check(L.samd_argmax_rows(_ptr(b["logits"]), dt, R, s.vocab, s.vocab, None, _ptr(b["argmax"]), st))
        return b

    def prefill(self, session: Session, input_ids, on_chunk=None):
        ids = input_ids.reshape(-1).to(device=self.device, dtype=torch.int32)
        N = ids.numel()
        if N < 1 or N > self.max_len:
            raise SamdError(f"prompt of {N} tokens does not fit max_cache_len {self.max_len}")
        if N >= 2 * TILE_ROWS and os.environ.get("SAMD_PREFILL", "wide") != "chunked" and not self.row_major_released:
            return self._prefill_wide(session, ids, on_chunk)
        if N >= self.MOE_PF_MIN_ROWS and os.environ.get("SAMD_PREFILL", "wide") != "chunked" and self.shape.moe:
            return self._prefill_moe(session, ids, on_chunk)
        if (self.weight_format in QUANT_FORMATS and not self.shape.moe and os.environ.get("SAMD_PREFILL", "wide") != "chunked"
                and N >= quant_prefill_min_rows(self.QUANT_PF_MIN_ROWS)):
            return self._prefill_wide(session, ids, on_chunk)
        v = session.device_views()
        b = None
        for c0 in range(0, N, TILE_ROWS):
            n = min(TILE_ROWS, N - c0)
            self.pf_tokens.zero_()
            self.pf_tokens[:n] = ids[c0:c0 + n]
            self.pf_n.fill_(n)
            session.set_cache_length(c0)
            b = self.forward_rows(TILE_ROWS, self.pf_tokens, self.pf_relpos, self.pf_mask, v["cache_length"], self.pf_n)
            if on_chunk is not None:
                on_chunk(self.pf_tokens, b["logits"], n, b["h"])
        session.set_cache_length(N)
        session.set_start_token(b["argmax"][(N - 1) % TILE_ROWS:])
        return b["logits"][(N - 1) % TILE_ROWS]

    MOE_PF_MIN_ROWS = 2 * TILE_ROWS

    def _moe_prefill_state(self, rows):
        st = getattr(self, "_moe_pf", None)
        if st is not None and st["rows"] >= rows:
            return st
        s, dev, n_sl = self.shape, self.device, rows // TILE_ROWS
        z = lambda *sz: torch.zeros(sz, dtype=self.dtype, device=dev)
        zi = lambda *sz: torch.zeros(sz, dtype=torch.int32, device=dev)
        self._moe_pf = st = dict(rows=rows, x=z(rows, s.hidden), h=z(rows, s.hidden), tok=zi(rows), L=zi(n_sl), n=zi(n_sl), n_all=zi(1),
                                 cs=torch.zeros((n_sl, MAX_DRAFT, s.head_dim), dtype=torch.float32, device=dev),
                                 first_row=torch.arange(n_sl, dtype=torch.int32, device=dev) * TILE_ROWS,
                                 moe=MOE.MoeWideBuffers(rows, s.hidden, s.moe_inter, s.n_experts, s.top_k, self.dtype, self.dt, dev))
        return st

    class _Span:
        __slots__ = ("b", "first", "delta", "head")

        def __init__(self, b, first, delta, head):
            self.b, self.first, self.delta, self.head = b, first, delta, head

    def _prefill_moe(self, session: Session, ids, on_chunk=None):
        s, N, T = self.shape, ids.numel(), TILE_ROWS
        cap = MOE.prefill_rows()
        st = self._moe_prefill_state(min(cap, MOE.wide_rows_pad(N)))
        mb, base, n_layers = st["moe"], self._buffers(T), len(self.w["layers"])
        log_routes = self.route_log is not None and not torch.cuda.is_current_stream_capturing()
        b = j_last = None
        for s0 in range(0, N, cap):
            rows = min(cap, N - s0)
            n_sl = -(-rows // T)
            st["tok"][:n_sl * T].zero_()
            st["tok"][:rows] = ids[s0:s0 + rows]
            st["L"][:n_sl] = st["first_row"][:n_sl] + s0
            st["n"][:n_sl] = (rows - st["first_row"][:n_sl]).clamp(max=T)
            st["n_all"].fill_(rows)
            slices = [dict(base, x=st["x"][j * T:(j + 1) * T], h=st["h"][j * T:(j + 1) * T], cs=st["cs"][j]) for j in range(n_sl)]
            first = 0
            while True:
                due = n_layers
                for j in range(n_sl):
                    head = on_chunk is not None or (s0 + rows == N and j == n_sl - 1)
                    if first == n_layers and not head:
                        continue
                    span = self._Span(slices[j], first, None if first == 0 else mb.out[j * T:(j + 1) * T], head)
                    b, due = self.forward_rows(T, st["tok"][j * T:(j + 1) * T], self.pf_relpos, self.pf_mask, st["L"][j:j + 1], st["n"][j:j + 1], _span=span)
                    if due == n_layers and head:
                        j_last = j
                        if on_chunk is not None:
                            on_chunk(st["tok"][j * T:(j + 1) * T], b["logits"], min(T, rows - j * T), b["h"])
                if due == n_layers:
                    break
                wp = self.wp["layers"][due]
                mb.route(st["h"], self.w["layers"][due]["router"], st["n_all"], s.norm_topk, rows=rows)
                if log_routes:
                    RP = MOE.wide_rows_pad(rows)
                    self.route_log.append((due, rows, mb.topk_idx[:RP].clone(), mb.topk_w[:RP].clone()))
                mb.lists(st["n_all"], rows=rows)
                mb.experts(st["h"], wp["moe_gu"], wp["moe_down"], st["n_all"], self.expert_format, rows=rows)
                first = due + 1
        base["h"].copy_(b["h"])
        session.set_cache_length(N)
        session.set_start_token(base["argmax"][(N - 1) % T:])
        return base["logits"][(N - 1) % T]

    PF_SPLIT_MIN_ROWS = 1024
    PF_ATTN_PAD = 128

    def _is_gfx950(self):
        if not hasattr(self, "_gfx950"):
            name = getattr(torch.cuda.get_device_properties(self.device), "gcnArchName", "") or ""
            self._gfx950 = name.split(":")[0] == "gfx950"
        return self._gfx950

    def _time_mm(self, x, wt, out, reps=3):
        best = float("inf")
        torch.mm(x, wt, out=out)
        for _ in range(reps):
            e0, e1 = torch.cuda.Event(enable_timing=True), torch.cuda.Event(enable_timing=True)
            e0.record()
            torch.mm(x, wt, out=out)
            e1.record()
            e1.synchronize()
            best = min(best, e0.elapsed_time(e1))
        return best

    def tune_prefill(self, max_rows=None):
        self._pf_plan = {}
        if os.environ.get("SAMD_PREFILL_SPLIT", "1") == "0" or self.row_major_released:
            return self._pf_plan
        max_rows = min(int(max_rows or self.max_len), 4096)
        w0 = self.w["layers"][0]
        try:
            for key in ("wqkv", "wo", "wgu", "wdown"):
                wt = w0[key].t()
                K, N = wt.shape
                x = torch.zeros((max_rows + 64, K), dtype=self.dtype, device=self.device)
                out = torch.empty((max_rows + 64, N), dtype=self.dtype, device=self.device)
                small = {r: self._time_mm(x[:r], wt, out[:r]) for r in (64, 128, 192, 256)}
                plan = {}
                for R in range(max(256, (self.PF_SPLIT_MIN_ROWS // 256) * 256), max_rows, 256):
                    t_at = self._time_mm(x[:R], wt, out[:R])
                    t_past = self._time_mm(x[:R + 64], wt, out[:R + 64])
                    plan[R] = {r: t_at + small[r] < 0.95 * t_past for r in small}
                self._pf_plan[key] = plan
                del x, out
        except RuntimeError as e:
            import warnings
            warnings.warn(f"tune_prefill: measurement failed ({str(e)[:120]}); projections of long prompts stay single library calls", RuntimeWarning)
            self._pf_plan = {}
        return self._pf_plan

    def prefill_plan_summary(self):
        plan = getattr(self, "_pf_plan", None) or {}
        return {k: [R for R, d in sorted(v.items()) if any(d.values())] for k, v in plan.items()}

    def _pf_split(self, key, M):
        if M <= self.PF_SPLIT_MIN_ROWS:
            return 0
        if getattr(self, "_pf_plan", None) is None:
            self.tune_prefill()
        R = ((M - 1) // 256) * 256
        rest = -(-(M - R) // 64) * 64
        return R if self._pf_plan.get(key, {}).get(R, {}).get(rest, False) else 0

    QUANT_PF_MIN_ROWS = 256

    def _pf_weight(self, li, key):
        w = self.w["layers"][li][key]
        if self.weight_format not in QUANT_FORMATS:
            return w
        N, K = w.shape
        if getattr(self, "_qpf_scratch", None) is None:
            elems = max(self.w["layers"][0][k].shape[0] * self.w["layers"][0][k].shape[1] for k in F8.PROJECTIONS)
            self._qpf_scratch = torch.empty(elems, dtype=self.dtype, device=self.device)
        if N * K > self._qpf_scratch.numel():
            raise SamdError(f"projection {key} of layer {li}, shape ({N}, {K}), exceeds the prefill scratch of {self._qpf_scratch.numel()} elements")
        out = self._qpf_scratch[:N * K].view(N, K)
        L, lp, st = lib(), self.wp["layers"][li], current_stream()
        if self.weight_format == "fp8":
            check(L.samd_gemm_unpack_f8(_ptr(lp[key + "_f8"][0]), _ptr(lp[key + "_f8"][1]), N, K, _ptr(out), self.dt, st))
        elif self.weight_format == "fp8b128":
            check(L.samd_gemm_unpack_f8b(_ptr(lp[key + "_f8b"][0]), _ptr(lp[key + "_f8b"][1]), N, K, _ptr(out), self.dt, st))
        elif self.weight_format == "mxfp4":
            check(L.samd_gemm_unpack_f4(_ptr(lp[key + "_f4"]), N, K, _ptr(out), self.dt, st))
        elif self.weight_format == "int4g128":
            check(L.samd_gemm_unpack_i4(_ptr(lp[key + "_i4"]), N, K, _ptr(out), self.dt, st))
        else:
            check(L.samd_gemm_unpack_i8(_ptr(lp[key + "_i8"]), N, K, _ptr(out), self.dt, st))
        return out

    def _pf_mm(self, x, w, out, key, bias=None):
        R = self._pf_split(key, x.shape[0])
        mm = torch.mm if bias is None else (lambda a, b, out: torch.addmm(bias, a, b, out=out))
        if R:
            mm(x[:R], w.t(), out=out[:R])
            mm(x[R:], w.t(), out=out[R:])
        else:
            mm(x, w.t(), out=out)

    def _prefill_wide(self, session: Session, ids, on_chunk=None):
        L, s, dt, st, N = lib(), self.shape, self.dt, current_stream(), ids.numel()
        dev, ty = self.device, self.dtype
        z = lambda *sz: torch.empty(sz, dtype=ty, device=dev)
        x, h = z(N, s.hidden), z(N, s.hidden)
        own_attn = (s.head_dim == 128 and os.environ.get("SAMD_PREFILL_ATTENTION", "own") != "sdpa"
                    and self._is_gfx950())
        Np = N if own_attn else -(-N // self.PF_ATTN_PAD) * self.PF_ATTN_PAD
        if Np > self.max_len:
            Np = N
        ao = z(N, s.heads * s.head_dim) if own_attn else None
        qkv_p, qp = z(Np, (s.heads + 2 * s.kv_heads) * s.head_dim), z(Np, s.heads, s.head_dim)
        qkv, q = qkv_p[:N], qp[:N]
        if Np > N:
            qp[N:].zero_()
            if self.v_transposed:
                qkv_p[N:].zero_()
                self.kv[:, 0, :, N:Np].zero_()
            else:
                self.kv[:, :, :, N:Np].zero_()
        o, gu, act, d = z(N, s.hidden), z(N, 2 * s.inter), z(N, s.inter), z(N, s.hidden)
        relpos = torch.arange(N, dtype=torch.int32, device=dev)
        d_L = torch.zeros(1, dtype=torch.int32, device=dev)
        d_n = torch.full((1,), N, dtype=torch.int32, device=dev)
        check(L.samd_embed_rows(_ptr(ids), _ptr(self.w["embed"]), _ptr(x), N, s.hidden, s.vocab, dt, st))
        delta = None
        for li, w in enumerate(self.w["layers"]):
            check(L.samd_rmsnorm(_ptr(x), _ptr(delta), _ptr(w["ln1"]), _ptr(h), N, s.hidden, s.eps, dt, 0, 0, st))
            self._pf_mm(h, self._pf_weight(li, "wqkv"), qkv, "wqkv", bias=w.get("bqkv"))
            if self.epi is not None:
                check(L.samd_rope_kv_write_epi(_ptr(qkv), _ptr(relpos), _ptr(d_L), _ptr(d_n), _ptr(self.cos), _ptr(self.sin), None, _ptr(q),
                                               _ptr(self.kv[li, 0]), _ptr(self.kv[li, 1]), int(self.v_transposed), N, s.heads, s.kv_heads,
                                               s.head_dim, self.max_len, self.rope_rows, dt, 0, 0, C.byref(self.epi_nobias[li]), st))
                if self.v_transposed:
                    vv = qkv_p[:, (s.heads + s.kv_heads) * s.head_dim:].view(Np, s.kv_heads, s.head_dim).transpose(0, 1)
                else:
                    vv = self.kv[li, 1][:, :Np]
            elif self.v_transposed:
                check(L.samd_rope_kv_write_vt(_ptr(qkv), _ptr(relpos), _ptr(d_L), _ptr(d_n), _ptr(self.cos), _ptr(self.sin), _ptr(q),
                                              _ptr(self.kv[li, 0]), _ptr(self.kv[li, 1]), N, s.heads, s.kv_heads, s.head_dim, self.max_len,
                                              self.rope_rows, dt, 0, 0, st))
                vv = qkv_p[:, (s.heads + s.kv_heads) * s.head_dim:].view(Np, s.kv_heads, s.head_dim).transpose(0, 1)
            else:
                check(L.samd_rope_kv_write(_ptr(qkv), _ptr(relpos), _ptr(d_L), _ptr(d_n), _ptr(self.cos), _ptr(self.sin), _ptr(q),
                                           _ptr(self.kv[li, 0]), _ptr(self.kv[li, 1]), N, s.heads, s.kv_heads, s.head_dim, self.max_len,
                                           self.rope_rows, dt, 0, 0, st))
                vv = self.kv[li, 1][:, :Np]
            if own_attn:
                check((L.samd_prefill_attention_vt if self.v_transposed else L.samd_prefill_attention)(
                    _ptr(q), _ptr(self.kv[li, 0]), _ptr(self.kv[li, 1]), _ptr(ao), dt, N, 0, s.heads, s.kv_heads,
                    s.head_dim, self.max_len, self.scale, st))
                self._pf_mm(ao, self._pf_weight(li, "wo"), o, "wo")
            else:
                kk = self.kv[li, 0][:, :Np]
                if s.kv_heads != s.heads:
                    kk, vv = kk.repeat_interleave(s.heads // s.kv_heads, dim=0), vv.repeat_interleave(s.heads // s.kv_heads, dim=0)
                att = torch.nn.functional.scaled_dot_product_attention(qp.transpose(0, 1)[None], kk[None], vv[None], is_causal=True, scale=self.scale)
                self._pf_mm(att[0, :, :N].transpose(0, 1).reshape(N, -1), self._pf_weight(li, "wo"), o, "wo")
            check(L.samd_rmsnorm(_ptr(x), _ptr(o), _ptr(w["ln2"]), _ptr(h), N, s.hidden, s.eps, dt, 0, 0, st))
            self._pf_mm(h, self._pf_weight(li, "wgu"), gu, "wgu")
            check(L.samd_silu_mul(_ptr(gu), _ptr(act), N, s.inter, dt, 0, 0, st))
            self._pf_mm(act, self._pf_weight(li, "wdown"), d, "wdown")
            delta = d
        check(L.samd_rmsnorm(_ptr(x), _ptr(delta), _ptr(self.w["norm"]), _ptr(h), N, s.hidden, s.eps, dt, 0, 0, st))
        b = self._buffers(1)
        if on_chunk is None:
            torch.mm(h[N - 1:N], self.w["lm_head"].t(), out=b["logits"][:1])
        else:
            logits = torch.mm(h, self.w["lm_head"].t())
            for c0 in range(0, N, TILE_ROWS):
                n = min(TILE_ROWS, N - c0)
                on_chunk(ids[c0:c0 + n], logits[c0:c0 + n], n, h[c0:c0 + n])
            b["logits"][:1].copy_(logits[N - 1:N])
        check(L.samd_argmax_rows(_ptr(b["logits"]), dt, 1, s.vocab, s.vocab, None, _ptr(b["argmax"]), st))
        session.set_cache_length(N)
        session.set_start_token(b["argmax"])
        return b["logits"][0]

    def warm(self, R):
        self.pf_n.zero_()
        scratch_L = torch.zeros(1, dtype=torch.int32, device=self.device)
        self.forward_rows(R, self.pf_tokens, self.pf_relpos, self.pf_mask, scratch_L, self.pf_n)
        torch.cuda.current_stream().synchronize()

    def hidden_rows(self, R):
        return self._buffers(R)["h"]

    def forward_tokens(self, session: Session, tokens, relpos, mask_rows, n, L, return_hidden=False):
        R = self.bucket(n)
        tok = torch.zeros(MAX_DRAFT, dtype=torch.int32, device=self.device)
        tok[:n] = tokens.reshape(-1)[:n].to(torch.int32)
        rel = torch.zeros(MAX_DRAFT, dtype=torch.int32, device=self.device)
        rel[:n] = relpos.reshape(-1)[:n].to(torch.int32)
        d_n = torch.tensor([n], dtype=torch.int32, device=self.device)
        session.set_cache_length(L)
        b = self.forward_rows(R, tok, rel, mask_rows, session.device_views()["cache_length"], d_n)
        torch.cuda.current_stream().synchronize()
        return (b["logits"][:n], b["h"][:n]) if return_hidden else b["logits"][:n]

    def verify(self, session: Session, R):
        v = session.device_views()
        n_ptr = C.c_void_p(v["dmeta"] + 4)
        return self.forward_rows(R, v["tokens"], v["position"], v["mask"], v["cache_length"], n_ptr)

    def compact(self, session: Session):
        s = self.shape
        session.kv_compact(self.kv_ptrs, 2 * s.layers, s.kv_heads, self.max_len, s.head_dim, self.kv.element_size(), n_transposed=s.layers if self.v_transposed else 0)
```

Baseline: 815.1.

## Add exact-row GEMM variants and per-row-count graphs for 5 and 9 draft rows

Generalizes the norm-fold QKV, gate/up and output GEMM kernels to fetch any activation row count up to 16, using exec-masked loads for odd counts, and instantiates 5- and 9-row variants. The decode engine captures extra graphs per (bucket, next-row-count) and picks the exact-row graph when the upcoming draft size matches. This cuts activation loads and staging for the padded rows in the 16-row bucket. In exchange it adds more captured graphs and compile instantiations, and correctness relies on the masked inline-asm loads and the zero-filled LDS rows.

```diff
diff --git a/sam-decoding_amd/csrc/gemm_kernels.hip b/sam-decoding_amd/csrc/gemm_kernels.hip
--- a/sam-decoding_amd/csrc/gemm_kernels.hip
+++ b/sam-decoding_amd/csrc/gemm_kernels.hip
@@ -214,6 +214,11 @@
     return out;
 }
 
+__device__ __forceinline__ void norm_load_masked(u32x4 &xd, u32x4 &gd, const void *xsrc, const void *gsrc, unsigned long long mask) {
+    unsigned long long saved;
+    asm volatile("s_and_saveexec_b64 %2, %5\n\tglobal_load_dwordx4 %0, %3, off\n\tglobal_load_dwordx4 %1, %4, off\n\ts_mov_b64 exec, %2"
+                 : "=&v"(xd), "=&v"(gd), "=&s"(saved) : "v"(xsrc), "v"(gsrc), "s"(mask) : "memory", "scc");
+}
 
 template <int DEPTH, int PC>
 __device__ __forceinline__ void gemm_wait_younger(int younger) {
@@ -246,8 +251,10 @@
 
     const int tid = threadIdx.x, w = tid >> 6, l = tid & 63, n = l & 15, g = l >> 4;
     const bool streams = CG == 4 || w < 2 * CG;
-    static_assert(AR == 16 || (AR == 8 && NORM && RT == 1), "8 activation rows: the norm-fold kernels only");
-    const bool stager = AR == 16 || w < GEMM_WAVES / 2;
+    static_assert(AR == 16 || (AR >= 1 && AR < 16 && NORM && RT == 1), "fewer than 16 activation rows: the norm-fold kernels only");
+    const bool stager = AR == 16 || w < (AR + 1) / 2;
+    const bool stages = !(AR & 1) ? stager : tid < 32 * AR;
+    const unsigned long long stage_mask = (AR & 1) && __builtin_amdgcn_readfirstlane(w) == AR / 2 ? 0xffffffffull : ~0ull;
     const int cg = CG == 4 ? (w & 3) : (streams ? w % CG : 0), kh = CG == 4 ? (w >> 2) : (streams ? w / CG : 0);
     const char *wtile = reinterpret_cast<const char *>(W) + (size_t)blockIdx.x * n_chunks * CH;
     const uint32_t wlane = (uint32_t)(64 * (CG * kh + cg) + l) * 16;
@@ -274,8 +281,11 @@
         const E *src = A + (size_t)row * K + (size_t)c * GEMM_KC + 8 * unit;
         if constexpr (NORM) {
             const E *gsrc = reinterpret_cast<const E *>(na.g) + (size_t)c * GEMM_KC + 8 * unit;
-            asm volatile("global_load_dwordx4 %0, %1, off" : "=v"(xr[d][i]) : "v"(src) : "memory");
-            asm volatile("global_load_dwordx4 %0, %1, off" : "=v"(gr[d][i]) : "v"(gsrc) : "memory");
+            if constexpr (AR & 1) norm_load_masked(xr[d][i], gr[d][i], src, gsrc, stage_mask);
+            else {
+                asm volatile("global_load_dwordx4 %0, %1, off" : "=v"(xr[d][i]) : "v"(src) : "memory");
+                asm volatile("global_load_dwordx4 %0, %1, off" : "=v"(gr[d][i]) : "v"(gsrc) : "memory");
+            }
         } else {
             E *dst = &xs[buf][0][0] + (size_t)(NT * i + 64 * w) * 8;
             __builtin_amdgcn_global_load_lds((gptr_t)src, (lptr_t)dst, 16, 0, 0);
@@ -297,7 +307,7 @@
                 const int slot = tid + NT * i, row = slot >> 5;
                 asm volatile("" : "+v"(xr[d][i]), "+v"(gr[d][i]) : : "memory");
                 const u32x4 v = norm_scale8<E>(xr[d][i], gr[d][i], norm_rs[row]);
-                *reinterpret_cast<u32x4 *>(&xs[buf][0][0] + (size_t)slot * 8) = v;
+                if (stages) *reinterpret_cast<u32x4 *>(&xs[buf][0][0] + (size_t)slot * 8) = v;
             }
         }
     };
@@ -345,8 +355,8 @@
 #pragma unroll
     for (int d = 0; d < DEPTH; d++)
         if (d < n_chunks) issue(wr[d], d, d, d);
-    if constexpr (AR == 8) {
-        if (!stager) {
+    if constexpr (AR < 16) {
+        if (!stages) {
 #pragma unroll
             for (int bz = 0; bz < NB; bz++) *reinterpret_cast<u32x4 *>(&xs[bz][0][0] + (size_t)tid * 8) = (u32x4){0u, 0u, 0u, 0u};
         }
@@ -444,8 +454,10 @@
 #endif
     const int p0 = (int)((long long)blockIdx.x * n_pairs / gridDim.x), p1 = (int)((long long)(blockIdx.x + 1) * n_pairs / gridDim.x);
     const bool active = w < 2 * (p1 - p0);
-    static_assert(AR == 16 || (AR == 8 && NORM && RT == 1), "8 activation rows: the norm-fold kernels only");
-    const bool stager = AR == 16 || w < GEMM_WAVES / 2;
+    static_assert(AR == 16 || (AR >= 1 && AR < 16 && NORM && RT == 1), "fewer than 16 activation rows: the norm-fold kernels only");
+    const bool stager = AR == 16 || w < (AR + 1) / 2;
+    const bool stages = !(AR & 1) ? stager : tid < 32 * AR;
+    const unsigned long long stage_mask = (AR & 1) && w == AR / 2 ? 0xffffffffull : ~0ull;
     const int gi = 2 * p0 + w;
     const char *wgrp = reinterpret_cast<const char *>(W) + (size_t)(active ? gi : 0) * n_chunks * 8192;
     const uint32_t wlane = (uint32_t)l * 16;
@@ -475,8 +487,11 @@
             const E *src = A + (size_t)((abl & 8) ? (row & 15) : row) * K + (size_t)c * GEMM_KC + 8 * unit;
             if constexpr (NORM) {
                 const E *gsrc = reinterpret_cast<const E *>(na.g) + (size_t)c * GEMM_KC + 8 * unit;
-                asm volatile("global_load_dwordx4 %0, %1, off" : "=v"(xr[d][i]) : "v"(src) : "memory");
-                asm volatile("global_load_dwordx4 %0, %1, off" : "=v"(gr[d][i]) : "v"(gsrc) : "memory");
+                if constexpr (AR & 1) norm_load_masked(xr[d][i], gr[d][i], src, gsrc, stage_mask);
+                else {
+                    asm volatile("global_load_dwordx4 %0, %1, off" : "=v"(xr[d][i]) : "v"(src) : "memory");
+                    asm volatile("global_load_dwordx4 %0, %1, off" : "=v"(gr[d][i]) : "v"(gsrc) : "memory");
+                }
             } else {
                 E *dst = &xs[buf][0][0] + (size_t)(NT * i + 64 * w) * 8;
                 __builtin_amdgcn_global_load_lds((gptr_t)src, (lptr_t)dst, 16, 0, 0);
@@ -495,7 +510,7 @@
                     const int slot = tid + NT * i, row = slot >> 5;
                     asm volatile("" : "+v"(xr[d][i]), "+v"(gr[d][i]) : : "memory");
                     const u32x4 v = norm_scale8<E>(xr[d][i], gr[d][i], norm_rs[row]);
-                    *reinterpret_cast<u32x4 *>(&xs[buf][0][0] + (size_t)slot * 8) = v;
+                    if (stages) *reinterpret_cast<u32x4 *>(&xs[buf][0][0] + (size_t)slot * 8) = v;
                 }
             }
             asm volatile("s_waitcnt lgkmcnt(0)" ::: "memory");
@@ -540,8 +555,8 @@
 #pragma unroll
     for (int d = 0; d < DEPTH; d++)
         if (d < n_chunks) { if (active) load_w(wr[d], d); stage_x(d, d, d); }
-    if constexpr (AR == 8) {
-        if (!stager) {
+    if constexpr (AR < 16) {
+        if (!stages) {
 #pragma unroll
             for (int bz = 0; bz < NB; bz++) *reinterpret_cast<u32x4 *>(&xs[bz][0][0] + (size_t)tid * 8) = (u32x4){0u, 0u, 0u, 0u};
         }
@@ -599,14 +614,15 @@
     const char *wgrp = reinterpret_cast<const char *>(W) + (size_t)blockIdx.x * n_chunks * 8192;
     const uint32_t wlane = (uint32_t)l * 16;
 
-    static_assert(ROWS == 8 || ROWS == 16, "");
-    constexpr int AL = ROWS / 2;
-    if constexpr (ROWS == 8) {
+    static_assert(ROWS >= 1 && ROWS <= 16, "");
+    constexpr int AL = (ROWS + 1) / 2;
+    if constexpr (ROWS < 16) {
 #pragma unroll
         for (int buf = 0; buf < CSD; buf++)
 #pragma unroll
-            for (int i = 4; i < 8; i++)
-                *reinterpret_cast<u32x4 *>(xs + (size_t)buf * 16 * GEMM_KC + (size_t)(64 * i + l) * 8) = (u32x4){0u, 0u, 0u, 0u};
+            for (int i = ROWS / 2; i < 8; i++)
+                if (!(ROWS & 1) || i > ROWS / 2 || l >= 32)
+                    *reinterpret_cast<u32x4 *>(xs + (size_t)buf * 16 * GEMM_KC + (size_t)(64 * i + l) * 8) = (u32x4){0u, 0u, 0u, 0u};
         asm volatile("s_waitcnt lgkmcnt(0)" ::: "memory");
     }
     floatx4 acc = (floatx4){0.f, 0.f, 0.f, 0.f};
@@ -625,7 +641,8 @@
             const int slot = l + 64 * i, row = slot >> 5, pos = slot & 31, unit = pos ^ (row & 15);
             const E *src = A + (size_t)row * K + (size_t)c * GEMM_KC + 8 * unit;
             E *dst_l = xs + (size_t)buf * 16 * GEMM_KC + (size_t)(64 * i) * 8;
-            __builtin_amdgcn_global_load_lds((gptr_t)src, (lptr_t)dst_l, 16, 0, 0);
+            if ((ROWS & 1) && i == AL - 1) { if (l < 32) __builtin_amdgcn_global_load_lds((gptr_t)src, (lptr_t)dst_l, 16, 0, 0); }
+            else __builtin_amdgcn_global_load_lds((gptr_t)src, (lptr_t)dst_l, 16, 0, 0);
             asm volatile("" ::: "memory");
         }
     };
@@ -771,6 +788,8 @@
     return hipSuccess;
 }
 
+static bool samd_rows_fetch_ok(int rows) { return rows == 5 || rows == 8 || rows == 9 || rows == 16; }
+
 extern "C" {
 
 int samd_gemm_splits(int32_t N, int32_t K, int32_t rows_pad) {
@@ -820,9 +839,9 @@
 
 int samd_gemm_pairs_silu_norm(const void *d_x, const float *d_ssq, const void *d_norm_weight, float eps, const void *d_Wg, int32_t rows_pad, int32_t inter, int32_t K,
                               void *d_out, int32_t dtype, void *stream) {
-    if (!d_x || !d_ssq || !d_norm_weight || !d_Wg || !d_out || (rows_pad != 16 && rows_pad != 8) || inter < 16 || inter % 16 != 0 || K < GEMM_KC || K % GEMM_KC != 0 ||
+    if (!d_x || !d_ssq || !d_norm_weight || !d_Wg || !d_out || !samd_rows_fetch_ok(rows_pad) || inter < 16 || inter % 16 != 0 || K < GEMM_KC || K % GEMM_KC != 0 ||
         K / 16 > 32 * NORM_NS || (dtype != SAMD_F16 && dtype != SAMD_BF16)) {
-        samd_set_error("samd_gemm_pairs_silu_norm: unsupported shape (8 or 16 rows, inter %% 16 == 0, K %% 256 == 0, K <= 8192, f16/bf16) or null pointer"); return SAMD_E_INVALID;
+        samd_set_error("samd_gemm_pairs_silu_norm: unsupported shape (5, 8, 9 or 16 rows, inter %% 16 == 0, K %% 256 == 0, K <= 8192, f16/bf16) or null pointer"); return SAMD_E_INVALID;
     }
     const int n_cu = samd_cu_count();
     const int n_pairs = inter / 16;
@@ -830,19 +849,20 @@
     while ((n_pairs + grid - 1) / grid > 4) grid += n_cu;
     const NormArgs na{d_ssq, d_norm_weight, K / 16, 1.f / (float)K, eps};
     hipStream_t st = (hipStream_t)stream;
-    const hipError_t e = rows_pad == 8
-        ? (dtype == SAMD_F16 ? pairs_silu_launch<GF16, 1, 3, true, 8>(st, grid, d_x, d_Wg, d_out, K, inter, n_pairs, na)
-                             : pairs_silu_launch<GBF16, 1, 3, true, 8>(st, grid, d_x, d_Wg, d_out, K, inter, n_pairs, na))
-        : (dtype == SAMD_F16 ? pairs_silu_launch<GF16, 1, 3, true>(st, grid, d_x, d_Wg, d_out, K, inter, n_pairs, na)
-                             : pairs_silu_launch<GBF16, 1, 3, true>(st, grid, d_x, d_Wg, d_out, K, inter, n_pairs, na));
+    hipError_t e = hipSuccess;
+#define GO(TT, AR) e = pairs_silu_launch<TT, 1, 3, true, AR>(st, grid, d_x, d_Wg, d_out, K, inter, n_pairs, na)
+#define ROWS(TT) do { if (rows_pad == 5) GO(TT, 5); else if (rows_pad == 8) GO(TT, 8); else if (rows_pad == 9) GO(TT, 9); else GO(TT, 16); } while (0)
+    if (dtype == SAMD_F16) ROWS(GF16); else ROWS(GBF16);
+#undef ROWS
+#undef GO
     if (e != hipSuccess) { samd_set_error("samd_gemm_pairs_silu_norm: %s", hipGetErrorString(e)); return SAMD_E_HIP; }
     LAUNCHCHK();
     return SAMD_OK;
 }
 
 int samd_gemm_cs_residual(const void *d_A, const void *d_Wg, int32_t rows_pad, int32_t N, int32_t K, void *d_x, float *d_ssq, int32_t dtype, void *stream) {
-    if (!d_A || !d_Wg || !d_x || !d_ssq || (rows_pad != 16 && rows_pad != 8) || N < 16 || N % 16 != 0 || K < GEMM_KC || K % GEMM_KC != 0 || (dtype != SAMD_F16 && dtype != SAMD_BF16)) {
-        samd_set_error("samd_gemm_cs_residual: unsupported shape (8 or 16 rows, N %% 16 == 0, K %% 256 == 0, f16/bf16) or null pointer"); return SAMD_E_INVALID;
+    if (!d_A || !d_Wg || !d_x || !d_ssq || !samd_rows_fetch_ok(rows_pad) || N < 16 || N % 16 != 0 || K < GEMM_KC || K % GEMM_KC != 0 || (dtype != SAMD_F16 && dtype != SAMD_BF16)) {
+        samd_set_error("samd_gemm_cs_residual: unsupported shape (5, 8, 9 or 16 rows, N %% 16 == 0, K %% 256 == 0, f16/bf16) or null pointer"); return SAMD_E_INVALID;
     }
     constexpr int lds = GEMM_WAVES * 2 * 16 * GEMM_KC * 2;
     hipStream_t st = (hipStream_t)stream;
@@ -850,8 +870,9 @@
 #define GO(TT, ROWS, ET) do { static unsigned long long done = 0ull; \
         e = samd_reserve_lds((const void *)k_gemm_cs_residual<TT, ROWS>, lds, &done); \
         if (e == hipSuccess) hipLaunchKernelGGL((k_gemm_cs_residual<TT, ROWS>), dim3(N / 16), dim3(64 * GEMM_WAVES), lds, st, (const ET *)d_A, (const ET *)d_Wg, (ET *)d_x, d_ssq, K, N, K / GEMM_KC, (const int *)nullptr, (int *)nullptr, 0); } while (0)
-    if (dtype == SAMD_F16) { if (rows_pad == 8) GO(GF16, 8, _Float16); else GO(GF16, 16, _Float16); }
-    else { if (rows_pad == 8) GO(GBF16, 8, __bf16); else GO(GBF16, 16, __bf16); }
+#define ROWS(TT, ET) do { if (rows_pad == 5) GO(TT, 5, ET); else if (rows_pad == 8) GO(TT, 8, ET); else if (rows_pad == 9) GO(TT, 9, ET); else GO(TT, 16, ET); } while (0)
+    if (dtype == SAMD_F16) ROWS(GF16, _Float16); else ROWS(GBF16, __bf16);
+#undef ROWS
 #undef GO
     if (e != hipSuccess) { samd_set_error("samd_gemm_cs_residual: %s", hipGetErrorString(e)); return SAMD_E_HIP; }
     LAUNCHCHK();
@@ -965,8 +986,8 @@
                                    const float *d_cs, const int32_t *d_cache_length, const int32_t *d_n, void *d_q_out, void *d_k_cache, void *d_v_cache,
                                    int32_t n_heads, int32_t n_kv_heads, int32_t head_dim, int64_t max_len, int32_t dtype, void *stream, int v_t) {
     if (!d_x || !d_ssq || !d_norm_weight || !d_W64 || !d_cs || !d_cache_length || !d_n || !d_q_out || !d_k_cache || !d_v_cache || head_dim != 128 || n_heads < 1 ||
-        n_kv_heads < 1 || (rows_pad != 16 && rows_pad != 8) || K < GEMM_KC || K % GEMM_KC != 0 || K / 16 > 32 * NORM_NS || (dtype != SAMD_F16 && dtype != SAMD_BF16)) {
-        samd_set_error("samd_gemm_qkv_rope_norm: unsupported shape (8 or 16 rows, head_dim 128, K %% 256 == 0, K <= 8192, f16/bf16) or null pointer"); return SAMD_E_INVALID;
+        n_kv_heads < 1 || !samd_rows_fetch_ok(rows_pad) || K < GEMM_KC || K % GEMM_KC != 0 || K / 16 > 32 * NORM_NS || (dtype != SAMD_F16 && dtype != SAMD_BF16)) {
+        samd_set_error("samd_gemm_qkv_rope_norm: unsupported shape (5, 8, 9 or 16 rows, head_dim 128, K %% 256 == 0, K <= 8192, f16/bf16) or null pointer"); return SAMD_E_INVALID;
     }
     const int groups = qkv_tile_groups(n_heads + 2 * n_kv_heads);
     const int tiles = (n_heads + 2 * n_kv_heads) * 128 / (16 * groups);
@@ -974,13 +995,10 @@
     hipStream_t st = (hipStream_t)stream;
     hipError_t e = hipSuccess;
 #define GO(TT, CG, AR) e = qkv_rope_launch<TT, 1, 4, CG, true, AR>(st, d_x, d_W64, K, tiles, d_cs, d_cache_length, d_n, d_q_out, d_k_cache, d_v_cache, n_heads, n_kv_heads, (long long)max_len, v_t, na)
-    if (rows_pad == 8) {
-        if (groups == 3) { if (dtype == SAMD_F16) GO(GF16, 3, 8); else GO(GBF16, 3, 8); }
-        else { if (dtype == SAMD_F16) GO(GF16, 4, 8); else GO(GBF16, 4, 8); }
-    } else {
-        if (groups == 3) { if (dtype == SAMD_F16) GO(GF16, 3, 16); else GO(GBF16, 3, 16); }
-        else { if (dtype == SAMD_F16) GO(GF16, 4, 16); else GO(GBF16, 4, 16); }
-    }
+#define ROWS(TT, CG) do { if (rows_pad == 5) GO(TT, CG, 5); else if (rows_pad == 8) GO(TT, CG, 8); else if (rows_pad == 9) GO(TT, CG, 9); else GO(TT, CG, 16); } while (0)
+    if (groups == 3) { if (dtype == SAMD_F16) ROWS(GF16, 3); else ROWS(GBF16, 3); }
+    else { if (dtype == SAMD_F16) ROWS(GF16, 4); else ROWS(GBF16, 4); }
+#undef ROWS
 #undef GO
     if (e != hipSuccess) { samd_set_error("samd_gemm_qkv_rope_norm: %s", hipGetErrorString(e)); return SAMD_E_HIP; }
     LAUNCHCHK();
diff --git a/sam-decoding_amd/samd_hip/engine.py b/sam-decoding_amd/samd_hip/engine.py
--- a/sam-decoding_amd/samd_hip/engine.py
+++ b/sam-decoding_amd/samd_hip/engine.py
@@ -117,8 +117,8 @@
         session.set_start_token(self.target[n:n + 1])
         return last
 
-    def verify(self, session, R):
-        b = self.runner.verify(session, R)
+    def verify(self, session, R, rows_fetch=None):
+        b = self.runner.verify(session, R, rows_fetch=rows_fetch)
         session.scripted_argmax(self.target, self.target_len, self.vocab, b["argmax"])
         if self.ranked_logits:
             if self.order1_hot_vocab > 0:
@@ -133,8 +133,11 @@
     def bucket(self, n):
         return self.runner.bucket(n)
 
-    def warm(self, R):
-        self.runner.warm(R)
+    def warm(self, R, rows_fetch=None):
+        self.runner.warm(R, rows_fetch=rows_fetch)
+
+    def rows_exact(self, R):
+        return self.runner.rows_exact(R)
 
     def hidden_rows(self, R):
         return self.runner.hidden_rows(R)
@@ -171,6 +174,7 @@
         self._report_np = self.report_buf.numpy()
         self.use_graphs = use_graphs
         self._graphs = {}
+        self._graphs_exact = {}
         self.bucket_steps = {}
         self._views = session.device_views()
         self._n_ptr = self._views["dmeta"] + 4
@@ -186,8 +190,19 @@
         self.recycle.draft(self._views["start_token"], self.tr_tokens)
         self.session.set_draft_if_deferred(self.tr_tokens, self.tr_parent, self.recycle.n_nodes, reverse=True)
 
-    def _enqueue_step(self, R):
-        b = self.verifier.verify(self.session, R)
+    def _verify(self, R, rows_fetch=None):
+        if rows_fetch is None:
+            return self.verifier.verify(self.session, R)
+        return self.verifier.verify(self.session, R, rows_fetch=rows_fetch)
+
+    def _rows_exact(self, R):
+        fn = getattr(self.verifier, "rows_exact", None)
+        if fn is None or self.recycle is not None or type(self) is not DecodeEngine:
+            return ()
+        return tuple(fn(R))
+
+    def _enqueue_step(self, R, rows_fetch=None):
+        b = self._verify(R, rows_fetch)
         if self.recycle is not None:
             self._recycle_update(self._views["tokens"], b["logits"], min(R, MAX_DRAFT), C.c_void_p(self._n_ptr))
         self.session.step(self.static, self.params, b["argmax"])
@@ -239,6 +254,7 @@
             g = self._graphs.get(R)
             if g is None:
                 g = self._capture(R)
+            g = self._graphs_exact.get((R, n_next), g)
         if push is not None:
             last = int(push[0][REPORT_INTS])
         if g is None:
@@ -334,7 +350,13 @@
         return StepReport(self._report_np)
 
     def _capture(self, R):
-        self._warm(R)
+        g = self._graphs[R] = self._capture_one(R)
+        for n in self._rows_exact(R):
+            self._graphs_exact[(R, n)] = self._capture_one(R, n)
+        return g
+
+    def _capture_one(self, R, rows_fetch=None):
+        self._warm(R, rows_fetch)
         torch.cuda.current_stream().synchronize()
         runner = getattr(self.verifier, "runner", self.verifier)
         cuts = [int(x) for x in os.environ.get("SAMD_GRAPH_SPLIT_LAYER", "2").split(",") if x.strip()]
@@ -345,7 +367,7 @@
         if not cuts and not eager:
             g = torch.cuda.CUDAGraph()
             with torch.cuda.graph(g):
-                self._enqueue_step(R)
+                self._enqueue_step(R, rows_fetch)
         else:
             def head():
                 def stop(li):
@@ -353,7 +375,7 @@
                         raise _StopForward()
                 runner.layer_hook = stop
                 try:
-                    self.verifier.verify(self.session, R)
+                    self._verify(R, rows_fetch)
                 except _StopForward:
                     pass
                 finally:
@@ -380,7 +402,7 @@
                         g.parts[part[0]].capture_begin()
                 runner.layer_hook = hook
                 try:
-                    self._enqueue_step(R)
+                    self._enqueue_step(R, rows_fetch)
                 except BaseException:
                     runner.layer_hook = None
                     try:
@@ -394,13 +416,15 @@
                     runner.layer_hook = None
                 g.parts[part[0]].capture_end()
             cur.wait_stream(side)
-        self._graphs[R] = g
         return g
 
-    def _warm(self, R):
+    def _warm(self, R, rows_fetch=None):
         v = self.verifier
         if hasattr(v, "warm"):
-            v.warm(R)
+            if rows_fetch is None:
+                v.warm(R)
+            else:
+                v.warm(R, rows_fetch=rows_fetch)
 
 
 class TreeModelEngine(DecodeEngine):
diff --git a/sam-decoding_amd/samd_hip/llama.py b/sam-decoding_amd/samd_hip/llama.py
--- a/sam-decoding_amd/samd_hip/llama.py
+++ b/sam-decoding_amd/samd_hip/llama.py
@@ -142,6 +142,7 @@
 class LlamaRunner:
 
     BUCKETS = (1, 8, 16, 32, 48, 64, 128)
+    ROWS_EXACT = (5, 9)
 
     def __init__(self, shape, weights, max_cache_len, dtype=torch.float16, device="cuda", kv=None, native_gemm=True, packed_lm_head=None,
                  attention=None, weight_format=None, draft_head=False, expert_format=MOE.AUTO):
@@ -1022,7 +1023,7 @@
                 return b
         raise SamdError(f"draft of {n} nodes exceeds {MAX_DRAFT}")
 
-    def forward_rows(self, R, d_tokens, d_relpos, d_mask, d_L, d_n, x_in=None, d_vis=None, _span=None):
+    def forward_rows(self, R, d_tokens, d_relpos, d_mask, d_L, d_n, x_in=None, d_vis=None, _span=None, rows_fetch=None):
         if self.shape.moe:
             MOE.reject_unsupported(draft_head=getattr(self, "draft_head", False))
         if self._rows_pad(R) > self.native_gemm_max_rows and self.row_major_released:
@@ -1033,7 +1034,7 @@
         resumed = _span is not None and _span.first > 0
         if (_span is None and self.norm_fold and RP == 16 and x_in is None and d_vis is None and not getattr(self, "draft_head", False)
                 and RP <= self.native_gemm_max_rows):
-            return self._forward_rows_fold(R, b, d_tokens, d_relpos, d_mask, d_L, d_n)
+            return self._forward_rows_fold(R, b, d_tokens, d_relpos, d_mask, d_L, d_n, rows_fetch)
 
         def hint(w, wp, fused=False, is_head=False):
             if wp is None or RP > self.native_gemm_max_rows or self.warm_kb <= 0:
@@ -1167,11 +1168,15 @@
             check(L.samd_argmax_rows(_ptr(b["logits"]), dt, R, s.vocab, s.vocab, None, _ptr(b["argmax"]), st))
         return b if _span is None else (b, len(self.w["layers"]))
 
-    def _forward_rows_fold(self, R, b, d_tokens, d_relpos, d_mask, d_L, d_n):
+    def _forward_rows_fold(self, R, b, d_tokens, d_relpos, d_mask, d_L, d_n, rows_fetch=None):
         L, s, dt, st = lib(), self.shape, self.dt, current_stream()
         x, ssq = b["x"], b["ssq"]
         rows_cs = 8 if R <= 8 else 16
         rows_a = rows_cs if os.environ.get("SAMD_NORM_ROWS8", "1") != "0" else 16
+        if rows_fetch is not None:
+            if rows_fetch not in self.ROWS_EXACT or self.bucket(rows_fetch) != R:
+                raise SamdError(f"rows_fetch {rows_fetch} is not an exact-row form of bucket {R}")
+            rows_cs = rows_a = rows_fetch
         if s.head_dim == 128 and os.environ.get("SAMD_FUSE_EMBED_ROPE", "1") != "0":
             check(L.samd_embed_rows_ssq_rope(_ptr(d_tokens), _ptr(self.w["embed"]), _ptr(x), _ptr(ssq), 16, s.hidden, s.vocab, dt, _ptr(d_relpos), _ptr(d_L),
                                              _ptr(self.cos), _ptr(self.sin), _ptr(b["cs"]), R, s.head_dim, self.rope_rows, st))
@@ -1466,10 +1471,10 @@
         session.set_start_token(b["argmax"])
         return b["logits"][0]
 
-    def warm(self, R):
+    def warm(self, R, rows_fetch=None):
         self.pf_n.zero_()
         scratch_L = torch.zeros(1, dtype=torch.int32, device=self.device)
-        self.forward_rows(R, self.pf_tokens, self.pf_relpos, self.pf_mask, scratch_L, self.pf_n)
+        self.forward_rows(R, self.pf_tokens, self.pf_relpos, self.pf_mask, scratch_L, self.pf_n, rows_fetch=rows_fetch)
         torch.cuda.current_stream().synchronize()
 
     def hidden_rows(self, R):
@@ -1487,10 +1492,16 @@
         torch.cuda.current_stream().synchronize()
         return (b["logits"][:n], b["h"][:n]) if return_hidden else b["logits"][:n]
 
-    def verify(self, session: Session, R):
+    def rows_exact(self, R):
+        if (not self.norm_fold or self._rows_pad(R) != 16 or self.native_gemm_max_rows < 16 or getattr(self, "draft_head", False)
+                or os.environ.get("SAMD_ROWS_EXACT", "1") == "0"):
+            return ()
+        return tuple(n for n in self.ROWS_EXACT if self.bucket(n) == R)
+
+    def verify(self, session: Session, R, rows_fetch=None):
         v = session.device_views()
         n_ptr = C.c_void_p(v["dmeta"] + 4)
-        return self.forward_rows(R, v["tokens"], v["position"], v["mask"], v["cache_length"], n_ptr)
+        return self.forward_rows(R, v["tokens"], v["position"], v["mask"], v["cache_length"], n_ptr, rows_fetch=rows_fetch)
 
     def compact(self, session: Session):
         s = self.shape
```

New measurement: 825.0, median of 6. 1.2% higher.
